# TRI-ML/sdflabel

Hardware: AMD Instinct MI355X
Metric: rendered rays/sec (fwd+bwd) (higher is better)
Workload: dtype f32; 1 GPU; BASELINE configs[1]: one 256x256 crop(s) per GPU, DeepSDF 8x512 on a 40^3 grid, fwd+bwd to yaw/trans/latent, decoder re-evaluated every step; crops_per_gpu=1, rays_per_crop=65536, grid_points=64000, surfels=2751, front_facing=763, parallelism=crop-parallel x1

## Files before the change

### include/sdfr.h

```cpp
#ifndef SDFR_H
#define SDFR_H

#include <stdint.h>

#ifdef __cplusplus
extern "C" {
#endif

#define SDFR_OK 0
#define SDFR_E_INVALID (-1)
#define SDFR_E_HIP (-2)
#define SDFR_E_UNSUPPORTED (-3)

#define SDFR_MAX_LAYERS 16
#define SDFR_TRACE_LEVELS 6
#define SDFR_TRACE_COUNTERS 32

#define SDFR_VERSION 421

int sdfr_version(void);
int sdfr_build_flags(void);
const char* sdfr_last_error(void);

typedef struct sdfr_decoder sdfr_decoder;

int sdfr_decoder_create(sdfr_decoder** out, int n_lin, const int* in_dim, const int* out_dim,
                        const int* inj_n, const int* inj_off, const float* const* h_W, const float* const* h_b,
                        const float* const* h_ln_w, const float* const* h_ln_b, int n_inputs, int use_tanh, int device);
int sdfr_decoder_destroy(sdfr_decoder* dec);
int64_t sdfr_decoder_macs(const sdfr_decoder* dec);

int sdfr_mlp_forward(const sdfr_decoder* dec, const float* inputs, int64_t n, float* sdf,
                     uint32_t* mask_ws ,
                     void* stream);
int sdfr_grid_tile_order(int D, int32_t* out);
int sdfr_mlp_forward_ordered(const sdfr_decoder* dec, const float* inputs, int64_t n, float* sdf, uint32_t* mask_ws, const int32_t* order,
                             int64_t order_rows, void* stream);
int64_t sdfr_mlp_balance_bytes(int64_t order_rows);
int sdfr_mlp_balance_init(void* state, const int32_t* order, int64_t order_rows, void* stream);
int sdfr_mlp_forward_balanced(const sdfr_decoder* dec, const float* inputs, int64_t n, float* sdf, uint32_t* mask_ws, void* state,
                              int64_t order_rows, void* stream);
int sdfr_mlp_forward_f16(const sdfr_decoder* dec, const float* inputs, int64_t n, float* sdf, uint32_t* mask_ws, void* stream);

int sdfr_mlp_forward_f16_counted(const sdfr_decoder* dec, const float* inputs, int64_t n_max, const int32_t* n_dev, float* sdf, uint32_t* mask_ws,
                                 void* stream);

int sdfr_mlp_forward_split(const sdfr_decoder* dec, const float* inputs, int64_t n, float* sdf, uint32_t* mask_ws, void* stream);
int sdfr_mlp_forward_split_counted(const sdfr_decoder* dec, const float* inputs, int64_t n_max, const int32_t* n_dev, float* sdf, void* stream);
int64_t sdfr_decoder_mask_words(const sdfr_decoder* dec, int64_t n);

int sdfr_mlp_jacobian(const sdfr_decoder* dec, const float* inputs, int64_t rows_per_crop, int B,
                      const int32_t* idx, int cap, const int32_t* cnt, float* J, float* sdf_sel,
                      const float* sdf_full ,
                      const uint32_t* mask_ws ,
                      int mask_from_f16 ,
                      void* stream);


int sdfr_band_select(const float* sdf, int64_t G, int B, float thr, int32_t* idx, int cap, int32_t* cnt,
                     int32_t* slot, int32_t* scratch, void* stream);

int sdfr_surface_project(const float* xyz, int xyz_stride, const float* sdf, int64_t G, int B,
                         const int32_t* idx, int cap, const int32_t* cnt, const float* J, int Jstride, int Joff,
                         float* points, float* nocs, float* normals, void* stream);

int sdfr_surface_project_bwd(const float* g_points, const float* g_nocs, const float* normals, int64_t G, int B,
                             const int32_t* idx, int cap, const int32_t* cnt, float* g_sdf, float* g_xyz, void* stream);

int sdfr_scatter_values(float* dst, const float* src, const int32_t* idx, int64_t G, int B, int cap, const int32_t* cnt, void* stream);
int sdfr_band_select_margin(const float* sdf, int64_t G, int B, float thr, const float* thr_extra, int32_t* idx, int cap, int32_t* cnt,
                            int32_t* slot, int32_t* scratch, void* stream);
int sdfr_prefilter_guard(float* sdf_grid, const float* sdf_exact, const int32_t* idx, int64_t G, int B, int cap, const int32_t* cnt,
                         float* margin, float* max_dev, int32_t* violations, void* stream);
int sdfr_prefilter_plan(const float* inputs, int64_t G, int n_inputs, int L, int B, float lip, const float* margin, const float* max_dev,
                        float* lat_ref, int32_t* age, int max_reuse, int32_t* reuse, int32_t* n_full, void* stream);
int sdfr_mlp_forward_f16_skip(const sdfr_decoder* dec, const float* inputs, int64_t n, float* sdf, const int32_t* skip, int64_t rows_per_crop,
                              void* stream);
int sdfr_band_select_skip(const float* sdf, int64_t G, int B, float thr, const float* thr_extra, const int32_t* skip, int32_t* idx, int cap,
                          int32_t* cnt, int32_t* slot, int32_t* scratch, void* stream);
int sdfr_prefilter_guard2(float* sdf_grid, const float* sdf_exact, const int32_t* idx, int64_t G, int B, int cap, const int32_t* cnt,
                          float* margin, float* max_dev, int32_t* violations, const int32_t* reused, void* stream);
int sdfr_gather_rows(float* out, const float* src, int ncol, const int32_t* idx, const int32_t* slot, int64_t G, int B, int cap,
                     int src_cap, const int32_t* cnt, void* stream);
int sdfr_prefilter_audit_select(const float* inputs, const int32_t* cslot, int64_t G, int n_inputs, int B, int stride, const int32_t* phase,
                                float* rows, int32_t* src, int32_t* n_audit, int cap_rows, void* stream);
int sdfr_prefilter_audit_check(const float* sdf_grid, const float* sdf_exact, const int32_t* src, const int32_t* n_audit, int cap_rows,
                               int64_t G, int B, float thr, const int32_t* reused, float* audit_dev, int32_t* violations, int32_t* phase,
                               void* stream);

int sdfr_candidate_rows(const float* inputs, int64_t G, int n_inputs, int B, const int32_t* cidx, int stride, const int32_t* ccnt, float* rows,
                        void* stream);
int sdfr_mlp_forward_f16_ragged(const sdfr_decoder* dec, const float* inputs, int B, int64_t rows_per_crop, const int32_t* cnt, float* sdf,
                                uint32_t* mask_ws, int half_tiles, void* stream);
int sdfr_candidate_band_map(const int32_t* idx, int cap, const int32_t* cnt, const int32_t* cslot, int64_t G, int B, int stride, int32_t* pos,
                            int32_t* violations, void* stream);
int sdfr_mlp_forward_skip(const sdfr_decoder* dec, const float* inputs, int64_t n, float* sdf, const int32_t* skip, int64_t rows_per_crop,
                          void* stream);
int sdfr_mlp_forward_ragged(const sdfr_decoder* dec, const float* inputs, int B, int64_t rows_per_crop, const int32_t* cnt, float* sdf,
                            uint32_t* mask_ws, int half_tiles, void* stream);

int sdfr_sdf_input_grad(const float* g_sdf, const int32_t* slot, const float* J, int n_inputs, int64_t G, int B, int cap,
                        float* g_inputs, int32_t* n_uncached, void* stream);

int sdfr_project_dcm(const float* pose, const float* K, const float* points, const float* normals, const float* colors,
                     int B, int cap, const int32_t* cnt, int output_nocs, int res_x, int res_y,
                     float* p_cam, float* n_cam, float* col, float* uv, int32_t* fidx, int32_t* fcnt, float* xyzf, int32_t* fslot,
                     void* stream);

int sdfr_surfels_forward(const float* xyz, int xyz_stride, const float* sdf, int64_t G, const int32_t* idx, const float* J, int Jstride,
                         int Joff, const float* pose, const float* K, int B, int cap, const int32_t* cnt, int output_nocs, int res_x,
                         int res_y, float diam, float* points, float* normals, float* p_cam, float* n_cam, float* col, int32_t* fidx,
                         int32_t* fcnt, float* xyzf, int32_t* fslot, int32_t* bbox, void* stream);

int sdfr_project_dcm_bwd(const float* pose, const float* points, const float* normals,
                         const float* g_p_cam, const float* g_n_cam, const float* g_col,
                         int B, int cap, const int32_t* cnt, int output_nocs,
                         float* g_points, float* g_normals, float* g_colors, float* g_pose, const float* g_xyzf, const int32_t* fslot,
                         void* stream);

#define SDFR_JAC_MANY_ROWS 16
#define SDFR_JAC_HALF_TILES 32
#define SDFR_JAC_QUARTER_TILES 64
#define SDFR_PRIM_BOXES_READY 256
#define SDFR_PRIM_BINS 512
int64_t sdfr_splat_ws_words(int B, int cap, int W, int H);
int sdfr_splat_forward(int primitive, const float* K, const float* Kinv, const float* p_cam, const float* n_cam, const float* attr,
                       const float* uv, const float* znorm, const float* bg, const float* bg_logit,
                       int B, int cap, const int32_t* cnt, int W, int H, float diam, float depth_constant,
                       int32_t* bbox_ws ,
                       float* color, float* mask, float* depth, float* normals, float* aux, void* stream);

int sdfr_splat_backward(int primitive, const float* K, const float* Kinv, const float* p_cam, const float* n_cam, const float* attr,
                        const float* uv, const float* znorm, const float* bg, const float* bg_logit,
                        int B, int cap, const int32_t* cnt, int W, int H, float diam, float depth_constant,
                        const float* aux, const float* color, const float* mask, const float* depth, const float* normals,
                        const float* g_color, const float* g_mask, const float* g_depth, const float* g_normals,
                        float* g_p_cam, float* g_n_cam, float* g_attr, void* stream);

int64_t sdfr_splat_ws_words_r(int B, int cap, int tiles_cap);
int sdfr_surfels_forward_r(const float* xyz, int xyz_stride, const float* sdf, int64_t G, const int32_t* idx, const float* J, int Jstride,
                           int Joff, const float* pose, const float* K, int B, int cap, const int32_t* cnt, int output_nocs,
                           const int32_t* wh, int tiles_cap, float diam, float* points, float* normals, float* p_cam, float* n_cam, float* col,
                           int32_t* fidx, int32_t* fcnt, float* xyzf, int32_t* fslot, int32_t* bbox, void* stream);
int sdfr_splat_forward_r(int flags , const float* K, const float* Kinv, const float* p_cam,
                         const float* n_cam, const float* attr, int B, int cap, const int32_t* cnt, const int32_t* wh, int pix_stride,
                         int tiles_cap, float diam, float depth_constant, int32_t* bbox_ws, float* color, float* mask, float* depth,
                         float* normals, float* aux, void* stream);
int sdfr_splat_backward_r(const float* K, const float* Kinv, const float* p_cam, const float* n_cam, const float* attr, int B, int cap,
                          const int32_t* cnt, const int32_t* wh, int pix_stride, float diam, float depth_constant, const float* aux,
                          const float* color, const float* mask, const float* depth, const float* normals, const float* g_color,
                          const float* g_mask, const float* g_depth, const float* g_normals, float* g_p_cam, float* g_n_cam, float* g_attr,
                          void* stream);
int sdfr_loss_2d_r(const float* rend, const float* target, int B, const int32_t* wh, int pix_stride, int tiles16_cap, float diam,
                   float threshold_nocs, float weight, float* loss, float* g_rend, int32_t* nvalid, float* scratch, void* stream);

int sdfr_splat_weights(int primitive, const float* K, const float* Kinv, const float* p_cam, const float* n_cam, const float* uv,
                       const float* znorm, const float* bg_logit, int B, int cap, const int32_t* cnt, int W, int H, float diam,
                       float depth_constant, const float* aux, float* weights, void* stream);
int sdfr_splat_weights_backward(int primitive, const float* K, const float* Kinv, const float* p_cam, const float* n_cam, const float* uv,
                                const float* znorm, int has_bg_row, int B, int cap, const int32_t* cnt, int W, int H, float diam,
                                float depth_constant, const float* aux, const float* g_weights, const float* wsum, float* g_p_cam,
                                float* g_n_cam, void* stream);

int sdfr_splat_forward_clamp(int primitive, const float* K, const float* Kinv, const float* p_cam, const float* n_cam, const float* attr,
                             const float* uv, const float* znorm, const float* bg, const float* bg_logit, int B, int cap, const int32_t* cnt,
                             int W, int H, float diam, float depth_constant, int clamp_alt, float clamp_constant, int32_t* bbox_ws,
                             float* color, float* mask, float* depth, float* normals, float* aux, void* stream);
int sdfr_splat_weights_clamp(int primitive, const float* K, const float* Kinv, const float* p_cam, const float* n_cam, const float* uv,
                             const float* znorm, const float* bg_logit, int B, int cap, const int32_t* cnt, int W, int H, float diam,
                             float depth_constant, int clamp_alt, float clamp_constant, const float* aux, float* weights, void* stream);
int sdfr_splat_weights_backward_clamp(int primitive, const float* K, const float* Kinv, const float* p_cam, const float* n_cam, const float* uv,
                                      const float* znorm, int has_bg_row, int B, int cap, const int32_t* cnt, int W, int H, float diam,
                                      float depth_constant, int clamp_alt, float clamp_constant, const float* aux, const float* g_weights,
                                      const float* wsum, float* g_p_cam, float* g_n_cam, void* stream);


int sdfr_params_forward(const float* yaw, const float* trans, const float* latent, int L, const float* grid, int64_t G, int B,
                        float* inputs, float* pose, float* latnorm, void* stream);

int sdfr_surface_latent_grad(const float* g_points, const float* g_nocs, const float* normals, const float* J, int n_inputs, int L,
                             int B, int cap, const int32_t* cnt, float* g_latn, void* stream);

int sdfr_params_backward(const float* yaw, const float* latent, int L, const float* latnorm, const float* g_pose, const float* g_latn,
                         int B, float* g_yaw, float* g_trans, float* g_latent, void* stream);

int sdfr_pose_latent_backward(const float* pose, const float* points, const float* normals, const float* g_p_cam, const float* g_n_cam,
                              const float* g_col, int B, int cap, const int32_t* cnt, int output_nocs, const float* g_xyzf,
                              const int32_t* fslot, const float* J, int n_inputs, int L, const float* yaw, const float* latent,
                              const float* latnorm, float* g_points, float* g_pose, float* g_latn, float* g_yaw, float* g_trans,
                              float* g_latent, void* stream);

int sdfr_gather_rows3(float* out, const float* src, const int32_t* idx, int B, int cap, const int32_t* cnt, void* stream);
int sdfr_scatter_add_rows3(float* dst, const float* src, const int32_t* idx, int B, int cap, const int32_t* cnt, void* stream);


int sdfr_loss_3d(const float* est, const int32_t* ecnt, int ecap, const float* lidar, const int32_t* lcnt, int lcap, const float* scale,
                 float threshold, float weight, int B, float* loss, float* g_est, float* g_scale, int32_t* npairs, float* scratch,
                 void* stream);

int sdfr_loss_2d(const float* rend, const float* target, int B, int H, int W, float diam, float threshold_nocs, float weight,
                 float* loss, float* g_rend, int32_t* nvalid, float* scratch , void* stream);

int sdfr_solver_step(float* params, const float* grads, int L, const float* loss2d, const float* loss3d, const int32_t* npairs,
                     float w2, float w3, float* adam_m, float* adam_v, int32_t* adam_t, float lr_adam, float lr_scale, float lr_latent,
                     int B, float* total, int32_t* stepped, void* stream);

int sdfr_params_plan(const float* yaw, const float* trans, const float* latent, int L, const float* grid, int64_t G, int B, float* inputs,
                     float* pose, float* latnorm, float lip, const float* margin, const float* max_dev, float* lat_ref, int32_t* age,
                     int max_reuse, int32_t* reuse, int32_t* n_full, void* stream);
int sdfr_band_select_ex(const float* sdf, int64_t G, int B, float thr, const float* thr_extra, const int32_t* skip, int32_t* idx, int cap,
                        int32_t* cnt, int32_t* slot, int32_t* scratch, int32_t* over, int over_bit, void* stream);
int sdfr_mlp_forward_candidates(const sdfr_decoder* d, const float* inputs, int64_t rows_per_crop_in, int B, const int32_t* cidx, int64_t stride,
                                const int32_t* cnt, float* sdf, uint32_t* mask_ws, int half, int half_tiles, void* stream);
int sdfr_candidate_band(float* sdf_grid, const float* csdf, const int32_t* cidx, int64_t G, int B, int stride, const int32_t* ccnt, float thr,
                        int32_t* idx, int cap, int32_t* cnt, int32_t* pos, int32_t* over, void* stream);
int sdfr_losses_fused(const float* rend, const float* target, int B, int H, int W, const int32_t* wh, int pix_stride, int tiles16_cap, float diam,
                      float threshold_nocs, float weight2d, float* loss2d, float* g_rend, int32_t* nvalid, float* scratch2, const float* est,
                      const int32_t* ecnt, int ecap, const float* lidar, const int32_t* lcnt, int lcap, const float* scale, float threshold3d,
                      float weight3d, float* loss3d, float* g_est, float* g_scale, int32_t* npairs, float* scratch3, float* kscale,
                      void* stream);
int sdfr_splat_backward_x(const float* K, const float* Kinv, const float* p_cam, const float* n_cam, const float* attr, int B, int cap,
                          const int32_t* cnt, int W, int H, const int32_t* wh, int pix_stride, float diam, float depth_constant, const float* aux,
                          const float* color, const float* g_color, const float* kscale, float* g_p_cam, float* g_n_cam, float* g_attr,
                          const int32_t* bbox_ws, void* stream);
int sdfr_pose_latent_solver(const float* pose, const float* points, const float* normals, const float* g_p_cam, const float* g_n_cam,
                            const float* g_col, int B, int cap, const int32_t* cnt, int output_nocs, const float* g_xyzf, const int32_t* fslot,
                            const float* kscale, const float* J, int n_inputs, int L, const float* yaw, const float* latent, const float* latnorm,
                            float* g_pose, float* g_latn, float* params, float* grads, const float* loss2d, const float* loss3d,
                            const int32_t* npairs, float w2, float w3, float* adam_m, float* adam_v, int32_t* adam_t, float lr_adam,
                            float lr_scale, float lr_latent, float* total, int32_t* stepped, void* stream);

int sdfr_mlp_forward_counted(const sdfr_decoder* dec, const float* inputs, int64_t n_max, const int32_t* n_dev, float* sdf, int half,
                             void* stream);
int sdfr_trace_setup(const float* pose, const float* Kinv, const float* latn, int L, int B, int W, int H, float bound, float near,
                     int32_t* counters, int32_t* pix,
                     float* lam ,
                     float* far, float* inputs, const float* cone, int cone_block, void* stream);
int sdfr_trace_setup2(const float* pose, const float* Kinv, const float* latn, int L, int B, int W, int H, float bound, float near,
                      int32_t* counters, int32_t* pix, float* lam, float* far, float* inputs, const float* cone, int cone_block, float* hit_lam,
                      float* hit_sdf, void* stream);
int sdfr_trace_cone(const sdfr_decoder* dec, const float* pose, const float* Kinv, const float* latn, int L, int B, int W, int H, float bound,
                    float near, float eps, int block, int cone_steps, int spec_k, float sigma, int half, int32_t* counters, int32_t* ids0,
                    float* st0, float* aux0, int32_t* ids1, float* st1, float* aux1, float* inputs, float* sdf, float* cone, void* stream);
int sdfr_trace_step(const float* pose, const float* Kinv, const float* latn, int L, int W, int H, float eps, const float* sdf,
                    int32_t* counters, int step, int64_t n_max, const int32_t* pix_in, const float* lam_in, int32_t* pix_out, float* lam_out,
                    const float* far, float* inputs, float* hit_lam, float* hit_sdf, void* stream);

int sdfr_trace_pool(void);
int sdfr_trace_march(const sdfr_decoder* dec, const float* pose, const float* Kinv, const float* latn, int L, int B, int W, int H, float eps,
                     int steps, int head_steps, int tail_rows, const int32_t* levels, int n_levels, float q_max, float sigma, int half,
                     int32_t* counters, int32_t* pix0, float* lam0, int32_t* pix1, float* lam1, int32_t* pix2, float* lam2, const float* far,
                     float* inputs, float* sdf, float* tail_rows_buf, float* hit_lam, float* hit_sdf, void* stream);
int sdfr_trace_hits(const float* pose, const float* Kinv, const float* latn, int L, int B, int W, int H, const float* hit_lam, int32_t* n_hits,
                    int32_t* hit_slot, int32_t* idx, float* rows, void* stream);
int sdfr_trace_composite(const float* pose, const float* Kinv, int L, int B, int W, int H, const float* hit_lam, const int32_t* hit_slot,
                         const float* J, const float* f0, float* color, float* mask, float* depth, float* normals, float* lam_s, void* stream);
int64_t sdfr_trace_backward_ws_floats(int B, int W, int H);
int sdfr_trace_backward(const float* pose, const float* Kinv, int L, int B, int W, int H, const float* hit_lam, const int32_t* hit_slot,
                        const float* J, const float* f0, const float* g_color, const float* g_depth, const float* g_normals, float* ws,
                        float* g_pose, float* g_latn, void* stream);

typedef struct sdfr_extents { const int32_t* wh; int pix_stride; int cone_cap; } sdfr_extents;
int sdfr_trace_setup_r(const float* pose, const float* Kinv, const float* latn, int L, int B, const sdfr_extents* ext, float bound, float near,
                       int32_t* counters, int32_t* pix, float* lam, float* far, float* inputs, const float* cone, int cone_block, float* hit_lam,
                       float* hit_sdf, void* stream);
int sdfr_trace_cone_r(const sdfr_decoder* dec, const float* pose, const float* Kinv, const float* latn, int L, int B, const sdfr_extents* ext,
                      float bound, float near, float eps, int block, int cone_steps, int spec_k, float sigma, int half, int32_t* counters,
                      int32_t* ids0, float* st0, float* aux0, int32_t* ids1, float* st1, float* aux1, float* inputs, float* sdf, float* cone,
                      void* stream);
int sdfr_trace_march_r(const sdfr_decoder* dec, const float* pose, const float* Kinv, const float* latn, int L, int B, const sdfr_extents* ext, float eps,
                       int steps, int head_steps, int tail_rows, const int32_t* levels, int n_levels, float q_max, float sigma, int half,
                       int32_t* counters, int32_t* pix0, float* lam0, int32_t* pix1, float* lam1, int32_t* pix2, float* lam2, const float* far,
                       float* inputs, float* sdf, float* tail_rows_buf, float* hit_lam, float* hit_sdf, void* stream);
int sdfr_trace_hits_r(const float* pose, const float* Kinv, const float* latn, int L, int B, const sdfr_extents* ext, const float* hit_lam,
                      int32_t* n_hits, int32_t* hit_slot, int32_t* idx, float* rows, void* stream);
int sdfr_trace_composite_r(const float* pose, const float* Kinv, int L, int B, const sdfr_extents* ext, const float* hit_lam, const int32_t* hit_slot,
                           const float* J, const float* f0, float* color, float* mask, float* depth, float* normals, float* lam_s, void* stream);
int sdfr_trace_points_r(const float* Kinv, int B, const sdfr_extents* ext, const int32_t* hit_slot, const float* lam_s, float* xyzf, int ecap,
                        int32_t* ecnt, int32_t* pt_slot, void* stream);
int sdfr_trace_refine_backward_r(const float* pose, const float* Kinv, int L, int B, const sdfr_extents* ext, const float* hit_lam,
                                 const int32_t* hit_slot, const float* J, const float* f0, const float* g_color, const float* g_depth,
                                 const float* g_normals, const float* g_xyzf, const int32_t* pt_slot, int ecap, int surfel, float* ws ,
                                 float* g_pose, float* g_latn, void* stream);

int sdfr_trace_points(const float* Kinv, int B, int W, int H, const int32_t* hit_slot, const float* lam_s, float* xyzf, int ecap,
                      int32_t* ecnt, int32_t* pt_slot, void* stream);
int sdfr_trace_refine_backward(const float* pose, const float* Kinv, int L, int B, int W, int H, const float* hit_lam, const int32_t* hit_slot,
                               const float* J, const float* f0, const float* g_color, const float* g_depth, const float* g_normals,
                               const float* g_xyzf, const int32_t* pt_slot, int ecap, int surfel, float* ws, float* g_pose, float* g_latn,
                               void* stream);

int sdfr_scale_net(const float* latent_row, int L, const float* W1, const float* b1, const float* W2, const float* b2, const float* W3,
                   const float* b3, float* out, void* stream);

int64_t sdfr_ransac_ws_bytes(int B, int ncap, int T);
int sdfr_ransac_sample(int64_t seed, const int64_t* keys, const int32_t* ncnt, int B, int T, int32_t* idx, void* stream);
int sdfr_ransac_pose(const float* model, const float* model_cls, const int32_t* mcnt, int mcap, int model_f16, const float* scene,
                     const float* scene_cls, const int32_t* ncnt, int ncap, int B, const int32_t* idx, int64_t seed, const int64_t* keys,
                     int T, int type, float scale_model, const double* h_thr, void* ws, int32_t* found, int32_t* best, int32_t* n_inliers,
                     float* scale, float* rot, float* tra, int32_t* cnn_idx, int32_t* gate, int32_t* counts, int32_t* idx_out, void* stream);

int sdfr_rotate_iou(const float* boxes, int N, const float* qboxes, int K, int G, const int32_t* boff, const int32_t* qoff,
                    const int64_t* ooff, int criterion, float* out, int64_t out_len, void* stream);
int sdfr_box3d_iou(const double* boxes, int N, const double* qboxes, int K, int G, const int32_t* boff, const int32_t* qoff,
                   const int64_t* ooff, int criterion, int camera_frame, const float* rinc, float* out, int64_t out_len, void* stream);
int sdfr_image_box_iou(const double* boxes, int N, const double* qboxes, int K, int G, const int32_t* boff, const int32_t* qoff,
                       const int64_t* ooff, int criterion, double* out, int64_t out_len, void* stream);

int64_t sdfr_eval_ws_bytes(int G, int NG, int C, int S, int max_nd, int frames_per_chunk);
int sdfr_eval_center_dist(const double* dt_loc, int ND, const double* gt_loc, int NG, int G, const int32_t* doff, const int32_t* goff,
                          const int64_t* ooff, int camera_frame, double* out, int64_t out_len, void* stream);
int sdfr_eval_match_scores(const void* overlaps, int ov_f32, int64_t ov_len, const int64_t* ooff, const int32_t* doff, const int32_t* goff,
                           int G, int ND, int NG, const double* dt_score, const int8_t* ign_dt, const int8_t* ign_gt, int ML, int K,
                           const double* min_overlap, int max_nd, void* ws, int64_t ws_bytes, double* out, void* stream);
int sdfr_eval_thresholds(const double* scores, int NG, const int64_t* num_gt, int ML, int K, int S, void* ws, int64_t ws_bytes, double* thr,
                         int32_t* nthr, int32_t* count, void* stream);
int sdfr_eval_pr(const void* overlaps, int ov_f32, int64_t ov_len, const int64_t* ooff, const int32_t* doff, const int32_t* goff, int G,
                 int ND, int NG, const double* dt_score, const double* dt_yaw, const double* dt_alpha, const double* gt_yaw,
                 const double* gt_alpha, const double* dt_bbox, const int8_t* ign_dt, const int8_t* ign_gt, const double* dc_boxes,
                 int NDC, const int32_t* dc_off, int ML, int K, const double* min_overlap, const double* thr, const int32_t* nthr,
                 int S, int angular, int max_nd, int frames_per_chunk, void* ws, int64_t ws_bytes, double* pr, void* stream);

int sdfr_reproject(const float* depth, const float* color, const int32_t* meta, const float* kinv, int B, int max_pix, int filter, int cap,
                   float* points, float* colors, int32_t* cnt, int32_t* scratch, int32_t* over, int over_bit, void* stream);
int sdfr_point_extents(const float* pts, const int64_t* off, const int32_t* cnt, int cap, int B, const float* A, const float* scale,
                       const float* t, const float* K, int flags, float* ext, int32_t* n_out, void* stream);

int sdfr_depth_map(const void* lidar, int lidar_f64, int N, const float* planes, const double* cam, int w, int h, float* depth,
                   int32_t* winner, int32_t* info, void* stream);
int sdfr_depth_map_masked(const void* lidar, int lidar_f64, int N, const uint8_t* mask, const float* planes, const double* cam, int w, int h,
                          float* depth, int32_t* winner, int32_t* info, void* stream);
int sdfr_match_boxes(const double* anno, int A, const double* det, int M, int32_t* best, double* iou, int32_t* keep, void* stream);
int sdfr_css_input(const float* image, int H, int W, const int32_t* meta, int A, const float* masks, int ksize, int n_hblocks,
                   int32_t* coef, uint8_t* tmp, float* im, float* im_orig, uint8_t* u8, void* stream);

#define SDFR_AUG_PARAMS 20
#define SDFR_AUG_BRIGHTNESS 0
#define SDFR_AUG_CONTRAST 1
#define SDFR_AUG_SATURATION 2
#define SDFR_AUG_HUE 3
#define SDFR_AUG_ORDER 4
#define SDFR_AUG_MATRIX 8
#define SDFR_AUG_BOX_I 14
#define SDFR_AUG_BOX_J 15
#define SDFR_AUG_BOX_H 16
#define SDFR_AUG_BOX_W 17
int sdfr_augment(const uint8_t* rgb_src, const uint8_t* uvw_src, const int32_t* meta, const double* params, int B, int ksize, int32_t* tab,
                 uint8_t* jit, uint8_t* mid_rgb, uint8_t* mid_uvw, float* rgb, uint8_t* uvw, uint8_t* mask, uint8_t* rgb_u8, void* stream);

int64_t sdfr_lidar_normals_ws_bytes(int N);
int sdfr_lidar_normals(const void* points, int points_f64, int N, const float* planes, float radius, int max_nn, double* normals,
                       int32_t* nn_count, int32_t* nn_idx, uint8_t* in_frustum, void* workspace, int64_t workspace_bytes, void* stream);

int sdfr_css_head(const float* x_u, const float* x_v, const float* x_w, const float* x_mask, int B, int C, int H, int W, const float* w_u,
                  const float* b_u, const float* w_v, const float* b_v, const float* w_w, const float* b_w, const float* w_mask,
                  const float* b_mask, float* uvw_sm, float* uvw_sm_masked, float* mask, float* mask_sm, float* u, float* v, float* w,
                  void* stream);
int sdfr_css_latent(const float* x4, int B, int C, int h, int w, const float* w_lat, const float* b_lat, float* latent, void* stream);

#define SDFR_CSS_LOSS_WS_FIXED 16045824ll
int sdfr_css_head_loss(const float* x_u, const float* x_v, const float* x_w, const float* x_mask, int B, int C, int H, int W, const float* w_u,
                       const float* b_u, const float* w_v, const float* b_v, const float* w_w, const float* b_w, const float* w_mask,
                       const float* b_mask, const uint8_t* uvw_gt, const uint8_t* mask_gt, float* loss, float* dx_u, float* dx_v, float* dx_w,
                       float* dx_mask, float* dw_u, float* db_u, float* dw_v, float* db_v, float* dw_w, float* db_w, float* dw_mask,
// ... 95 lines not shown
```

### sdflabel_amd/_lib.py

```python
import ctypes
import os
from ctypes import POINTER, c_char_p, c_float, c_int, c_int32, c_int64, c_void_p

_HERE = os.path.dirname(os.path.abspath(__file__))
LIB_PATH = os.environ.get("SDFR_LIB") or os.path.join(_HERE, "lib", "libsdfr_hip.so")

ABI_VERSION = 421
_lib = None

_PROTOS = {
    "sdfr_version": (c_int, []),
    "sdfr_build_flags": (c_int, []),
    "sdfr_last_error": (c_char_p, []),
    "sdfr_debug_set_trace": (c_int, [c_void_p]),
    "sdfr_debug_set_tile_trace": (c_int, [c_void_p, c_int64]),
    "sdfr_mlp_forward_counted": (c_int, [c_void_p, c_void_p, c_int64, c_void_p, c_void_p, c_int, c_void_p]),
    "sdfr_trace_setup": (c_int, [c_void_p, c_void_p, c_void_p, c_int, c_int, c_int, c_int, c_float, c_float, c_void_p, c_void_p, c_void_p,
                                 c_void_p, c_void_p, c_void_p, c_int, c_void_p]),
    "sdfr_trace_setup2": (c_int, [c_void_p, c_void_p, c_void_p, c_int, c_int, c_int, c_int, c_float, c_float, c_void_p, c_void_p, c_void_p,
                                  c_void_p, c_void_p, c_void_p, c_int, c_void_p, c_void_p, c_void_p]),
    "sdfr_trace_cone": (c_int, [c_void_p, c_void_p, c_void_p, c_void_p, c_int, c_int, c_int, c_int, c_float, c_float, c_float, c_int, c_int,
                                c_int, c_float, c_int, c_void_p, c_void_p, c_void_p, c_void_p, c_void_p, c_void_p, c_void_p, c_void_p, c_void_p,
                                c_void_p, c_void_p]),
    "sdfr_trace_step": (c_int, [c_void_p, c_void_p, c_void_p, c_int, c_int, c_int, c_float, c_void_p, c_void_p, c_int, c_int64, c_void_p,
                                c_void_p, c_void_p, c_void_p, c_void_p, c_void_p, c_void_p, c_void_p, c_void_p]),
    "sdfr_trace_march": (c_int, [c_void_p, c_void_p, c_void_p, c_void_p, c_int, c_int, c_int, c_int, c_float, c_int, c_int, c_int, c_void_p, c_int,
                                 c_float, c_float, c_int, c_void_p, c_void_p, c_void_p, c_void_p, c_void_p, c_void_p, c_void_p, c_void_p,
                                 c_void_p, c_void_p, c_void_p, c_void_p, c_void_p, c_void_p]),
    "sdfr_trace_pool": (c_int, []),
    "sdfr_trace_hits": (c_int, [c_void_p, c_void_p, c_void_p, c_int, c_int, c_int, c_int, c_void_p, c_void_p, c_void_p, c_void_p, c_void_p, c_void_p]),
    "sdfr_trace_composite": (c_int, [c_void_p, c_void_p, c_int, c_int, c_int, c_int, c_void_p, c_void_p, c_void_p, c_void_p, c_void_p, c_void_p,
                                     c_void_p, c_void_p, c_void_p, c_void_p]),
    "sdfr_trace_backward_ws_floats": (c_int64, [c_int, c_int, c_int]),
    "sdfr_trace_backward": (c_int, [c_void_p, c_void_p, c_int, c_int, c_int, c_int, c_void_p, c_void_p, c_void_p, c_void_p, c_void_p, c_void_p,
                                    c_void_p, c_void_p, c_void_p, c_void_p, c_void_p]),
    "sdfr_trace_setup_r": (c_int, [c_void_p, c_void_p, c_void_p, c_int, c_int, c_void_p, c_float, c_float, c_void_p, c_void_p, c_void_p, c_void_p,
                                   c_void_p, c_void_p, c_int, c_void_p, c_void_p, c_void_p]),
    "sdfr_trace_cone_r": (c_int, [c_void_p, c_void_p, c_void_p, c_void_p, c_int, c_int, c_void_p, c_float, c_float, c_float, c_int, c_int, c_int,
                                  c_float, c_int, c_void_p, c_void_p, c_void_p, c_void_p, c_void_p, c_void_p, c_void_p, c_void_p, c_void_p, c_void_p,
                                  c_void_p]),
    "sdfr_trace_march_r": (c_int, [c_void_p, c_void_p, c_void_p, c_void_p, c_int, c_int, c_void_p, c_float, c_int, c_int, c_int, c_void_p, c_int,
                                   c_float, c_float, c_int, c_void_p, c_void_p, c_void_p, c_void_p, c_void_p, c_void_p, c_void_p, c_void_p, c_void_p,
                                   c_void_p, c_void_p, c_void_p, c_void_p, c_void_p]),
    "sdfr_trace_hits_r": (c_int, [c_void_p, c_void_p, c_void_p, c_int, c_int, c_void_p, c_void_p, c_void_p, c_void_p, c_void_p, c_void_p, c_void_p]),
    "sdfr_trace_composite_r": (c_int, [c_void_p, c_void_p, c_int, c_int, c_void_p, c_void_p, c_void_p, c_void_p, c_void_p, c_void_p, c_void_p, c_void_p,
                                       c_void_p, c_void_p, c_void_p]),
    "sdfr_trace_points_r": (c_int, [c_void_p, c_int, c_void_p, c_void_p, c_void_p, c_void_p, c_int, c_void_p, c_void_p, c_void_p]),
    "sdfr_trace_refine_backward_r": (c_int, [c_void_p, c_void_p, c_int, c_int, c_void_p, c_void_p, c_void_p, c_void_p, c_void_p, c_void_p, c_void_p,
                                             c_void_p, c_void_p, c_void_p, c_int, c_int, c_void_p, c_void_p, c_void_p, c_void_p]),
    "sdfr_trace_points": (c_int, [c_void_p, c_int, c_int, c_int, c_void_p, c_void_p, c_void_p, c_int, c_void_p, c_void_p, c_void_p]),
    "sdfr_trace_refine_backward": (c_int, [c_void_p, c_void_p, c_int, c_int, c_int, c_int, c_void_p, c_void_p, c_void_p, c_void_p, c_void_p,
                                           c_void_p, c_void_p, c_void_p, c_void_p, c_int, c_int, c_void_p, c_void_p, c_void_p, c_void_p]),
    "sdfr_splat_ws_words_r": (c_int64, [c_int, c_int, c_int]),
    "sdfr_surfels_forward_r": (c_int, [c_void_p, c_int, c_void_p, c_int64, c_void_p, c_void_p, c_int, c_int, c_void_p, c_void_p, c_int, c_int,
                                       c_void_p, c_int, c_void_p, c_int, c_float, c_void_p, c_void_p, c_void_p, c_void_p, c_void_p, c_void_p, c_void_p,
                                       c_void_p, c_void_p, c_void_p, c_void_p]),
    "sdfr_splat_forward_r": (c_int, [c_int, c_void_p, c_void_p, c_void_p, c_void_p, c_void_p, c_int, c_int, c_void_p, c_void_p, c_int, c_int,
                                     c_float, c_float, c_void_p, c_void_p, c_void_p, c_void_p, c_void_p, c_void_p, c_void_p]),
    "sdfr_splat_backward_r": (c_int, [c_void_p, c_void_p, c_void_p, c_void_p, c_void_p, c_int, c_int, c_void_p, c_void_p, c_int, c_float, c_float,
                                      c_void_p, c_void_p, c_void_p, c_void_p, c_void_p, c_void_p, c_void_p, c_void_p, c_void_p, c_void_p, c_void_p,
                                      c_void_p, c_void_p]),
    "sdfr_loss_2d_r": (c_int, [c_void_p, c_void_p, c_int, c_void_p, c_int, c_int, c_float, c_float, c_float, c_void_p, c_void_p, c_void_p,
                               c_void_p, c_void_p]),
    "sdfr_prefilter_audit_select": (c_int, [c_void_p, c_void_p, c_int64, c_int, c_int, c_int, c_void_p, c_void_p, c_void_p, c_void_p, c_int, c_void_p]),
    "sdfr_prefilter_audit_check": (c_int, [c_void_p, c_void_p, c_void_p, c_void_p, c_int, c_int64, c_int, c_float, c_void_p, c_void_p, c_void_p,
                                           c_void_p, c_void_p]),
    "sdfr_scale_net": (c_int, [c_void_p, c_int, c_void_p, c_void_p, c_void_p, c_void_p, c_void_p, c_void_p, c_void_p, c_void_p]),
    "sdfr_decoder_create": (c_int, [POINTER(c_void_p), c_int, POINTER(c_int), POINTER(c_int), POINTER(c_int), POINTER(c_int),
                                    POINTER(c_void_p), POINTER(c_void_p), POINTER(c_void_p), POINTER(c_void_p), c_int, c_int, c_int]),
    "sdfr_decoder_destroy": (c_int, [c_void_p]),
    "sdfr_decoder_macs": (c_int64, [c_void_p]),
    "sdfr_mlp_forward": (c_int, [c_void_p, c_void_p, c_int64, c_void_p, c_void_p, c_void_p]),
    "sdfr_grid_tile_order": (c_int, [c_int, c_void_p]),
    "sdfr_mlp_forward_ordered": (c_int, [c_void_p, c_void_p, c_int64, c_void_p, c_void_p, c_void_p, c_int64, c_void_p]),
    "sdfr_mlp_balance_bytes": (c_int64, [c_int64]),
    "sdfr_mlp_balance_init": (c_int, [c_void_p, c_void_p, c_int64, c_void_p]),
    "sdfr_mlp_forward_balanced": (c_int, [c_void_p, c_void_p, c_int64, c_void_p, c_void_p, c_void_p, c_int64, c_void_p]),
    "sdfr_mlp_forward_f16": (c_int, [c_void_p, c_void_p, c_int64, c_void_p, c_void_p, c_void_p]),
    "sdfr_mlp_forward_f16_counted": (c_int, [c_void_p, c_void_p, c_int64, c_void_p, c_void_p, c_void_p, c_void_p]),
    "sdfr_mlp_forward_split": (c_int, [c_void_p, c_void_p, c_int64, c_void_p, c_void_p, c_void_p]),
    "sdfr_mlp_forward_split_counted": (c_int, [c_void_p, c_void_p, c_int64, c_void_p, c_void_p, c_void_p]),
    "sdfr_decoder_mask_words": (c_int64, [c_void_p, c_int64]),
    "sdfr_mlp_jacobian": (c_int, [c_void_p, c_void_p, c_int64, c_int, c_void_p, c_int, c_void_p, c_void_p, c_void_p, c_void_p,
                                  c_void_p, c_int, c_void_p]),
    "sdfr_band_select": (c_int, [c_void_p, c_int64, c_int, c_float, c_void_p, c_int, c_void_p, c_void_p, c_void_p, c_void_p]),
    "sdfr_band_select_margin": (c_int, [c_void_p, c_int64, c_int, c_float, c_void_p, c_void_p, c_int, c_void_p, c_void_p, c_void_p, c_void_p]),
    "sdfr_prefilter_guard": (c_int, [c_void_p, c_void_p, c_void_p, c_int64, c_int, c_int, c_void_p, c_void_p, c_void_p, c_void_p, c_void_p]),
    "sdfr_prefilter_plan": (c_int, [c_void_p, c_int64, c_int, c_int, c_int, c_float, c_void_p, c_void_p, c_void_p, c_void_p, c_int, c_void_p, c_void_p,
                                    c_void_p]),
    "sdfr_mlp_forward_f16_skip": (c_int, [c_void_p, c_void_p, c_int64, c_void_p, c_void_p, c_int64, c_void_p]),
    "sdfr_band_select_skip": (c_int, [c_void_p, c_int64, c_int, c_float, c_void_p, c_void_p, c_void_p, c_int, c_void_p, c_void_p, c_void_p, c_void_p]),
    "sdfr_prefilter_guard2": (c_int, [c_void_p, c_void_p, c_void_p, c_int64, c_int, c_int, c_void_p, c_void_p, c_void_p, c_void_p, c_void_p, c_void_p]),
    "sdfr_candidate_rows": (c_int, [c_void_p, c_int64, c_int, c_int, c_void_p, c_int, c_void_p, c_void_p, c_void_p]),
    "sdfr_mlp_forward_f16_ragged": (c_int, [c_void_p, c_void_p, c_int, c_int64, c_void_p, c_void_p, c_void_p, c_int, c_void_p]),
    "sdfr_mlp_forward_skip": (c_int, [c_void_p, c_void_p, c_int64, c_void_p, c_void_p, c_int64, c_void_p]),
    "sdfr_mlp_forward_ragged": (c_int, [c_void_p, c_void_p, c_int, c_int64, c_void_p, c_void_p, c_void_p, c_int, c_void_p]),
    "sdfr_candidate_band_map": (c_int, [c_void_p, c_int, c_void_p, c_void_p, c_int64, c_int, c_int, c_void_p, c_void_p, c_void_p]),
    "sdfr_surface_project": (c_int, [c_void_p, c_int, c_void_p, c_int64, c_int, c_void_p, c_int, c_void_p, c_void_p, c_int, c_int,
                                     c_void_p, c_void_p, c_void_p, c_void_p]),
    "sdfr_surface_project_bwd": (c_int, [c_void_p, c_void_p, c_void_p, c_int64, c_int, c_void_p, c_int, c_void_p, c_void_p, c_void_p,
                                         c_void_p]),
    "sdfr_sdf_input_grad": (c_int, [c_void_p, c_void_p, c_void_p, c_int, c_int64, c_int, c_int, c_void_p, c_void_p, c_void_p]),
    "sdfr_project_dcm": (c_int, [c_void_p, c_void_p, c_void_p, c_void_p, c_void_p, c_int, c_int, c_void_p, c_int, c_int, c_int,
                                 c_void_p, c_void_p, c_void_p, c_void_p, c_void_p, c_void_p, c_void_p, c_void_p, c_void_p]),
    "sdfr_surfels_forward": (c_int, [c_void_p, c_int, c_void_p, c_int64, c_void_p, c_void_p, c_int, c_int, c_void_p, c_void_p, c_int, c_int,
                                     c_void_p, c_int, c_int, c_int, c_float, c_void_p, c_void_p, c_void_p, c_void_p, c_void_p, c_void_p, c_void_p,
                                     c_void_p, c_void_p, c_void_p, c_void_p]),
    "sdfr_project_dcm_bwd": (c_int, [c_void_p, c_void_p, c_void_p, c_void_p, c_void_p, c_void_p, c_int, c_int, c_void_p, c_int,
                                     c_void_p, c_void_p, c_void_p, c_void_p, c_void_p, c_void_p, c_void_p]),
    "sdfr_splat_forward": (c_int, [c_int, c_void_p, c_void_p, c_void_p, c_void_p, c_void_p, c_void_p, c_void_p, c_void_p, c_void_p,
                                   c_int, c_int, c_void_p, c_int, c_int, c_float, c_float, c_void_p, c_void_p, c_void_p, c_void_p,
                                   c_void_p, c_void_p, c_void_p]),
    "sdfr_splat_backward": (c_int, [c_int, c_void_p, c_void_p, c_void_p, c_void_p, c_void_p, c_void_p, c_void_p, c_void_p, c_void_p,
                                    c_int, c_int, c_void_p, c_int, c_int, c_float, c_float, c_void_p, c_void_p, c_void_p, c_void_p,
                                    c_void_p, c_void_p, c_void_p, c_void_p, c_void_p, c_void_p, c_void_p, c_void_p, c_void_p]),
    "sdfr_splat_ws_words": (c_int64, [c_int, c_int, c_int, c_int]),
    "sdfr_splat_weights": (c_int, [c_int, c_void_p, c_void_p, c_void_p, c_void_p, c_void_p, c_void_p, c_void_p, c_int, c_int, c_void_p, c_int,
                                   c_int, c_float, c_float, c_void_p, c_void_p, c_void_p]),
    "sdfr_splat_weights_backward": (c_int, [c_int, c_void_p, c_void_p, c_void_p, c_void_p, c_void_p, c_void_p, c_int, c_int, c_int, c_void_p,
                                            c_int, c_int, c_float, c_float, c_void_p, c_void_p, c_void_p, c_void_p, c_void_p, c_void_p]),
    "sdfr_splat_forward_clamp": (c_int, [c_int, c_void_p, c_void_p, c_void_p, c_void_p, c_void_p, c_void_p, c_void_p, c_void_p, c_void_p,
                                         c_int, c_int, c_void_p, c_int, c_int, c_float, c_float, c_int, c_float, c_void_p, c_void_p, c_void_p, c_void_p,
                                         c_void_p, c_void_p, c_void_p]),
    "sdfr_splat_weights_clamp": (c_int, [c_int, c_void_p, c_void_p, c_void_p, c_void_p, c_void_p, c_void_p, c_void_p, c_int, c_int, c_void_p, c_int,
                                         c_int, c_float, c_float, c_int, c_float, c_void_p, c_void_p, c_void_p]),
    "sdfr_splat_weights_backward_clamp": (c_int, [c_int, c_void_p, c_void_p, c_void_p, c_void_p, c_void_p, c_void_p, c_int, c_int, c_int, c_void_p,
                                                  c_int, c_int, c_float, c_float, c_int, c_float, c_void_p, c_void_p, c_void_p, c_void_p, c_void_p,
                                                  c_void_p]),
    "sdfr_params_forward": (c_int, [c_void_p, c_void_p, c_void_p, c_int, c_void_p, c_int64, c_int, c_void_p, c_void_p, c_void_p, c_void_p]),
    "sdfr_surface_latent_grad": (c_int, [c_void_p, c_void_p, c_void_p, c_void_p, c_int, c_int, c_int, c_int, c_void_p, c_void_p, c_void_p]),
    "sdfr_params_backward": (c_int, [c_void_p, c_void_p, c_int, c_void_p, c_void_p, c_void_p, c_int, c_void_p, c_void_p, c_void_p,
                                     c_void_p]),
    "sdfr_pose_latent_backward": (c_int, [c_void_p, c_void_p, c_void_p, c_void_p, c_void_p, c_void_p, c_int, c_int, c_void_p, c_int, c_void_p,
                                          c_void_p, c_void_p, c_int, c_int, c_void_p, c_void_p, c_void_p, c_void_p, c_void_p, c_void_p, c_void_p,
                                          c_void_p, c_void_p, c_void_p]),
    "sdfr_gather_rows3": (c_int, [c_void_p, c_void_p, c_void_p, c_int, c_int, c_void_p, c_void_p]),
    "sdfr_scatter_values": (c_int, [c_void_p, c_void_p, c_void_p, c_int64, c_int, c_int, c_void_p, c_void_p]),
    "sdfr_gather_rows": (c_int, [c_void_p, c_void_p, c_int, c_void_p, c_void_p, c_int64, c_int, c_int, c_int, c_void_p, c_void_p]),
    "sdfr_scatter_add_rows3": (c_int, [c_void_p, c_void_p, c_void_p, c_int, c_int, c_void_p, c_void_p]),
    "sdfr_loss_3d": (c_int, [c_void_p, c_void_p, c_int, c_void_p, c_void_p, c_int, c_void_p, c_float, c_float, c_int, c_void_p, c_void_p,
                             c_void_p, c_void_p, c_void_p, c_void_p]),
    "sdfr_loss_2d": (c_int, [c_void_p, c_void_p, c_int, c_int, c_int, c_float, c_float, c_float, c_void_p, c_void_p, c_void_p, c_void_p,
                             c_void_p]),
    "sdfr_solver_step": (c_int, [c_void_p, c_void_p, c_int, c_void_p, c_void_p, c_void_p, c_float, c_float, c_void_p, c_void_p, c_void_p,
                                 c_float, c_float, c_float, c_int, c_void_p, c_void_p, c_void_p]),
    "sdfr_params_plan": (c_int, [c_void_p, c_void_p, c_void_p, c_int, c_void_p, c_int64, c_int, c_void_p, c_void_p, c_void_p, c_float, c_void_p,
                                 c_void_p, c_void_p, c_void_p, c_int, c_void_p, c_void_p, c_void_p]),
    "sdfr_band_select_ex": (c_int, [c_void_p, c_int64, c_int, c_float, c_void_p, c_void_p, c_void_p, c_int, c_void_p, c_void_p, c_void_p, c_void_p,
                                    c_int, c_void_p]),
    "sdfr_mlp_forward_candidates": (c_int, [c_void_p, c_void_p, c_int64, c_int, c_void_p, c_int64, c_void_p, c_void_p, c_void_p, c_int, c_int,
                                            c_void_p]),
    "sdfr_candidate_band": (c_int, [c_void_p, c_void_p, c_void_p, c_int64, c_int, c_int, c_void_p, c_float, c_void_p, c_int, c_void_p, c_void_p,
                                    c_void_p, c_void_p]),
    "sdfr_losses_fused": (c_int, [c_void_p, c_void_p, c_int, c_int, c_int, c_void_p, c_int, c_int, c_float, c_float, c_float, c_void_p, c_void_p,
                                  c_void_p, c_void_p, c_void_p, c_void_p, c_int, c_void_p, c_void_p, c_int, c_void_p, c_float, c_float, c_void_p,
                                  c_void_p, c_void_p, c_void_p, c_void_p, c_void_p, c_void_p]),
    "sdfr_splat_backward_x": (c_int, [c_void_p, c_void_p, c_void_p, c_void_p, c_void_p, c_int, c_int, c_void_p, c_int, c_int, c_void_p, c_int,
                                      c_float, c_float, c_void_p, c_void_p, c_void_p, c_void_p, c_void_p, c_void_p, c_void_p, c_void_p, c_void_p]),
    "sdfr_pose_latent_solver": (c_int, [c_void_p, c_void_p, c_void_p, c_void_p, c_void_p, c_void_p, c_int, c_int, c_void_p, c_int, c_void_p,
                                        c_void_p, c_void_p, c_void_p, c_int, c_int, c_void_p, c_void_p, c_void_p, c_void_p, c_void_p, c_void_p,
                                        c_void_p, c_void_p, c_void_p, c_void_p, c_float, c_float, c_void_p, c_void_p, c_void_p, c_float, c_float,
                                        c_float, c_void_p, c_void_p, c_void_p]),
    "sdfr_ransac_ws_bytes": (c_int64, [c_int, c_int, c_int]),
    "sdfr_ransac_sample": (c_int, [c_int64, c_void_p, c_void_p, c_int, c_int, c_void_p, c_void_p]),
    "sdfr_ransac_pose": (c_int, [c_void_p, c_void_p, c_void_p, c_int, c_int, c_void_p, c_void_p, c_void_p, c_int, c_int, c_void_p, c_int64,
                                 c_void_p, c_int, c_int, c_float, c_void_p, c_void_p, c_void_p, c_void_p, c_void_p, c_void_p, c_void_p, c_void_p,
                                 c_void_p, c_void_p, c_void_p, c_void_p, c_void_p]),
    "sdfr_rotate_iou": (c_int, [c_void_p, c_int, c_void_p, c_int, c_int, c_void_p, c_void_p, c_void_p, c_int, c_void_p, c_int64, c_void_p]),
    "sdfr_box3d_iou": (c_int, [c_void_p, c_int, c_void_p, c_int, c_int, c_void_p, c_void_p, c_void_p, c_int, c_int, c_void_p, c_void_p,
                               c_int64, c_void_p]),
    "sdfr_image_box_iou": (c_int, [c_void_p, c_int, c_void_p, c_int, c_int, c_void_p, c_void_p, c_void_p, c_int, c_void_p, c_int64, c_void_p]),
    "sdfr_eval_ws_bytes": (c_int64, [c_int, c_int, c_int, c_int, c_int, c_int]),
    "sdfr_eval_center_dist": (c_int, [c_void_p, c_int, c_void_p, c_int, c_int, c_void_p, c_void_p, c_void_p, c_int, c_void_p, c_int64, c_void_p]),
    "sdfr_eval_match_scores": (c_int, [c_void_p, c_int, c_int64, c_void_p, c_void_p, c_void_p, c_int, c_int, c_int, c_void_p, c_void_p, c_void_p,
                                       c_int, c_int, c_void_p, c_int, c_void_p, c_int64, c_void_p, c_void_p]),
    "sdfr_eval_thresholds": (c_int, [c_void_p, c_int, c_void_p, c_int, c_int, c_int, c_void_p, c_int64, c_void_p, c_void_p, c_void_p, c_void_p]),
    "sdfr_eval_pr": (c_int, [c_void_p, c_int, c_int64, c_void_p, c_void_p, c_void_p, c_int, c_int, c_int, c_void_p, c_void_p, c_void_p, c_void_p,
                             c_void_p, c_void_p, c_void_p, c_void_p, c_void_p, c_int, c_void_p, c_int, c_int, c_void_p, c_void_p, c_void_p, c_int,
                             c_int, c_int, c_int, c_void_p, c_int64, c_void_p, c_void_p]),
    "sdfr_reproject": (c_int, [c_void_p, c_void_p, c_void_p, c_void_p, c_int, c_int, c_int, c_int, c_void_p, c_void_p, c_void_p, c_void_p,
                               c_void_p, c_int, c_void_p]),
    "sdfr_point_extents": (c_int, [c_void_p, c_void_p, c_void_p, c_int, c_int, c_void_p, c_void_p, c_void_p, c_void_p, c_int, c_void_p,
                                   c_void_p, c_void_p]),
    "sdfr_depth_map": (c_int, [c_void_p, c_int, c_int, c_void_p, c_void_p, c_int, c_int, c_void_p, c_void_p, c_void_p, c_void_p]),
    "sdfr_match_boxes": (c_int, [c_void_p, c_int, c_void_p, c_int, c_void_p, c_void_p, c_void_p, c_void_p]),
    "sdfr_css_input": (c_int, [c_void_p, c_int, c_int, c_void_p, c_int, c_void_p, c_int, c_int, c_void_p, c_void_p, c_void_p, c_void_p,
                               c_void_p, c_void_p]),
    "sdfr_depth_map_masked": (c_int, [c_void_p, c_int, c_int, c_void_p, c_void_p, c_void_p, c_int, c_int, c_void_p, c_void_p, c_void_p, c_void_p]),
    "sdfr_augment": (c_int, [c_void_p, c_void_p, c_void_p, c_void_p, c_int, c_int] + [c_void_p] * 9),
    "sdfr_lidar_normals_ws_bytes": (c_int64, [c_int]),
    "sdfr_lidar_normals": (c_int, [c_void_p, c_int, c_int, c_void_p, c_float, c_int, c_void_p, c_void_p, c_void_p, c_void_p, c_void_p, c_int64,
                                   c_void_p]),
    "sdfr_css_head": (c_int, [c_void_p, c_void_p, c_void_p, c_void_p, c_int, c_int, c_int, c_int, c_void_p, c_void_p, c_void_p, c_void_p, c_void_p,
                              c_void_p, c_void_p, c_void_p, c_void_p, c_void_p, c_void_p, c_void_p, c_void_p, c_void_p, c_void_p, c_void_p]),
    "sdfr_css_latent": (c_int, [c_void_p, c_int, c_int, c_int, c_int, c_void_p, c_void_p, c_void_p, c_void_p]),
    "sdfr_css_head_loss": (c_int, [c_void_p, c_void_p, c_void_p, c_void_p, c_int, c_int, c_int, c_int] + [c_void_p] * 8 + [c_void_p, c_void_p]
                           + [c_void_p] * 13 + [c_void_p, c_int64, c_void_p]),
    "sdfr_css_latent_loss": (c_int, [c_void_p, c_int, c_int, c_int, c_int, c_void_p, c_void_p, c_void_p, c_void_p, c_void_p, c_void_p, c_void_p,
                                     c_void_p, c_int64, c_void_p]),
    "sdfr_mesh_ws_bytes": (c_int64, [c_int, c_int]),
    "sdfr_mesh_lattice_inputs": (c_int, [c_void_p, c_int, c_int, c_int, c_int64, c_int64, c_void_p, c_void_p]),
    "sdfr_mesh_count": (c_int, [c_void_p, c_int, c_int, c_void_p, c_void_p, c_void_p, c_int64, c_void_p]),
    "sdfr_mesh_emit": (c_int, [c_void_p, c_int, c_int, c_void_p, c_void_p, c_void_p, c_int64, c_void_p, c_int64, c_void_p, c_int64, c_void_p]),
    "sdfr_mesh_raster": (c_int, [c_void_p, c_int64, c_void_p, c_int64, c_void_p, c_void_p, c_void_p, c_void_p, c_int64, c_int, c_int, c_int,
                                 c_void_p, c_float, c_void_p, c_void_p, c_void_p, c_void_p, c_void_p, c_void_p]),
    "sdfr_verify_mask_counts": (c_int, [c_void_p, c_void_p, c_void_p, c_void_p, c_int64, c_int, c_int, c_int, c_void_p, c_void_p]),
    "sdfr_verify_point_rows": (c_int, [c_void_p, c_int64, c_void_p, c_int, c_void_p, c_void_p, c_int, c_int64, c_int64, c_void_p, c_void_p,
                                       c_void_p]),
    "sdfr_verify_band_counts": (c_int, [c_void_p, c_void_p, c_int64, c_void_p, c_int, c_void_p, c_float, c_void_p, c_void_p]),
    "sdfr_crop_owner": (c_int, [c_void_p, c_void_p, c_void_p, c_void_p, c_int64, c_int, c_int, c_int, c_void_p, c_void_p]),
    "sdfr_crop_export": (c_int, [c_void_p, c_int64, c_void_p, c_int64, c_void_p, c_void_p, c_void_p, c_void_p, c_void_p, c_int64, c_void_p, c_void_p,
                                 c_void_p, c_void_p, c_int64, c_void_p, c_int, c_int, c_int, c_void_p, c_float, c_void_p, c_void_p, c_void_p,
                                 c_void_p]),
    "sdfr_crop_counts": (c_int, [c_void_p, c_void_p, c_void_p, c_void_p, c_int64, c_void_p, c_void_p, c_int64, c_void_p, c_int, c_int, c_int,
                                 c_void_p, c_void_p]),
    "sdfr_synth_owner": (c_int, [c_void_p, c_void_p, c_void_p, c_void_p, c_int64, c_void_p, c_int, c_int, c_int, c_void_p, c_void_p]),
    "sdfr_synth_shade": (c_int, [c_void_p, c_int64, c_void_p, c_int64, c_void_p, c_void_p, c_void_p, c_void_p, c_void_p, c_int64, c_void_p, c_void_p,
                                 c_void_p, c_void_p, c_void_p, c_int64, c_void_p, c_void_p, c_int, c_void_p, c_void_p, c_int, c_void_p, c_int, c_int,
                                 c_int, c_void_p, c_float, c_void_p, c_void_p, c_void_p]),
    "sdfr_mesh_sdf_ws_bytes": (c_int64, [c_int, c_int64, c_int64]),
    "sdfr_mesh_sdf": (c_int, [c_void_p, c_int64, c_void_p, c_int64, c_void_p, c_void_p, c_void_p, c_int64, c_void_p, c_int, c_int, c_void_p, c_int64,
                              c_void_p, c_void_p, c_void_p, c_void_p, c_void_p, c_void_p, c_void_p]),
    "sdfr_mesh_surface_ws_bytes": (c_int64, [c_int, c_int64]),
    "sdfr_mesh_surface_points": (c_int, [c_void_p, c_int64, c_void_p, c_int64, c_void_p, c_void_p, c_void_p, c_int64, c_void_p, c_int, c_void_p,
                                         c_int64, c_void_p, c_void_p, c_void_p, c_void_p]),
    "sdfr_decoder_train_bytes": (c_int64, [c_int, POINTER(c_int), POINTER(c_int), POINTER(c_int), POINTER(c_int), c_int, c_int64]),
    "sdfr_decoder_train_forward": (c_int, [c_int, POINTER(c_int), POINTER(c_int), POINTER(c_int), POINTER(c_int), c_int, c_int, POINTER(c_void_p),
                                           POINTER(c_void_p), c_void_p, c_int64, c_float, c_int, c_int64, c_void_p, c_void_p, c_int64, c_void_p]),
    "sdfr_decoder_train_backward": (c_int, [c_int, POINTER(c_int), POINTER(c_int), POINTER(c_int), POINTER(c_int), c_int, c_int, POINTER(c_void_p),
                                            c_void_p, c_int64, c_void_p, c_int64, POINTER(c_void_p), POINTER(c_void_p), c_void_p, c_void_p]),
    "sdfr_encode_ws_bytes": (c_int64, [c_int, c_int64, c_int]),
    "sdfr_encode_rows": (c_int, [c_void_p, c_int64, c_void_p, c_int, c_int, c_int64, c_int, c_int64, c_int64, c_void_p, c_int, c_int, c_void_p, c_void_p,
                                 c_void_p, c_void_p, c_void_p]),
    "sdfr_encode_reduce": (c_int, [c_void_p, c_void_p, c_void_p, c_int, c_int, c_int, c_int64, c_float, c_void_p, c_int64, c_void_p, c_void_p,
                                   c_void_p, c_void_p]),
    "sdfr_encode_step": (c_int, [c_void_p, c_void_p, c_void_p, c_int, c_int, c_int, c_void_p, c_void_p, c_void_p, c_float, c_float, c_int, c_void_p,
                                 c_int64, c_void_p]),
    "sdfr_view_samples": (c_int, [c_void_p, c_void_p, c_int64, c_void_p, c_int, c_void_p, c_void_p, c_int, c_int, c_float, c_float, c_int64,
                                  c_void_p, c_void_p, c_void_p]),
    "sdfr_bound_rows": (c_int, [c_void_p, c_int64, c_void_p, c_int, c_int, c_int64, c_int, c_int64, c_int64, c_void_p, c_int, c_int, c_void_p, c_void_p,
                                c_void_p, c_void_p, c_void_p, c_void_p]),
    "sdfr_bound_reduce": (c_int, [c_void_p, c_void_p, c_void_p, c_void_p, c_int, c_int, c_int, c_int64, c_float, c_void_p, c_int64, c_void_p, c_void_p,
                                  c_void_p, c_void_p]),
    "sdfr_align_samples": (c_int, [c_void_p, c_void_p, c_int64, c_void_p, c_int, c_void_p, c_int, c_int, c_float, c_float, c_int64, c_void_p,
                                   c_void_p, c_void_p]),
    "sdfr_align_rows": (c_int, [c_void_p, c_int64, c_void_p, c_int, c_int, c_int64, c_int, c_int64, c_int64, c_void_p, c_int, c_int, c_void_p, c_void_p,
                                c_void_p, c_void_p, c_void_p, c_void_p, c_void_p, c_void_p]),
    "sdfr_align_ws_bytes": (c_int64, [c_int, c_int64, c_int]),
    "sdfr_align_reduce": (c_int, [c_void_p, c_void_p, c_void_p, c_void_p, c_int, c_void_p, c_void_p, c_int, c_int, c_int64, c_float, c_void_p, c_int64,
                                  c_void_p, c_void_p, c_void_p, c_void_p]),
    "sdfr_align_step": (c_int, [c_void_p, c_void_p, c_void_p, c_int, c_int, c_int, c_void_p, c_void_p, c_void_p, c_void_p, c_void_p, c_void_p, c_void_p,
                                c_float, c_float, c_void_p, c_int, c_void_p, c_int64, c_void_p]),
    "sdfr_cluster_ws_bytes": (c_int64, [c_int, c_int]),
    "sdfr_lidar_clusters": (c_int, [c_void_p, c_int, c_int, c_void_p, c_float, c_int, c_int, c_int, c_void_p, c_void_p, c_void_p, c_void_p, c_void_p,
                                    c_int64, c_void_p]),
    "sdfr_cluster_boxes": (c_int, [c_void_p, c_int, c_int, c_void_p, c_void_p, c_void_p, c_int, c_void_p, c_int, c_void_p, c_void_p]),
}

EXPORTS = tuple(_PROTOS)


class SdfrError(RuntimeError):
    pass


class Extents(ctypes.Structure):
    _fields_ = [("wh", c_void_p), ("pix_stride", c_int), ("cone_cap", c_int)]


def lib():
    global _lib
    if _lib is None:
        if not os.path.isfile(LIB_PATH):
            raise SdfrError("libsdfr_hip.so is missing (%s): build it with `python -c 'import __graft_entry__ as g; g.build()'` "
                            "or sdflabel_amd/csrc/build.sh -- there is no CPU fallback" % LIB_PATH)
        h = ctypes.CDLL(LIB_PATH)
        try:
            h.sdfr_version.restype = c_int
            h.sdfr_version.argtypes = []
            ver = int(h.sdfr_version())
        except AttributeError:
            ver = -1
        if ver != ABI_VERSION:
            raise SdfrError("%s reports ABI version %d, this binding is written against %d (include/sdfr.h SDFR_VERSION): rebuild the library"
                            % (LIB_PATH, ver, ABI_VERSION))
        for name, (res, args) in _PROTOS.items():
            fn = getattr(h, name)
            fn.restype = res
            fn.argtypes = args
        if h.sdfr_version() != ABI_VERSION:
            raise SdfrError("%s reports ABI version %d, this binding is written against %d (include/sdfr.h SDFR_VERSION): rebuild the library"
                            % (LIB_PATH, h.sdfr_version(), ABI_VERSION))
        flags = h.sdfr_build_flags()
        if flags and os.environ.get("SDFR_ALLOW_AB") != "1":
            raise SdfrError("%s is an experiment build (sdfr_build_flags() = %d%s): the product refuses it; set SDFR_ALLOW_AB=1 for A/B timing runs"
                            % (LIB_PATH, flags, ", results wrong by construction" if flags & 2 else ""))
        _lib = h
    return _lib


def check(rc, what):
    if rc != 0:
# ... 89 lines not shown
```

### sdflabel_amd/batch.py

```python
import math
import os

import torch

from . import _lib
from .grid import Grid3D

_DIAM_DISC = 0.04
_DEPTH_CONSTANT = 150.0
P, ck = _lib.ptr, _lib.check


class BatchRenderer:
    def __init__(self, decoder, density, K, resolution_px, batch, cap=None, device="cuda", threshold=0.03, output_nocs=True,
                 max_pixels=None, max_side=None, candidate_reuse=None):
        dev = torch.device(device)
        if dev.type != "cuda":
            raise _lib.SdfrError("BatchRenderer runs on the GPU only")
        self.dev, self.B = dev, int(batch)
        self._f = lambda *shape: torch.zeros(shape, dtype=torch.float32, device=dev)
        self._i = lambda *shape: torch.zeros(shape, dtype=torch.int32, device=dev)
        self.W, self.H = int(resolution_px[0]), int(resolution_px[1])
        self.thr = float(threshold)
        self.nocs_mode = 1 if output_nocs else 0
        if not output_nocs:
            raise NotImplementedError("BatchRenderer composites NOCS colours (the optimizer's configuration)")
        self.decoder = decoder
        prec = getattr(decoder, "mlp_precision", torch.float32)
        self.f16, self.split, self.prefilter = prec == torch.float16, prec == "float32_split", prec == "float32_prefilter"
        self.margin = float(getattr(decoder, "prefilter_margin", 0.005))
        self.handle = decoder.handle(dev)
        self.fused = bool(getattr(decoder, "fused_launches", True))
        self.L, self.NI = decoder.latent_size, decoder.latent_size + 3
        self.grid = Grid3D(density, dev).points.detach().contiguous()
        self.G = self.grid.shape[0]
        self.fwd_order = None
        if prec == torch.float32 and self.handle.hp == 512 and not self.handle.has_ln and self.G == int(density) ** 3:
            order = torch.empty(self.G, dtype=torch.int32)
            ck(_lib.lib().sdfr_grid_tile_order(int(density), P(order)), "sdfr_grid_tile_order")
            self.fwd_order = order.to(dev)
            lib = _lib.lib()
            self.fwd_balance = torch.empty(int(lib.sdfr_mlp_balance_bytes(self.G)) // 4, dtype=torch.int32, device=dev)
            with _lib.guard(dev):
                ck(lib.sdfr_mlp_balance_init(P(self.fwd_balance), P(self.fwd_order), self.G, _lib.stream_ptr()), "sdfr_mlp_balance_init")
        self.cap = int(cap) if cap is not None else max(256, self.G // 8)
        self._init_extents(K, max_pixels, max_side)
        self._alloc_common()
        want_reuse = bool(getattr(decoder, "candidate_reuse", False)) if candidate_reuse is None else bool(candidate_reuse)
        self.creuse = (self.f16 or prec == torch.float32) and want_reuse and self.handle.hp == 512 and not self.handle.has_ln
        self.reuse_off_reason = None
        if want_reuse and not self.creuse:
            self.reuse_off_reason = "candidate reuse needs a float16 / float32 decoder of padded width 512 without LayerNorm"
        if self.prefilter:
            self._setup_prefilter(decoder)
        elif self.creuse:
            self._setup_candidate_reuse(decoder)
        self.mode = "prefilter" if self.prefilter else ("creuse" if self.creuse else "plain")
        self.guarded = self.prefilter or self.creuse
        self.n_full = self._i(self.B) if self.guarded else None
        if self.guarded:
            self._alloc_audit()
            self.fault = None
        self._alloc_surfels_images_backward()
        self._graph = None
        self.freeze_shape, self._shape_valid = False, False
        self.fused_tail = True
        self.fused_head = True

    def _init_extents(self, K, max_pixels, max_side):
        B, W, H, dev = self.B, self.W, self.H, self.dev
        self.ragged = max_pixels is not None
        if self.ragged:
            self.PS = int(max_pixels)
            self.max_side = int(max_side) if max_side is not None else min(self.PS, 4 * int(math.ceil(math.sqrt(self.PS))))
            if W * H > self.PS or max(W, H) > self.max_side:
                raise _lib.SdfrError("resolution_px %dx%d exceeds max_pixels %d / max_side %d" % (W, H, self.PS, self.max_side))
            self.tiles_cap = (self.PS + 63) // 64 + (2 * self.max_side + 7) // 8 + 2
            self.tiles16_cap = (self.PS + 255) // 256 + (2 * self.max_side + 15) // 16 + 2
            self.wh = torch.tensor([[W, H]] * B, dtype=torch.int32, device=dev)
            self.sizes = [(W, H)] * B
        else:
            self.PS = W * H
        K = torch.as_tensor(K, dtype=torch.float32)
        if K.dim() == 2:
            K = K.unsqueeze(0).expand(B, 3, 3)
        self.K = K.contiguous().to(dev)
        self.Kinv = torch.linalg.inv(K.cpu().float()).contiguous().to(dev)

    def _alloc_common(self):
        f, i, B, G, cap, NI = self._f, self._i, self.B, self.G, self.cap, self.NI
        self.yaw, self.trans, self.latent = f(B), f(B, 3), f(B, self.L)
        self.inputs, self.sdf, self.pose, self.latnorm = f(B * G, NI), f(B * G), f(B, 16), f(B)
        self.mask_ws = i(int(_lib.lib().sdfr_decoder_mask_words(self.handle.h, B * G)))
        self.idx, self.cnt, self.scratch, self.J, self.sdf_band = i(B, cap), i(B), i(B * ((G + 255) // 256) + 1), f(B, cap, NI), f(B, cap)
        self.over, self._side_pending = i(B), False

    def _half_kernel_deviation(self, each=None):
        L, G, st = _lib.lib(), self.G, _lib.stream_ptr()
        gen = torch.Generator().manual_seed(0)
        s32, s16 = self._f(G), self._f(G)
        worst = 0.0
        for _ in range(4):
            lat = torch.nn.functional.normalize(torch.randn(self.L, generator=gen), dim=0).to(self.dev)
            inp = torch.cat([lat.expand(G, -1), self.grid], 1).contiguous()
            ck(L.sdfr_mlp_forward(self.handle.h, P(inp), G, P(s32), None, st), "sdfr_mlp_forward")
            ck(L.sdfr_mlp_forward_f16(self.handle.h, P(inp), G, P(s16), None, st), "sdfr_mlp_forward_f16")
            worst = max(worst, float((s32 - s16).abs().max()))
            if each is not None:
                each(gen, lat, s32)
        return worst, inp

    def _setup_prefilter(self, decoder):
        f, i, B, G, cap, st = self._f, self._i, self.B, self.G, self.cap, _lib.stream_ptr()
        self.reuse = bool(getattr(decoder, "prefilter_reuse", False))
        self.max_reuse = int(getattr(decoder, "prefilter_max_reuse", 16))
        self.audit = bool(getattr(decoder, "prefilter_audit", True))
        self.audit_stride = int(getattr(decoder, "prefilter_audit_stride", 16))
        self.audit_split = str(getattr(decoder, "prefilter_audit_arith", "split")) == "split" and self.handle.hp == 512 and not self.handle.has_ln
        self.cidx, self.ccnt, self.cslot = i(B, cap), i(B), i(B * G)
        self.Jc = f(B, cap, self.NI)
        s32b, lip = f(G), [0.0]

        def sampled_lipschitz(gen, lat, s32):
            lat2 = torch.nn.functional.normalize(lat + 0.02 * torch.randn(self.L, generator=gen).to(self.dev), dim=0)
            inp2 = torch.cat([lat2.expand(G, -1), self.grid], 1).contiguous()
            ck(_lib.lib().sdfr_mlp_forward(self.handle.h, P(inp2), G, P(s32b), None, st), "sdfr_mlp_forward")
            lip[0] = max(lip[0], float((s32b - s32).abs().max()) / max(float((lat2 - lat).norm()), 1e-12))

        self.f16_error, _ = self._half_kernel_deviation(sampled_lipschitz)
        self.margin = max(self.margin, 4.0 * self.f16_error)
        self.lipschitz_sampled = lip[0]
        self.margin_dev = torch.full((B,), self.margin, dtype=torch.float32, device=self.dev)
        self.max_dev = f(B)
        self.violations = i(B, 2)
        self.lipschitz = float(decoder.latent_lipschitz_bound())
        self.lat_ref, self.age, self.reuse_flag = f(B, self.L), i(B), i(B)

    def _setup_candidate_reuse(self, decoder):
        f, i, B, G, cap, dev = self._f, self._i, self.B, self.G, self.cap, self.dev
        safety, max_margin = float(getattr(decoder, "candidate_error_safety", 2.0)), float(getattr(decoder, "candidate_max_margin", self.thr))
        select = str(getattr(decoder, "candidate_select", "float16"))
        self.max_reuse = int(getattr(decoder, "candidate_max_reuse", 64))
        self.audit = bool(getattr(decoder, "candidate_audit", True))
        self.audit_stride = int(getattr(decoder, "candidate_audit_stride", 32))
        self.audit_split = (not self.f16) and str(getattr(decoder, "candidate_audit_arith", "split")) == "split"
        self.audit_side = self.audit and B <= int(getattr(decoder, "candidate_audit_side_max_crops", 64)) and bool(getattr(decoder, "candidate_audit_side_stream", True))
        self.half_tiles = self.f16 and B <= 2 and bool(getattr(decoder, "candidate_half_tiles", True))
        self.quarter_tiles = self.half_tiles and B == 1 and self.fused and bool(getattr(decoder, "candidate_quarter_tiles", True))
        self.e32 = max(1e-6, 4.0 * float(decoder.kernel_error_f32(dev)))
        self.f16_deviation_sampled, self.calib_inputs = self._half_kernel_deviation()
        e16 = safety * self.f16_deviation_sampled + self.e32
        self.select_half = (not self.f16) and select == "float16"
        self.f16_error = e16 if self.f16 else self.e32
        self.select_error = e16 if self.select_half else self.f16_error
        need = 4.0 * max(self.f16_error, self.select_error)
        lipschitz = float(decoder.latent_lipschitz_bound())
        if need > max_margin:
            self.reuse_off_reason = ("kernel error %.3g (x%g safety) needs a candidate margin %.3g > candidate_max_margin %.3g"
                                     % (max(self.f16_error, self.select_error), safety, need, max_margin))
        elif not (lipschitz < float("inf")):
            self.reuse_off_reason = "no finite latent Lipschitz bound for this decoder"
        if self.reuse_off_reason is not None:
            self.creuse = False
            return
        self.cstride = cs = (cap + 127) // 128 * 128
        self.cidx, self.ccnt, self.cslot, self.cpos = i(B, cs), i(B), i(B * G), i(B, cap)
        self.crow, self.csdf = f(B * cs, self.NI), f(B * cs)
        self.cmask = i(int(_lib.lib().sdfr_decoder_mask_words(self.handle.h, B * cs)))
        self.margin_grown = need > self.margin
        self.margin = max(self.margin, need)
        self.margin_dev = torch.full((B,), self.margin, dtype=torch.float32, device=dev)
        self.max_dev = f(B)
        self.violations = i(B, 2)
        self.lipschitz = lipschitz
        kernel_errors = 2.0 * self.f16_error if self.f16 else self.select_error + self.f16_error
        self.latent_share = max(0.45, 0.95 - kernel_errors / self.margin)
        self.lipschitz_plan = self.lipschitz * (0.25 / self.latent_share)
        self.reuse = True
        self.lat_ref, self.age, self.reuse_flag = f(B, self.L), i(B), i(B)
        self._side = torch.cuda.Stream(device=dev) if self.audit_side else None

    def _alloc_audit(self):
        if self.audit:
            self.audit_cap = self.B * ((self.G + self.audit_stride - 1) // self.audit_stride)
            self.audit_rows, self.audit_src, self.audit_sdf = self._f(self.audit_cap, self.NI), self._i(self.audit_cap), self._f(self.audit_cap)
            self.audit_n, self.audit_phase, self.audit_dev = self._i(1), self._i(1), self._f(self.B)

    def _alloc_surfels_images_backward(self):
        f, i, B, cap, W, H, dev = self._f, self._i, self.B, self.cap, self.W, self.H, self.dev
        self.points, self.nocs, self.normals = f(B, cap, 3), f(B, cap, 3), f(B, cap, 3)
        self.p_cam, self.n_cam, self.attr = f(B, cap, 3), f(B, cap, 3), f(B, cap, 3)
        self.fidx, self.fcnt, self.fslot = i(B, cap), i(B), i(B, cap)
        if self.ragged:
            self.bbox = torch.empty((int(_lib.lib().sdfr_splat_ws_words_r(B, max(cap, 1), self.tiles_cap)),), dtype=torch.int32, device=dev)
        else:
            self.bbox = _lib.splat_ws(B, cap, W, H, dev)
        self.binned = B >= 4
        px = (self.PS,) if self.ragged else (H, W)
        self.color, self.mask, self.depth, self.nimg = f(B, 3, *px), f(B, 1, *px), f(B, 1, *px), f(B, 3, *px)
        self.aux, self.xyzf = f(B, self.PS, 4), f(B, cap, 3)
        self.g_p, self.g_n, self.g_a = f(B, cap, 3), f(B, cap, 3), f(B, cap, 3)
        self.g_points, self.g_normals, self.g_pose, self.g_latn = f(B, cap, 3), f(B, cap, 3), f(B, 16), f(B, self.L)
        self.g_yaw, self.g_trans, self.g_latent = f(B), f(B, 3), f(B, self.L)

    @property
    def boxes(self):
        return self.bbox[:self.B * self.cap * 4].view(self.B, self.cap, 4)

    def set_extents(self, sizes_wh, K=None):
        if not self.ragged:
            raise _lib.SdfrError("set_extents needs a BatchRenderer built with max_pixels")
        sizes = [(int(w), int(h)) for w, h in sizes_wh]
        if len(sizes) != self.B:
            raise _lib.SdfrError("set_extents: %d sizes for %d crops" % (len(sizes), self.B))
        for w, h in sizes:
            if w < 1 or h < 1 or w * h > self.PS or max(w, h) > self.max_side:
                raise _lib.SdfrError("crop of %dx%d pixels exceeds max_pixels %d / max_side %d" % (w, h, self.PS, self.max_side))
        self.sizes = sizes
        self.wh.copy_(torch.tensor(sizes, dtype=torch.int32))
        if K is not None:
            K = torch.as_tensor(K, dtype=torch.float32).cpu()
            if K.dim() == 2:
                K = K.unsqueeze(0).expand(self.B, 3, 3)
            self.K.copy_(K.contiguous())
            self.Kinv.copy_(torch.linalg.inv(K.float()).contiguous())

    def image(self, b, name="color"):
        t = {"color": self.color, "mask": self.mask, "depth": self.depth, "normals": self.nimg}[name]
        if not self.ragged:
            return t[b]
        w, h = self.sizes[b]
        return t[b, :, :w * h].view(t.shape[1], h, w)

    def set_params(self, yaw, trans, latent):
        self.yaw.copy_(yaw.reshape(self.B))
        self.trans.copy_(trans.reshape(self.B, 3))
        self.latent.copy_(latent.reshape(self.B, self.L))
        self._shape_valid = False
        self.clear_overflow()
        self.reset_guard()

    def invalidate_shape(self):
        self._shape_valid = False
        if self.guarded:
            self.age.zero_()

    def clear_overflow(self):
        self.over.zero_()

    def reset_guard(self):
        if self.guarded:
            self.age.zero_()
            self.violations.zero_()
            self.over.zero_()
            self.n_full.zero_()
            self.max_dev.zero_()
            self.margin_dev.fill_(self.margin)
            if self.audit:
                self.audit_dev.zero_()

    def forward(self, yaw=None, trans=None, latent=None, mlp_events=None, events=None):
        with _lib.guard(self.dev):
            return self._forward(yaw, trans, latent, mlp_events, events or {})

    def backward(self, g_color=None, g_mask=None, g_depth=None, g_normals=None, g_xyzf=None, events=None):
        with _lib.guard(self.dev):
            return self._backward(g_color, g_mask, g_depth, g_normals, g_xyzf, events or {})

    def _forward(self, yaw, trans, latent, mlp_events, events):
        if yaw is not None:
            self.set_params(yaw, trans, latent)
        L, st = _lib.lib(), _lib.stream_ptr()
        frozen = self.freeze_shape and self._shape_valid
        self._params_stage(L, st, frozen)
        if mlp_events is not None:
            mlp_events[0].record()
        if frozen:
            if mlp_events is not None:
                mlp_events[1].record()
        elif self.mode == "prefilter":
            self._decoder_prefilter(L, st, mlp_events)
        elif self.mode == "creuse":
            self._decoder_candidates(L, st, mlp_events, events)
        else:
            self._decoder_plain(L, st, mlp_events, events)
        self._shape_valid = True
        prim = self._surfels_stage(L, st)
        if "splat_fwd" in events:
            events["splat_fwd"][0].record()
        self._splat_stage(L, st, prim)
        if "splat_fwd" in events:
            events["splat_fwd"][1].record()
        if self._side_pending:
            torch.cuda.current_stream(self.dev).wait_stream(self._side)
            self._side_pending = False
        return {"color": self.color, "mask": self.mask, "depth": self.depth, "normals": self.nimg, "xyzf": self.xyzf, "nf": self.fcnt, "n": self.cnt}

    def _params_stage(self, L, st, frozen):
        B, G = self.B, self.G
        if self.creuse and self.fused and not frozen:
            ck(L.sdfr_params_plan(P(self.yaw), P(self.trans), P(self.latent), self.L, P(self.grid), G, B, P(self.inputs), P(self.pose), P(self.latnorm),
                                  self.lipschitz_plan, P(self.margin_dev), P(self.max_dev), P(self.lat_ref), P(self.age), self.max_reuse, P(self.reuse_flag),
                                  P(self.n_full), st), "sdfr_params_plan")
        else:
            ck(L.sdfr_params_forward(P(self.yaw), P(self.trans), P(self.latent), self.L, P(self.grid), G, B, None if frozen else P(self.inputs),
                                     P(self.pose), P(self.latnorm), st), "sdfr_params_forward")

    def _decoder_plain(self, L, st, mlp_events, events):
        B, G, cap = self.B, self.G, self.cap
        fwd = L.sdfr_mlp_forward_f16 if self.f16 else (L.sdfr_mlp_forward_split if self.split else L.sdfr_mlp_forward)
        if self.fwd_order is not None and os.environ.get("SDFR_FWD_ORDER", "1") != "0" and os.environ.get("SDFR_FWD_BALANCE", "1") != "0":
            ck(L.sdfr_mlp_forward_balanced(self.handle.h, P(self.inputs), B * G, P(self.sdf), P(self.mask_ws), P(self.fwd_balance), G, st),
               "sdfr_mlp_forward_balanced")
        elif self.fwd_order is not None and os.environ.get("SDFR_FWD_ORDER", "1") != "0":
            ck(L.sdfr_mlp_forward_ordered(self.handle.h, P(self.inputs), B * G, P(self.sdf), P(self.mask_ws), P(self.fwd_order), G, st),
               "sdfr_mlp_forward_ordered")
        else:
            ck(fwd(self.handle.h, P(self.inputs), B * G, P(self.sdf), P(self.mask_ws), st), fwd.__name__)
        if mlp_events is not None:
            mlp_events[1].record()
        ck(L.sdfr_band_select_ex(P(self.sdf), G, B, self.thr, None, None, P(self.idx), cap, P(self.cnt), None, P(self.scratch), P(self.over), 1, st),
           "sdfr_band_select_ex")
        if "jacobian" in events:
            events["jacobian"][0].record()
        ck(L.sdfr_mlp_jacobian(self.handle.h, P(self.inputs), G, B, P(self.idx), cap, P(self.cnt), P(self.J), P(self.sdf_band), P(self.sdf),
                               P(self.mask_ws), 2 if self.f16 else 0, st), "sdfr_mlp_jacobian")
        if "jacobian" in events:
            events["jacobian"][1].record()

    def _audit(self, L, st, half, reuse_flag):
        ck(L.sdfr_prefilter_audit_select(P(self.inputs), P(self.cslot), self.G, self.NI, self.B, self.audit_stride, P(self.audit_phase), P(self.audit_rows),
                                         P(self.audit_src), P(self.audit_n), self.audit_cap, st), "sdfr_prefilter_audit_select")
        if half is None:
            ck(L.sdfr_mlp_forward_split_counted(self.handle.h, P(self.audit_rows), self.audit_cap, P(self.audit_n), P(self.audit_sdf), st),
               "sdfr_mlp_forward_split_counted")
        else:
            ck(L.sdfr_mlp_forward_counted(self.handle.h, P(self.audit_rows), self.audit_cap, P(self.audit_n), P(self.audit_sdf), half, st), "sdfr_mlp_forward_counted")
        ck(L.sdfr_prefilter_audit_check(P(self.sdf), P(self.audit_sdf), P(self.audit_src), P(self.audit_n), self.audit_cap, self.G, self.B, self.thr,
                                        reuse_flag, P(self.audit_dev), P(self.violations), P(self.audit_phase), st), "sdfr_prefilter_audit_check")

    def _decoder_prefilter(self, L, st, mlp_events):
        B, G, cap = self.B, self.G, self.cap
        flag = P(self.reuse_flag) if self.reuse else None
        if self.reuse:
            ck(L.sdfr_prefilter_plan(P(self.inputs), G, self.NI, self.L, B, self.lipschitz, P(self.margin_dev), P(self.max_dev), P(self.lat_ref),
                                     P(self.age), self.max_reuse, P(self.reuse_flag), P(self.n_full), st), "sdfr_prefilter_plan")
            ck(L.sdfr_mlp_forward_f16_skip(self.handle.h, P(self.inputs), B * G, P(self.sdf), flag, G, st), "sdfr_mlp_forward_f16_skip")
        else:
            ck(L.sdfr_mlp_forward_f16(self.handle.h, P(self.inputs), B * G, P(self.sdf), None, st), "sdfr_mlp_forward_f16")
        if self.fault is not None:
            self.sdf.index_copy_(0, self.fault[0], self.fault[1])
        ck(L.sdfr_band_select_ex(P(self.sdf), G, B, self.thr, P(self.margin_dev), flag, P(self.cidx), cap, P(self.ccnt), P(self.cslot),
                                 P(self.scratch), P(self.over), 2, st), "sdfr_band_select_ex")
        if self.audit:
            self._audit(L, st, None if self.audit_split else 0, flag)
        ck(L.sdfr_mlp_jacobian(self.handle.h, P(self.inputs), G, B, P(self.cidx), cap, P(self.ccnt), P(self.Jc), P(self.sdf_band), None, None, 0, st), "sdfr_mlp_jacobian")
        ck(L.sdfr_prefilter_guard2(P(self.sdf), P(self.sdf_band), P(self.cidx), G, B, cap, P(self.ccnt), P(self.margin_dev), P(self.max_dev),
                                   P(self.violations), flag, st), "sdfr_prefilter_guard2")
        ck(L.sdfr_band_select_ex(P(self.sdf), G, B, self.thr, None, None, P(self.idx), cap, P(self.cnt), None, P(self.scratch), P(self.over), 1, st),
           "sdfr_band_select_ex")
        ck(L.sdfr_gather_rows(P(self.J), P(self.Jc), self.NI, P(self.idx), P(self.cslot), G, B, cap, cap, P(self.cnt), st), "sdfr_gather_rows")
        if mlp_events is not None:
            mlp_events[1].record()

    def _decoder_candidates(self, L, st, mlp_events, events):
        B, G, cap, cs, flag = self.B, self.G, self.cap, self.cstride, P(self.reuse_flag)
        if not self.fused:
            ck(L.sdfr_prefilter_plan(P(self.inputs), G, self.NI, self.L, B, self.lipschitz_plan, P(self.margin_dev), P(self.max_dev), P(self.lat_ref),
                                     P(self.age), self.max_reuse, P(self.reuse_flag), P(self.n_full), st), "sdfr_prefilter_plan")
        fwd_skip = L.sdfr_mlp_forward_f16_skip if (self.f16 or self.select_half) else L.sdfr_mlp_forward_skip
        ck(fwd_skip(self.handle.h, P(self.inputs), B * G, P(self.sdf), flag, G, st), fwd_skip.__name__)
        if self.fault is not None:
            self.sdf.index_copy_(0, self.fault[0], self.fault[1])
        if self.fused:
            ck(L.sdfr_band_select_ex(P(self.sdf), G, B, self.thr, P(self.margin_dev), flag, P(self.cidx), cs, P(self.ccnt), P(self.cslot),
                                     P(self.scratch), P(self.over), 2, st), "sdfr_band_select_ex")
        else:
            ck(L.sdfr_band_select_skip(P(self.sdf), G, B, self.thr, P(self.margin_dev), flag, P(self.cidx), cs, P(self.ccnt), P(self.cslot),
                                       P(self.scratch), st), "sdfr_band_select_skip")
        if self.audit:
            ast = st
            if self.audit_side:
                self._side.wait_stream(torch.cuda.current_stream(self.dev))
                ast = self._side.cuda_stream
                self._side_pending = True
            self._audit(L, ast, 3 if self.f16 else (None if self.audit_split else 0), flag)
        ht = 2 if self.quarter_tiles else (1 if self.half_tiles else 0)
        if self.fused:
            ck(L.sdfr_mlp_forward_candidates(self.handle.h, P(self.inputs), G, B, P(self.cidx), cs, P(self.ccnt), P(self.csdf), P(self.cmask),
                                             1 if self.f16 else 0, ht, st), "sdfr_mlp_forward_candidates")
            if mlp_events is not None:
                mlp_events[1].record()
            ck(L.sdfr_candidate_band(P(self.sdf), P(self.csdf), P(self.cidx), G, B, cs, P(self.ccnt), self.thr, P(self.idx), cap, P(self.cnt),
                                     P(self.cpos), P(self.over), st), "sdfr_candidate_band")
        else:
            ck(L.sdfr_candidate_rows(P(self.inputs), G, self.NI, B, P(self.cidx), cs, P(self.ccnt), P(self.crow), st), "sdfr_candidate_rows")
            fwd_ragged = L.sdfr_mlp_forward_f16_ragged if self.f16 else L.sdfr_mlp_forward_ragged
            ck(fwd_ragged(self.handle.h, P(self.crow), B, cs, P(self.ccnt), P(self.csdf), P(self.cmask), ht, st), fwd_ragged.__name__)
            ck(L.sdfr_scatter_values(P(self.sdf), P(self.csdf), P(self.cidx), G, B, cs, P(self.ccnt), st), "sdfr_scatter_values")
            if mlp_events is not None:
                mlp_events[1].record()
            ck(L.sdfr_band_select(P(self.sdf), G, B, self.thr, P(self.idx), cap, P(self.cnt), None, P(self.scratch), st), "sdfr_band_select")
            ck(L.sdfr_candidate_band_map(P(self.idx), cap, P(self.cnt), P(self.cslot), G, B, cs, P(self.cpos), P(self.violations), st), "sdfr_candidate_band_map")
        if "jacobian" in events:
            events["jacobian"][0].record()
        ck(L.sdfr_mlp_jacobian(self.handle.h, P(self.crow), cs, B, P(self.cpos), cap, P(self.cnt), P(self.J), P(self.sdf_band), P(self.csdf), P(self.cmask),
                               (2 if self.f16 else 0) | (64 if self.quarter_tiles else (32 if self.half_tiles else 0)), st), "sdfr_mlp_jacobian")
        if "jacobian" in events:
            events["jacobian"][1].record()

    def _surfels_stage(self, L, st):
        B, G, cap, NI = self.B, self.G, self.cap, self.NI
        xyz = self.inputs[:, NI - 3:]
        prim = 512 if self.binned else 0
        if self.ragged:
            ck(L.sdfr_surfels_forward_r(P(xyz), NI, P(self.sdf), G, P(self.idx), P(self.J), NI, NI - 3, P(self.pose), P(self.K), B, cap, P(self.cnt),
                                        self.nocs_mode | 4 | (8 if self.binned else 0), P(self.wh), self.tiles_cap, _DIAM_DISC, P(self.points), P(self.normals),
                                        P(self.p_cam), P(self.n_cam), P(self.attr), P(self.fidx), P(self.fcnt), P(self.xyzf), P(self.fslot), P(self.bbox), st),
               "sdfr_surfels_forward_r")
            return prim | 256
        if self.fused_head:
            ck(L.sdfr_surfels_forward(P(xyz), NI, P(self.sdf), G, P(self.idx), P(self.J), NI, NI - 3, P(self.pose), P(self.K), B, cap, P(self.cnt),
                                      self.nocs_mode | 4 | (8 if self.binned else 0), self.W, self.H, _DIAM_DISC, P(self.points), P(self.normals), P(self.p_cam),
                                      P(self.n_cam), P(self.attr), P(self.fidx), P(self.fcnt), P(self.xyzf), P(self.fslot), P(self.bbox), st), "sdfr_surfels_forward")
            return prim | 256
        ck(L.sdfr_surface_project(P(xyz), NI, P(self.sdf), G, B, P(self.idx), cap, P(self.cnt), P(self.J), NI, NI - 3,
                                  P(self.points), P(self.nocs), P(self.normals), st), "sdfr_surface_project")
        ck(L.sdfr_project_dcm(P(self.pose), P(self.K), P(self.points), P(self.normals), None, B, cap, P(self.cnt), self.nocs_mode | 4, self.W, self.H, P(self.p_cam),
                              P(self.n_cam), P(self.attr), None, P(self.fidx), P(self.fcnt), P(self.xyzf), P(self.fslot), st), "sdfr_project_dcm")
        return prim

    def _splat_stage(self, L, st, prim):
        B, cap = self.B, self.cap
        if self.ragged:
            ck(L.sdfr_splat_forward_r(prim, P(self.K), P(self.Kinv), P(self.p_cam), P(self.n_cam), P(self.attr), B, cap, P(self.cnt), P(self.wh), self.PS, self.tiles_cap,
                                      _DIAM_DISC, _DEPTH_CONSTANT, P(self.bbox), P(self.color), P(self.mask), P(self.depth), P(self.nimg), P(self.aux), st),
               "sdfr_splat_forward_r")
        else:
            ck(L.sdfr_splat_forward(prim, P(self.K), P(self.Kinv), P(self.p_cam), P(self.n_cam), P(self.attr), None, None, None, None, B, cap, P(self.cnt), self.W, self.H,
                                    _DIAM_DISC, _DEPTH_CONSTANT, P(self.bbox), P(self.color), P(self.mask), P(self.depth), P(self.nimg), P(self.aux), st),
               "sdfr_splat_forward")

    def _backward(self, g_color, g_mask, g_depth, g_normals, g_xyzf, events):
        L, st = _lib.lib(), _lib.stream_ptr()
        B, cap, W, H = self.B, self.cap, self.W, self.H

        def c(g, shape):
            return None if g is None else g.to(torch.float32).expand(shape).contiguous()

        g_color, g_mask = c(g_color, self.color.shape), c(g_mask, self.mask.shape)
        g_depth, g_normals = c(g_depth, self.depth.shape), c(g_normals, self.nimg.shape)
        if "splat_bwd" in events:
            events["splat_bwd"][0].record()
        if self.ragged:
            ck(L.sdfr_splat_backward_r(P(self.K), P(self.Kinv), P(self.p_cam), P(self.n_cam), P(self.attr), B, cap, P(self.cnt), P(self.wh), self.PS,
                                       _DIAM_DISC, _DEPTH_CONSTANT, P(self.aux), P(self.color), P(self.mask), P(self.depth), P(self.nimg),
                                       P(g_color), P(g_mask), P(g_depth), P(g_normals), P(self.g_p), P(self.g_n), P(self.g_a), st),
               "sdfr_splat_backward_r")
        else:
            ck(L.sdfr_splat_backward(0, P(self.K), P(self.Kinv), P(self.p_cam), P(self.n_cam), P(self.attr), None, None, None, None, B, cap, P(self.cnt), W, H, _DIAM_DISC,
                                     _DEPTH_CONSTANT, P(self.aux), P(self.color), P(self.mask), P(self.depth), P(self.nimg), P(g_color),
                                     P(g_mask), P(g_depth), P(g_normals), P(self.g_p), P(self.g_n), P(self.g_a), st), "sdfr_splat_backward")
        if "splat_bwd" in events:
            events["splat_bwd"][1].record()
        g_xyzf = c(g_xyzf, self.xyzf.shape)
        if self.L <= 8 and self.fused_tail:
            ck(L.sdfr_pose_latent_backward(P(self.pose), P(self.points), P(self.normals), P(self.g_p), P(self.g_n), P(self.g_a), B, cap,
                                           P(self.cnt), self.nocs_mode | 4, P(g_xyzf), P(self.fslot), None if self.freeze_shape else P(self.J), self.NI, self.L, P(self.yaw),
                                           P(self.latent), P(self.latnorm), None, P(self.g_pose), P(self.g_latn), P(self.g_yaw),
                                           P(self.g_trans), P(self.g_latent), st), "sdfr_pose_latent_backward")
            return self.g_yaw, self.g_trans, self.g_latent
        ck(L.sdfr_project_dcm_bwd(P(self.pose), P(self.points), P(self.normals), P(self.g_p), P(self.g_n), P(self.g_a), B, cap,
                                  P(self.cnt), self.nocs_mode | 4, P(self.g_points), P(self.g_normals), None, P(self.g_pose), P(g_xyzf),
                                  P(self.fslot), st), "sdfr_project_dcm_bwd")
        ck(L.sdfr_surface_latent_grad(P(self.g_points), None, P(self.normals), P(self.J), self.NI, self.L, B, cap, P(self.cnt),
# ... 95 lines not shown
```

### sdflabel_amd/csrc/mlp.hip

```cpp
#include "mlp_kernel.h"
#include <algorithm>
#include <cmath>
#include <stdlib.h>
#include <string.h>
#include <vector>


#define SDFR_DEVICE_CHECK(d, what)                                                                                                          \
    do {                                                                                                                                    \
        int cur_ = -1;                                                                                                                      \
        SDFR_HIP_CHECK(hipGetDevice(&cur_));                                                                                                \
        SDFR_REQUIRE(cur_ == (d)->device, "%s: the decoder's weights live on device %d but the current device (the launch stream's) is %d: " \
                     "create one decoder handle per device", what, (d)->device, cur_);                                                      \
    } while (0)

extern "C" int sdfr_decoder_create(sdfr_decoder** out, int n_lin, const int* in_dim, const int* out_dim,
                                   const int* inj_n, const int* inj_off, const float* const* h_W,
                                   const float* const* h_b, const float* const* h_ln_w, const float* const* h_ln_b, int n_inputs,
                                   int use_tanh, int device) {
    SDFR_REQUIRE(out && in_dim && out_dim && inj_n && inj_off && h_W && h_b, "sdfr_decoder_create: NULL argument");
    SDFR_REQUIRE(n_lin >= 2 && n_lin <= SDFR_MAX_LAYERS, "sdfr_decoder_create: n_lin=%d outside [2,%d]", n_lin, SDFR_MAX_LAYERS);
    SDFR_REQUIRE(out_dim[n_lin - 1] == 1, "sdfr_decoder_create: last layer must have out_dim 1 (got %d)", out_dim[n_lin - 1]);
    SDFR_REQUIRE(in_dim[0] == n_inputs && inj_n[0] == 0, "sdfr_decoder_create: layer 0 must consume exactly the input row");
    int width = 0;
    for (int l = 0; l < n_lin; ++l) {
        SDFR_REQUIRE(in_dim[l] > 0 && out_dim[l] > 0 && inj_n[l] >= 0 && inj_off[l] >= 0 && inj_off[l] + inj_n[l] <= n_inputs,
                     "sdfr_decoder_create: bad dims at layer %d", l);
        if (l > 0) SDFR_REQUIRE(in_dim[l] == out_dim[l - 1] + inj_n[l], "sdfr_decoder_create: layer %d in_dim %d != %d + %d", l,
                                in_dim[l], out_dim[l - 1], inj_n[l]);
        width = in_dim[l] > width ? in_dim[l] : width;
        if (l < n_lin - 1) width = out_dim[l] > width ? out_dim[l] : width;
    }
    SDFR_REQUIRE(width <= 512, "sdfr_decoder_create: hidden width %d > 512 unsupported", width);
    const int HP = width <= 128 ? 128 : (width <= 256 ? 256 : 512);
    SdfrDeviceGuard dev_guard(device);
    SDFR_HIP_CHECK(dev_guard.err);

    sdfr_decoder* d = new sdfr_decoder();
    memset(d, 0, sizeof(*d));
    d->device = device; d->n_lin = n_lin; d->n_inputs = n_inputs; d->use_tanh = use_tanh; d->HP = HP;
    MlpParams& P = d->proto;
    P.n_mfma = n_lin - 1; P.n_inputs = n_inputs; P.use_tanh = use_tanh;
    int64_t off_f = 0, off_b = 0, off_h = 0, off_s = 0, off_bh = 0;
    const bool kinj = (n_inputs <= 8) && (HP == 512);
    P.kinj = kinj ? 1 : 0;
    for (int l = 0; l < n_lin; ++l) {
        MlpLayer& L = P.L[l];
        L.in_dim = in_dim[l]; L.out_dim = out_dim[l]; L.inj_n = inj_n[l]; L.inj_off = inj_off[l];
        L.ln = (l < n_lin - 1 && h_ln_w && h_ln_w[l] != nullptr) ? 1 : 0;
        if (L.ln) { SDFR_REQUIRE(h_ln_b && h_ln_b[l], "sdfr_decoder_create: LayerNorm weight without bias at layer %d", l); d->has_ln = 1; }
        L.kp_f = 16 * ((in_dim[l] + 15) / 16); L.kp_b = 16 * ((out_dim[l] + 15) / 16); L.kp_h = 32 * ((in_dim[l] + 31) / 32);
        L.off_f = (int)off_f; L.off_b = (int)off_b; L.off_h = (int)off_h;
        if (kinj && l > 0 && inj_n[l] > 0) L.kp_h = HP + 32;
        L.kp_s = 64 * ((in_dim[l] + 63) / 64); L.off_s = (int)off_s;
        L.kp_bh = 128 * ((out_dim[l] + 127) / 128); L.off_bh = (int)off_bh;
        d->macs += (int64_t)in_dim[l] * out_dim[l];
        if (l < n_lin - 1) { off_f += (int64_t)(L.kp_f / 4) * HP; off_b += (int64_t)(L.kp_b / 4) * HP; off_h += (int64_t)(L.kp_h / 8) * HP;
                             off_s += (int64_t)(L.kp_s / 8) * HP * 2; off_bh += (int64_t)(L.kp_bh / 8) * HP; }
    }
    std::vector<float> Wf((size_t)off_f * 4, 0.f), Wb((size_t)off_b * 4, 0.f), bias((size_t)(n_lin - 1) * HP, 0.f), wl(HP, 0.f);
    std::vector<_Float16> Wh((size_t)off_h * 8, (_Float16)0.f), Ws((size_t)off_s * 8, (_Float16)0.f), Wbh((size_t)off_bh * 8, (_Float16)0.f);
    for (int l = 0; l < n_lin - 1; ++l) {
        const MlpLayer& L = P.L[l];
        const float* W = h_W[l];
        for (int r = 0; r < L.out_dim; ++r)
            for (int k = 0; k < L.in_dim; ++k) {
                const float w = W[(size_t)r * L.in_dim + k];
                Wf[((size_t)L.off_f + (size_t)(k / 4) * HP + r) * 4 + (k % 4)] = w;
                const _Float16 wh = (_Float16)w;
                const int prev_out = l > 0 ? P.L[l - 1].out_dim : 0;
                const int kh = (kinj && l > 0 && L.inj_n > 0 && k >= prev_out) ? HP + L.inj_off + (k - prev_out) : k;
                Wh[((size_t)L.off_h + (size_t)(kh / 8) * HP + r) * 8 + (kh % 8)] = wh;
                const size_t es = ((size_t)L.off_s + ((size_t)(k / 8) * HP + r) * 2) * 8 + (k % 8);
                Ws[es] = wh;
                Ws[es + 8] = (_Float16)((w - (float)wh) * 2048.f);
                Wb[((size_t)L.off_b + (size_t)(r / 4) * HP + k) * 4 + (r % 4)] = w;
                Wbh[((size_t)L.off_bh + (size_t)(r / 8) * HP + k) * 8 + (r % 8)] = wh;
            }
        for (int r = 0; r < L.out_dim; ++r) bias[(size_t)l * HP + r] = h_b[l][r];
    }
    std::vector<float> Wk;
    bool finite = true;
    if (HP == 512 && !d->has_ln) {
        int64_t wk_floats = off_f * 4;
        for (int l = 1; l < n_lin - 1; ++l) wk_floats = std::max(wk_floats, sdfr_kcd_wk_floats((int64_t)P.L[l].off_f * 4));
        Wk.assign((size_t)wk_floats, 0.f);
        for (int l = 0; l < n_lin - 1; ++l) {
            const MlpLayer& L = P.L[l];
            for (int r = 0; r < L.out_dim; ++r)
                for (int k = 0; k < L.in_dim; ++k) {
                    const float w = h_W[l][(size_t)r * L.in_dim + k];
                    finite = finite && std::isfinite(w);
                    Wk[(size_t)L.off_f * 4 + (size_t)k * HP + sdfr_wk_row(r)] = w;
                }
        }
    }
    std::vector<float> Wkj;
    bool kcj_ok = HP == 512 && !d->has_ln && n_lin >= 3;
    for (int l = 1; l < n_lin - 1; ++l) kcj_ok = kcj_ok && in_dim[l] == HP;
    if (kcj_ok) {
        Wkj.assign((size_t)off_b * 4, 0.f);
        for (int l = 0; l < n_lin - 1; ++l) {
            const MlpLayer& L = P.L[l];
            for (int r = 0; r < L.out_dim; ++r)
                for (int k = 0; k < L.in_dim; ++k) Wkj[(size_t)L.off_b * 4 + (size_t)r * HP + sdfr_kcj_col(k)] = h_W[l][(size_t)r * L.in_dim + k];
        }
    }
    for (int k = 0; k < in_dim[n_lin - 1]; ++k) wl[k] = h_W[n_lin - 1][k];
    P.b_last = h_b[n_lin - 1][0];

    SDFR_HIP_CHECK(hipMalloc(&d->d_Wf, Wf.size() * sizeof(float)));
    SDFR_HIP_CHECK(hipMalloc(&d->d_Wb, Wb.size() * sizeof(float)));
    if (d->has_ln) {
        std::vector<float> lg((size_t)(n_lin - 1) * HP, 0.f), lb((size_t)(n_lin - 1) * HP, 0.f);
        for (int l = 0; l < n_lin - 1; ++l)
            if (P.L[l].ln)
                for (int r = 0; r < P.L[l].out_dim; ++r) { lg[(size_t)l * HP + r] = h_ln_w[l][r]; lb[(size_t)l * HP + r] = h_ln_b[l][r]; }
        SDFR_HIP_CHECK(hipMalloc(&d->d_lng, lg.size() * sizeof(float)));
        SDFR_HIP_CHECK(hipMalloc(&d->d_lnb, lb.size() * sizeof(float)));
        SDFR_HIP_CHECK(hipMemcpy(d->d_lng, lg.data(), lg.size() * sizeof(float), hipMemcpyHostToDevice));
        SDFR_HIP_CHECK(hipMemcpy(d->d_lnb, lb.data(), lb.size() * sizeof(float), hipMemcpyHostToDevice));
        P.ln_gamma = d->d_lng; P.ln_beta = d->d_lnb;
    }
    SDFR_HIP_CHECK(hipMalloc(&d->d_Wh, Wh.size() * sizeof(_Float16)));
    SDFR_HIP_CHECK(hipMemcpy(d->d_Wh, Wh.data(), Wh.size() * sizeof(_Float16), hipMemcpyHostToDevice));
    SDFR_HIP_CHECK(hipMalloc(&d->d_Wbh, Wbh.size() * sizeof(_Float16)));
    SDFR_HIP_CHECK(hipMemcpy(d->d_Wbh, Wbh.data(), Wbh.size() * sizeof(_Float16), hipMemcpyHostToDevice));
    SDFR_HIP_CHECK(hipMalloc(&d->d_Ws, Ws.size() * sizeof(_Float16)));
    SDFR_HIP_CHECK(hipMemcpy(d->d_Ws, Ws.data(), Ws.size() * sizeof(_Float16), hipMemcpyHostToDevice));
    SDFR_HIP_CHECK(hipMalloc(&d->d_bias, bias.size() * sizeof(float)));
    SDFR_HIP_CHECK(hipMalloc(&d->d_wlast, wl.size() * sizeof(float)));
    SDFR_HIP_CHECK(hipMemcpy(d->d_Wf, Wf.data(), Wf.size() * sizeof(float), hipMemcpyHostToDevice));
    SDFR_HIP_CHECK(hipMemcpy(d->d_Wb, Wb.data(), Wb.size() * sizeof(float), hipMemcpyHostToDevice));
    SDFR_HIP_CHECK(hipMemcpy(d->d_bias, bias.data(), bias.size() * sizeof(float), hipMemcpyHostToDevice));
    SDFR_HIP_CHECK(hipMemcpy(d->d_wlast, wl.data(), wl.size() * sizeof(float), hipMemcpyHostToDevice));
    if (!Wk.empty()) {
        SDFR_HIP_CHECK(hipMalloc(&d->d_Wk, Wk.size() * sizeof(float)));
        SDFR_HIP_CHECK(hipMemcpy(d->d_Wk, Wk.data(), Wk.size() * sizeof(float), hipMemcpyHostToDevice));
        P.Wk = d->d_Wk;
        P.kcompact = finite ? 1 : 0;
    }
    if (!Wkj.empty()) {
        SDFR_HIP_CHECK(hipMalloc(&d->d_Wkj, Wkj.size() * sizeof(float)));
        SDFR_HIP_CHECK(hipMemcpy(d->d_Wkj, Wkj.data(), Wkj.size() * sizeof(float), hipMemcpyHostToDevice));
        P.Wkj = d->d_Wkj;
        P.jcompact = finite ? 1 : 0;
    }
    P.Wf = d->d_Wf; P.Wb = d->d_Wb; P.Wh = d->d_Wh; P.Ws = d->d_Ws; P.Wbh = d->d_Wbh; P.bias = d->d_bias; P.w_last = d->d_wlast; P.fwd_np = 2;
    *out = d;
    return SDFR_OK;
}

static unsigned long long* g_trace = nullptr;
extern "C" int sdfr_debug_set_trace(void* device_buffer) { g_trace = (unsigned long long*)device_buffer; return SDFR_OK; }
static unsigned long long* g_tile_trace = nullptr;
static int64_t g_tile_trace_cap = 0;
extern "C" int sdfr_debug_set_tile_trace(void* device_buffer, int64_t tiles) {
    g_tile_trace = tiles > 0 ? (unsigned long long*)device_buffer : nullptr;
    g_tile_trace_cap = g_tile_trace ? tiles : 0;
    return SDFR_OK;
}

extern "C" int sdfr_decoder_destroy(sdfr_decoder* d) {
    if (!d) return SDFR_OK;
    void* bufs[] = {d->d_Wf, d->d_Wb, d->d_Wk, d->d_Wkj, d->d_Wh, d->d_Ws, d->d_Wbh, d->d_bias, d->d_wlast, d->d_lng, d->d_lnb, d->ln_ws};
    for (void* b : bufs) (void)hipFree(b);
    delete d;
    return SDFR_OK;
}

extern "C" int64_t sdfr_decoder_macs(const sdfr_decoder* d) { return d ? d->macs : 0; }

static void mask_geometry(int HP, int* ft, int* nt) {
    if (HP == 128) { *ft = 1; *nt = 256; }
    else if (HP == 256) { *ft = 2; *nt = 256; }
    else { *ft = 2; *nt = 512; }
}

extern "C" int64_t sdfr_decoder_mask_words(const sdfr_decoder* d, int64_t n) {
    if (!d || n <= 0) return 0;
    int ft, nt;
    mask_geometry(d->HP, &ft, &nt);
    return ((n + 127) / 128) * 2 * (int64_t)(d->n_lin - 1) * ft * nt;
}

extern "C" int sdfr_mlp_forward(const sdfr_decoder* d, const float* inputs, int64_t n, float* sdf, uint32_t* mask_ws, void* stream) {
    SDFR_REQUIRE(d && inputs && sdf, "sdfr_mlp_forward: NULL argument");
    SDFR_DEVICE_CHECK(d, "sdfr_mlp_forward");
    SDFR_REQUIRE(n >= 0 && n < (int64_t)1 << 31, "sdfr_mlp_forward: n=%lld out of range", (long long)n);
    if (n == 0) return SDFR_OK;
    MlpParams P = d->proto;
    P.inputs = inputs; P.n = n; P.sdf = sdf; P.maskbuf = mask_ws; P.trace = g_trace;
    P.tile_trace = g_tile_trace; P.tile_trace_cap = g_tile_trace_cap;
    const int grid = sdfr_cdiv(n, 64);
    if (d->has_ln) sdfr_launch_ln(P, d->HP, false, grid, 1, (hipStream_t)stream);
    else if (d->HP == 512) sdfr_launch_fwd_f32_512(P, n, mask_ws != nullptr, (hipStream_t)stream);
    else sdfr_launch_small(P, d->HP, mask_ws ? 1 : 0, grid, 1, (hipStream_t)stream);
    SDFR_LAUNCH_CHECK();
    return SDFR_OK;
}

extern "C" int sdfr_grid_tile_order(int D, int32_t* out) {
    SDFR_REQUIRE(out, "sdfr_grid_tile_order: NULL argument");
    SDFR_REQUIRE(D >= 1 && D <= 1024, "sdfr_grid_tile_order: D=%d outside [1,1024]", D);
    int64_t j = 0;
    for (int bx = 0; bx < D; bx += 4)
        for (int by = 0; by < D; by += 4)
            for (int bz = 0; bz < D; bz += 4)
                for (int x = bx; x < bx + 4 && x < D; ++x)
                    for (int y = by; y < by + 4 && y < D; ++y)
                        for (int z = bz; z < bz + 4 && z < D; ++z) out[j++] = (int32_t)(((int64_t)x * D + y) * D + z);
    return SDFR_OK;
}

extern "C" int sdfr_mlp_forward_ordered(const sdfr_decoder* d, const float* inputs, int64_t n, float* sdf, uint32_t* mask_ws, const int32_t* order,
                                        int64_t order_rows, void* stream) {
    SDFR_REQUIRE(d && inputs && sdf && order, "sdfr_mlp_forward_ordered: NULL argument");
    SDFR_REQUIRE(n >= 0 && n < (int64_t)1 << 31, "sdfr_mlp_forward_ordered: n=%lld out of range", (long long)n);
    SDFR_REQUIRE(order_rows > 0, "sdfr_mlp_forward_ordered: order_rows=%lld must be positive", (long long)order_rows);
    SDFR_REQUIRE(n % order_rows == 0, "sdfr_mlp_forward_ordered: n=%lld is not a multiple of order_rows=%lld", (long long)n, (long long)order_rows);
    SDFR_REQUIRE(d->HP == 512 && !d->has_ln, "sdfr_mlp_forward_ordered: needs a float32 decoder of padded width 512 without LayerNorm (this one: %d%s)",
                 d->HP, d->has_ln ? ", LayerNorm" : "");
    SDFR_REQUIRE(!mask_ws || ((n + 127) / 128) * 128 * (int64_t)(d->n_lin - 1) < (int64_t)1 << 31,
                 "sdfr_mlp_forward_ordered: n=%lld rows with masks of %d layers exceed the kernel's line index", (long long)n, d->n_lin - 1);
    SDFR_DEVICE_CHECK(d, "sdfr_mlp_forward_ordered");
    if (n == 0) return SDFR_OK;
    MlpParams P = d->proto;
    P.inputs = inputs; P.n = n; P.sdf = sdf; P.maskbuf = mask_ws; P.trace = g_trace;
    P.tile_trace = g_tile_trace; P.tile_trace_cap = g_tile_trace_cap;
    sdfr_launch_fwd_f32_512_ordered(P, n, order, order_rows, (hipStream_t)stream);
    SDFR_LAUNCH_CHECK();
    return SDFR_OK;
}

extern "C" int64_t sdfr_mlp_balance_bytes(int64_t order_rows) {
    return order_rows > 0 && order_rows < (int64_t)1 << 31 ? sdfr_tb_state_words(order_rows) * 4 : 0;
}

extern "C" int sdfr_mlp_balance_init(void* state, const int32_t* order, int64_t order_rows, void* stream) {
    SDFR_REQUIRE(state && order, "sdfr_mlp_balance_init: NULL argument");
    SDFR_REQUIRE(order_rows > 0 && order_rows < (int64_t)1 << 31, "sdfr_mlp_balance_init: order_rows=%lld out of range", (long long)order_rows);
    int cur = -1;
    hipPointerAttribute_t attr;
    SDFR_HIP_CHECK(hipGetDevice(&cur));
    SDFR_HIP_CHECK(hipPointerGetAttributes(&attr, state));
    SDFR_REQUIRE(attr.type == hipMemoryTypeDevice && attr.device == cur,
                 "sdfr_mlp_balance_init: the state must be device memory of the current device %d (the launch stream's); it is %s of device %d", cur,
                 attr.type == hipMemoryTypeDevice ? "memory" : "not device memory", attr.device);
    sdfr_launch_tile_balance_init((int32_t*)state, order, order_rows, (hipStream_t)stream);
    SDFR_LAUNCH_CHECK();
    return SDFR_OK;
}

extern "C" int sdfr_mlp_forward_balanced(const sdfr_decoder* d, const float* inputs, int64_t n, float* sdf, uint32_t* mask_ws, void* state,
                                         int64_t order_rows, void* stream) {
    SDFR_REQUIRE(d && inputs && sdf && state, "sdfr_mlp_forward_balanced: NULL argument");
    SDFR_REQUIRE(n >= 0 && n < (int64_t)1 << 31, "sdfr_mlp_forward_balanced: n=%lld out of range", (long long)n);
    SDFR_REQUIRE(order_rows > 0, "sdfr_mlp_forward_balanced: order_rows=%lld must be positive", (long long)order_rows);
    SDFR_REQUIRE(n % order_rows == 0, "sdfr_mlp_forward_balanced: n=%lld is not a multiple of order_rows=%lld", (long long)n, (long long)order_rows);
    SDFR_REQUIRE(d->HP == 512 && !d->has_ln, "sdfr_mlp_forward_balanced: needs a float32 decoder of padded width 512 without LayerNorm (this one: %d%s)",
                 d->HP, d->has_ln ? ", LayerNorm" : "");
    SDFR_REQUIRE(!mask_ws || ((n + 127) / 128) * 128 * (int64_t)(d->n_lin - 1) < (int64_t)1 << 31,
                 "sdfr_mlp_forward_balanced: n=%lld rows with masks of %d layers exceed the kernel's line index", (long long)n, d->n_lin - 1);
    SDFR_DEVICE_CHECK(d, "sdfr_mlp_forward_balanced");
    if (n == 0) return SDFR_OK;
    int32_t* st = (int32_t*)state;
    const bool ranked = sdfr_tb_ranked(order_rows);
    MlpParams P = d->proto;
    P.inputs = inputs; P.n = n; P.sdf = sdf; P.maskbuf = mask_ws; P.trace = g_trace;
    P.tile_trace = g_tile_trace; P.tile_trace_cap = g_tile_trace_cap;
    P.tile_cost = ranked ? st + sdfr_tb_cost_word(order_rows) : nullptr;
    P.tile_at = st + sdfr_tb_at_word(order_rows);
    sdfr_launch_fwd_f32_512_ordered(P, n, st + sdfr_tb_order_word(order_rows), order_rows, (hipStream_t)stream);
    SDFR_LAUNCH_CHECK();
    if (ranked) {
        sdfr_launch_tile_balance(st, order_rows, (hipStream_t)stream);
        SDFR_LAUNCH_CHECK();
    }
    return SDFR_OK;
}

#ifndef SDFR_COUNTED_TILE16_ROWS
#define SDFR_COUNTED_TILE16_ROWS 4096
#endif
extern "C" int sdfr_mlp_forward_counted(const sdfr_decoder* d, const float* inputs, int64_t n_max, const int32_t* n_dev, float* sdf, int half,
                                        void* stream) {
    SDFR_REQUIRE(d && inputs && sdf && n_dev, "sdfr_mlp_forward_counted: NULL argument");
    SDFR_DEVICE_CHECK(d, "sdfr_mlp_forward_counted");
    SDFR_REQUIRE(n_max >= 0 && n_max < (int64_t)1 << 31, "sdfr_mlp_forward_counted: n_max=%lld out of range", (long long)n_max);
    SDFR_REQUIRE(!half || (d->HP == 512 && !d->has_ln), "sdfr_mlp_forward_counted: half operands need a 512-wide decoder without LayerNorm");
    if (n_max == 0) return SDFR_OK;
    MlpParams P = d->proto;
    P.inputs = inputs; P.n = n_max; P.sdf = sdf; P.maskbuf = nullptr; P.n_dev = n_dev; P.trace = g_trace;
    hipStream_t s = (hipStream_t)stream;
    if (half & 2) {
        const int mid = 64 * 256 + 1;
        P.n_dev_lo = mid; P.n_dev_hi = 0x7fffffff;
        if (n_max >= mid) sdfr_launch_fwd_f16_512(P, n_max, false, s);
        P.n_dev_lo = 0; P.n_dev_hi = mid;
        sdfr_launch_fwd_f16_512_tile64(P, n_max < mid ? n_max : (int64_t)mid, s);
    } else if (half) {
        P.n_dev_lo = SDFR_COUNTED_TILE16_ROWS; P.n_dev_hi = 0x7fffffff;
        if (n_max >= SDFR_COUNTED_TILE16_ROWS) sdfr_launch_fwd_f16_512(P, n_max, false, s);
        P.n_dev_lo = 0; P.n_dev_hi = SDFR_COUNTED_TILE16_ROWS;
        sdfr_launch_fwd_f16_512_tile16(P, n_max < SDFR_COUNTED_TILE16_ROWS ? n_max : (int64_t)SDFR_COUNTED_TILE16_ROWS, s);
    } else if (d->has_ln) sdfr_launch_ln(P, d->HP, false, sdfr_cdiv(n_max, 64), 1, s);
    else if (d->HP == 512) {
        P.n_dev_lo = SDFR_COUNTED_TILE16_ROWS; P.n_dev_hi = 0x7fffffff;
        if (n_max >= SDFR_COUNTED_TILE16_ROWS) sdfr_launch_fwd_f32_512(P, n_max, false, s);
        P.n_dev_lo = 0; P.n_dev_hi = SDFR_COUNTED_TILE16_ROWS;
        sdfr_launch_fwd_f32_512_tile16(P, n_max < SDFR_COUNTED_TILE16_ROWS ? n_max : (int64_t)SDFR_COUNTED_TILE16_ROWS, s);
    } else sdfr_launch_small(P, d->HP, 0, sdfr_cdiv(n_max, 64), 1, s);
    SDFR_LAUNCH_CHECK();
    return SDFR_OK;
}

extern "C" int sdfr_mlp_forward_f16_counted(const sdfr_decoder* d, const float* inputs, int64_t n_max, const int32_t* n_dev, float* sdf,
                                            uint32_t* mask_ws, void* stream) {
    SDFR_REQUIRE(d && inputs && sdf && n_dev, "sdfr_mlp_forward_f16_counted: NULL argument");
    SDFR_DEVICE_CHECK(d, "sdfr_mlp_forward_f16_counted");
    SDFR_REQUIRE(n_max >= 0 && n_max < (int64_t)1 << 31, "sdfr_mlp_forward_f16_counted: n_max=%lld out of range", (long long)n_max);
    SDFR_REQUIRE(d->HP == 512 && !d->has_ln, "sdfr_mlp_forward_f16_counted: half operands need a 512-wide decoder without LayerNorm");
    if (n_max == 0) return SDFR_OK;
    MlpParams P = d->proto;
    P.inputs = inputs; P.n = n_max; P.sdf = sdf; P.maskbuf = mask_ws; P.n_dev = n_dev; P.n_dev_lo = 0; P.n_dev_hi = 0; P.trace = nullptr;
    sdfr_launch_fwd_f16_512(P, n_max, mask_ws != nullptr, (hipStream_t)stream);
    SDFR_LAUNCH_CHECK();
    return SDFR_OK;
}

extern "C" int sdfr_mlp_forward_f16(const sdfr_decoder* d, const float* inputs, int64_t n, float* sdf, uint32_t* mask_ws, void* stream) {
    SDFR_REQUIRE(d && inputs && sdf, "sdfr_mlp_forward_f16: NULL argument");
    SDFR_DEVICE_CHECK(d, "sdfr_mlp_forward_f16");
    SDFR_REQUIRE(n >= 0 && n < (int64_t)1 << 31, "sdfr_mlp_forward_f16: n=%lld out of range", (long long)n);
    SDFR_REQUIRE(d->HP == 512, "sdfr_mlp_forward_f16: built for hidden widths 257..512 (padded width %d)", d->HP);
    SDFR_REQUIRE(!d->has_ln, "sdfr_mlp_forward_f16: LayerNorm decoders run in float32");
    if (n == 0) return SDFR_OK;
    MlpParams P = d->proto;
    P.inputs = inputs; P.n = n; P.sdf = sdf; P.maskbuf = mask_ws; P.trace = g_trace;
    sdfr_launch_fwd_f16_512(P, n, mask_ws != nullptr, (hipStream_t)stream);
    SDFR_LAUNCH_CHECK();
    return SDFR_OK;
}

extern "C" int sdfr_mlp_forward_skip(const sdfr_decoder* d, const float* inputs, int64_t n, float* sdf, const int32_t* skip, int64_t rows_per_crop,
                                     void* stream) {
    SDFR_REQUIRE(d && inputs && sdf && skip && rows_per_crop > 0, "sdfr_mlp_forward_skip: bad argument");
    SDFR_DEVICE_CHECK(d, "sdfr_mlp_forward_skip");
    SDFR_REQUIRE(n >= 0 && n < (int64_t)1 << 31, "sdfr_mlp_forward_skip: n=%lld out of range", (long long)n);
    SDFR_REQUIRE(d->HP == 512 && !d->has_ln, "sdfr_mlp_forward_skip: 512-wide decoders without LayerNorm");
    if (n == 0) return SDFR_OK;
    MlpParams P = d->proto;
    P.inputs = inputs; P.n = n; P.sdf = sdf; P.maskbuf = nullptr; P.skip = skip; P.skip_rows = rows_per_crop;
    P.n_crops = (int)((n + rows_per_crop - 1) / rows_per_crop);
    sdfr_launch_pool_f32_skip(P, n, (hipStream_t)stream);
    SDFR_LAUNCH_CHECK();
    return SDFR_OK;
}

extern "C" int sdfr_mlp_forward_ragged(const sdfr_decoder* d, const float* inputs, int B, int64_t rows_per_crop, const int32_t* cnt, float* sdf,
                                       uint32_t* mask_ws, int half_tiles, void* stream) {
    SDFR_REQUIRE(d && inputs && sdf && cnt, "sdfr_mlp_forward_ragged: NULL argument");
    SDFR_DEVICE_CHECK(d, "sdfr_mlp_forward_ragged");
    SDFR_REQUIRE(B >= 0 && rows_per_crop >= 0 && rows_per_crop % 64 == 0 && (int64_t)B * rows_per_crop < (int64_t)1 << 31,
                 "sdfr_mlp_forward_ragged: B=%d rows_per_crop=%lld (a multiple of 64, B * rows < 2^31)", B, (long long)rows_per_crop);
    SDFR_REQUIRE(d->HP == 512 && !d->has_ln, "sdfr_mlp_forward_ragged: 512-wide decoders without LayerNorm");
    if (B == 0 || rows_per_crop == 0) return SDFR_OK;
    MlpParams P = d->proto;
    P.inputs = inputs; P.n = (int64_t)B * rows_per_crop; P.sdf = sdf; P.maskbuf = mask_ws; P.crop_cnt = cnt; P.crop_rows = rows_per_crop; P.trace = nullptr;
    if (half_tiles) { sdfr_set_error("sdfr_mlp_forward_ragged: half_tiles is a float16 option (sdfr_mlp_forward_f16_ragged)"); return SDFR_E_UNSUPPORTED; }
    P.n_crops = B;
    sdfr_launch_pool_f32_ragged(P, P.n, false, (hipStream_t)stream);
    SDFR_LAUNCH_CHECK();
    return SDFR_OK;
}

extern "C" int sdfr_mlp_forward_f16_ragged(const sdfr_decoder* d, const float* inputs, int B, int64_t rows_per_crop, const int32_t* cnt, float* sdf,
                                           uint32_t* mask_ws, int half_tiles, void* stream) {
    SDFR_REQUIRE(d && inputs && sdf && cnt, "sdfr_mlp_forward_f16_ragged: NULL argument");
    SDFR_DEVICE_CHECK(d, "sdfr_mlp_forward_f16_ragged");
    SDFR_REQUIRE(B >= 0 && rows_per_crop >= 0 && rows_per_crop % 128 == 0 && (int64_t)B * rows_per_crop < (int64_t)1 << 31,
                 "sdfr_mlp_forward_f16_ragged: B=%d rows_per_crop=%lld (a multiple of 128, B * rows < 2^31)", B, (long long)rows_per_crop);
    SDFR_REQUIRE(d->HP == 512 && !d->has_ln, "sdfr_mlp_forward_f16_ragged: half operands need a 512-wide decoder without LayerNorm");
    if (B == 0 || rows_per_crop == 0) return SDFR_OK;
    MlpParams P = d->proto;
    P.inputs = inputs; P.n = (int64_t)B * rows_per_crop; P.sdf = sdf; P.maskbuf = mask_ws; P.crop_cnt = cnt; P.crop_rows = rows_per_crop; P.trace = nullptr;
    P.n_crops = B;
    if (half_tiles) sdfr_launch_pool_f16_ragged_half_tiles(P, P.n, false, (hipStream_t)stream);
    else sdfr_launch_pool_f16_ragged(P, P.n, false, (hipStream_t)stream);
    SDFR_LAUNCH_CHECK();
    return SDFR_OK;
}

extern "C" int sdfr_mlp_forward_candidates(const sdfr_decoder* d, const float* inputs, int64_t rows_per_crop_in, int B, const int32_t* cidx,
                                           int64_t stride, const int32_t* cnt, float* sdf, uint32_t* mask_ws, int half, int half_tiles,
                                           void* stream) {
    SDFR_REQUIRE(d && inputs && cidx && cnt && sdf, "sdfr_mlp_forward_candidates: NULL argument");
    SDFR_DEVICE_CHECK(d, "sdfr_mlp_forward_candidates");
    const int tile = half ? (half_tiles == 2 ? 32 : (half_tiles ? 64 : 128)) : 64;
    SDFR_REQUIRE(B >= 0 && stride >= 0 && stride % tile == 0 && (int64_t)B * stride < (int64_t)1 << 31 && rows_per_crop_in > 0 &&
                 (int64_t)B * rows_per_crop_in < (int64_t)1 << 31, "sdfr_mlp_forward_candidates: B=%d stride=%lld (a multiple of %d) rows_per_crop_in=%lld",
                 B, (long long)stride, tile, (long long)rows_per_crop_in);
    SDFR_REQUIRE(d->HP == 512 && !d->has_ln, "sdfr_mlp_forward_candidates: 512-wide decoders without LayerNorm");
    SDFR_REQUIRE(half || !half_tiles, "sdfr_mlp_forward_candidates: half_tiles is a float16 option");
    if (B == 0 || stride == 0) return SDFR_OK;
    MlpParams P = d->proto;
    P.inputs = inputs; P.n = (int64_t)B * stride; P.sdf = sdf; P.maskbuf = mask_ws; P.crop_cnt = cnt; P.crop_rows = stride; P.trace = nullptr;
    P.gather_idx = cidx; P.gather_rows = rows_per_crop_in; P.n_crops = B;
    if (!half) sdfr_launch_pool_f32_ragged(P, P.n, true, (hipStream_t)stream);
    else if (half_tiles == 2) sdfr_launch_pool_f16_ragged_quarter_tiles(P, P.n, (hipStream_t)stream);
    else if (half_tiles) sdfr_launch_pool_f16_ragged_half_tiles(P, P.n, true, (hipStream_t)stream);
    else sdfr_launch_pool_f16_ragged(P, P.n, true, (hipStream_t)stream);
    SDFR_LAUNCH_CHECK();
    return SDFR_OK;
}

extern "C" int sdfr_mlp_forward_f16_skip(const sdfr_decoder* d, const float* inputs, int64_t n, float* sdf, const int32_t* skip,
                                         int64_t rows_per_crop, void* stream) {
    SDFR_REQUIRE(d && inputs && sdf && skip && rows_per_crop > 0, "sdfr_mlp_forward_f16_skip: bad argument");
    SDFR_DEVICE_CHECK(d, "sdfr_mlp_forward_f16_skip");
    SDFR_REQUIRE(n >= 0 && n < (int64_t)1 << 31, "sdfr_mlp_forward_f16_skip: n=%lld out of range", (long long)n);
    SDFR_REQUIRE(d->HP == 512 && !d->has_ln, "sdfr_mlp_forward_f16_skip: 512-wide decoders without LayerNorm");
    if (n == 0) return SDFR_OK;
    MlpParams P = d->proto;
    P.inputs = inputs; P.n = n; P.sdf = sdf; P.maskbuf = nullptr; P.skip = skip; P.skip_rows = rows_per_crop;
    P.n_crops = (int)((n + rows_per_crop - 1) / rows_per_crop);
    sdfr_launch_pool_f16_skip(P, n, (hipStream_t)stream);
    SDFR_LAUNCH_CHECK();
    return SDFR_OK;
}

extern "C" int sdfr_mlp_forward_split(const sdfr_decoder* d, const float* inputs, int64_t n, float* sdf, uint32_t* mask_ws, void* stream) {
// ... 72 lines not shown
```

### sdflabel_amd/csrc/mlp_balance.hip

```cpp
#include <hip/hip_runtime.h>
#include "sdfr_common.h"
#include "tile_balance.h"

constexpr int TB_NT = 256, TB_WAVES = TB_NT / 64;

__global__ __launch_bounds__(256) void sdfr_tile_balance_init_kernel(int32_t* __restrict__ state, const int32_t* __restrict__ order, int64_t order_rows) {
    const int64_t i = (int64_t)blockIdx.x * blockDim.x + threadIdx.x;
    const int64_t T = sdfr_tb_chunks(order_rows);
    if (i < 3 * T + SDFR_TB_CTL) state[i] = (i < 2 * T || i >= 3 * T) ? 0 : (int32_t)(i - 2 * T);
    if (i < order_rows) {
        const int32_t o = order[i];
        state[sdfr_tb_order_word(order_rows) + i] = o;
        state[sdfr_tb_fixed_word(order_rows) + i] = o;
    }
}

__global__ __launch_bounds__(TB_NT) void sdfr_tile_balance_kernel(int32_t* __restrict__ state, int64_t order_rows) {
    __shared__ int32_t cost[SDFR_TB_MAX_CHUNKS];
    __shared__ int last_reader;
    const int T = (int)sdfr_tb_chunks(order_rows), full = (int)sdfr_tb_full_chunks(order_rows);
    int32_t* g_cost = state + sdfr_tb_cost_word(order_rows);
    int32_t* g_last = state + sdfr_tb_last_word(order_rows);
    int32_t* g_at = state + sdfr_tb_at_word(order_rows);
    int32_t* ctl = state + sdfr_tb_ctl_word(order_rows);
    int32_t* order = state + sdfr_tb_order_word(order_rows);
    const int32_t* fixed = state + sdfr_tb_fixed_word(order_rows);
    const int tid = threadIdx.x, lane = tid & 63, wave = tid >> 6;
    const int c = (int)blockIdx.x * TB_WAVES + wave;
    const int64_t i = (int64_t)c * SDFR_TB_CHUNK + lane;
    const bool moves = c < T && i < order_rows;
    const int32_t entry = moves ? fixed[i] : 0;
    for (int k = tid; k < T; k += TB_NT) cost[k] = g_cost[k];
    __syncthreads();
    if (c < T) {
        int r = c;
        if (c < full) {
            r = sdfr_tb_rank_part(cost, full, c, lane, 64);
#pragma unroll
            for (int d = 32; d >= 1; d >>= 1) r += __shfl_xor(r, d, 64);
        }
        if (lane == 0) {
            g_last[c] = cost[c];
            g_at[r] = c;
        }
        if (moves) order[sdfr_tb_dest(c, r, lane, full)] = entry;
    }
    if (tid == 0) last_reader = atomicAdd(ctl, 1) == (int)gridDim.x - 1 ? 1 : 0;
    __syncthreads();
    if (last_reader) {
        for (int k = tid; k < T; k += TB_NT) g_cost[k] = 0;
        if (tid == 0) ctl[0] = 0;
    }
}

void sdfr_launch_tile_balance_init(int32_t* state, const int32_t* order, int64_t order_rows, hipStream_t s) {
    const int64_t head = 3 * sdfr_tb_chunks(order_rows) + SDFR_TB_CTL, n = order_rows > head ? order_rows : head;
    hipLaunchKernelGGL(sdfr_tile_balance_init_kernel, dim3(sdfr_cdiv(n, 256)), dim3(256), 0, s, state, order, order_rows);
}

void sdfr_launch_tile_balance(int32_t* state, int64_t order_rows, hipStream_t s) {
    hipLaunchKernelGGL(sdfr_tile_balance_kernel, dim3(sdfr_cdiv(sdfr_tb_chunks(order_rows), TB_WAVES)), dim3(TB_NT), 0, s, state, order_rows);
}
```

### sdflabel_amd/csrc/mlp_jac.hip

```cpp
#include "mlp_kernel.h"
#ifndef SDFR_JAC_MS
#define SDFR_JAC_MS 32
#define SDFR_JAC_FT 4
#define SDFR_JAC_NP 1
#define SDFR_JAC_NW 4
#define SDFR_JAC_PF 2
#endif
#ifndef SDFR_JAC_SMALL_FT
#define SDFR_JAC_SMALL_FT 8
#define SDFR_JAC_SMALL_NW 4
#define SDFR_JAC_SMALL_PF 4
#endif
#ifndef SDFR_JAC_SWITCH_ROWS
#define SDFR_JAC_SWITCH_ROWS 8
#endif
void sdfr_launch_jac_f32_512_recompute32(const MlpParams& P, int cap, int B, hipStream_t s) {
    hipLaunchKernelGGL((sdfr_mlp_kernel<float, 32, 4, 1, 4, 2, 2>), dim3(sdfr_cdiv(cap, 32), B), dim3(256), 0, s, P);
}

#include <stdlib.h>
static int jac_pool_crops() {
    static const int v = [] { const char* e = getenv("SDFR_JAC_POOL_CROPS"); return e ? atoi(e) : 12; }();
    return v;
}
void sdfr_launch_jac_f32_512(const MlpParams& P, int cap, int B, bool from_masks, hipStream_t s) {
    static_assert(SDFR_JAC_MS * SDFR_JAC_FT * SDFR_JAC_NW == 512 && 16 * SDFR_JAC_SMALL_FT * SDFR_JAC_SMALL_NW == 512, "padded width 512 = MS * FT * NW");
    if (!from_masks) {
        hipLaunchKernelGGL((sdfr_mlp_kernel<float, 16, 8, 1, 4, 4, 2>), dim3(sdfr_cdiv(cap, 16), B), dim3(256), 0, s, P);
    } else if (B >= jac_pool_crops() && B <= 64 && P.n_crops == B) {
        const int64_t tiles = (int64_t)sdfr_cdiv(cap, SDFR_JAC_MS * SDFR_JAC_NP) * B;
        hipLaunchKernelGGL((sdfr_mlp_kernel<float, SDFR_JAC_MS, SDFR_JAC_FT, SDFR_JAC_NP, SDFR_JAC_NW, SDFR_JAC_PF, 3, 0, false, 2>),
                           dim3((unsigned)(tiles < 512 ? tiles : 512)), dim3(64 * SDFR_JAC_NW), 0, s, P);
    } else if (B >= SDFR_JAC_SWITCH_ROWS) {
        hipLaunchKernelGGL((sdfr_mlp_kernel<float, SDFR_JAC_MS, SDFR_JAC_FT, SDFR_JAC_NP, SDFR_JAC_NW, SDFR_JAC_PF, 3>),
                           dim3(sdfr_cdiv(cap, SDFR_JAC_MS * SDFR_JAC_NP), B), dim3(64 * SDFR_JAC_NW), 0, s, P);
    } else {
        MlpParams Q = P;
        const char* e = getenv("SDFR_JAC_COMPACT");
        if (e && e[0] == '0') Q.jcompact = 0;
        hipLaunchKernelGGL((sdfr_mlp_kernel<float, 16, SDFR_JAC_SMALL_FT, 1, SDFR_JAC_SMALL_NW, SDFR_JAC_SMALL_PF, 3>), dim3(sdfr_cdiv(cap, 16), B),
                           dim3(64 * SDFR_JAC_SMALL_NW), 0, s, Q);
    }
}

void sdfr_launch_fwd_f32_512_tile16(const MlpParams& P, int64_t n, hipStream_t s) {
    hipLaunchKernelGGL((sdfr_mlp_kernel<float, 16, SDFR_JAC_SMALL_FT, 1, SDFR_JAC_SMALL_NW, SDFR_JAC_SMALL_PF, 0>), dim3(sdfr_cdiv(n, 16)),
                       dim3(64 * SDFR_JAC_SMALL_NW), 0, s, P);
}

void sdfr_launch_tail_f32_512(const MlpParams& P, int64_t n_rays, int spec_k, hipStream_t s) {
    const dim3 grid(sdfr_cdiv(n_rays, P.t_rt));
    if (spec_k > 1)
        hipLaunchKernelGGL((sdfr_mlp_kernel<float, 16, SDFR_JAC_SMALL_FT, 4, SDFR_JAC_SMALL_NW, 2, 4>), grid, dim3(64 * SDFR_JAC_SMALL_NW), 0, s, P);
    else
        hipLaunchKernelGGL((sdfr_mlp_kernel<float, 16, SDFR_JAC_SMALL_FT, 1, SDFR_JAC_SMALL_NW, SDFR_JAC_SMALL_PF, 4>), grid, dim3(64 * SDFR_JAC_SMALL_NW), 0,
                           s, P);
}
```

### sdflabel_amd/csrc/mlp_kernel.h

```cpp
#pragma once
#include "sdfr_common.h"
#include "kc_slots.h"
#include "kcj_slots.h"
#include "tile_balance.h"
#include <math.h>
#include <type_traits>

typedef float f32x16 __attribute__((ext_vector_type(16)));
typedef float f32x4 __attribute__((ext_vector_type(4)));
typedef _Float16 h16;
typedef h16 h16x8 __attribute__((ext_vector_type(8)));
typedef h16 h16x4 __attribute__((ext_vector_type(4)));

struct MlpLayer {
    int in_dim, out_dim;
    int inj_n, inj_off;
    int kp_f, kp_b, kp_h;
    int off_f, off_b, off_h;
    int kp_bh, off_bh;
    int kp_s, off_s;
    int ln;
};

struct MlpParams {
    const float4* Wf;
    const float4* Wb;
    const void* Wh;
    const void* Wbh;
    const void* Ws;
    const float* Wk;
    int kcompact;
    int kinj;
    int fwd_np;
    const float* bias;
    const float* ln_gamma;
    const float* ln_beta;
    float4* ln_ws;
    const float* w_last;
    float b_last;
    int n_mfma;
    int n_inputs;
    int use_tanh;
    MlpLayer L[SDFR_MAX_LAYERS];
    const float* inputs;
    int64_t n;
    float* sdf;
    int64_t rows_per_crop;
    const int32_t* idx;
    const int32_t* cnt;
    int cap;
    float* J;
    float* sdf_sel;
    const float* sdf_in;
    uint32_t* maskbuf;
    const int32_t* skip;
    int64_t skip_rows;
    const int32_t* crop_cnt;
    int64_t crop_rows;
    const int32_t* gather_idx;
    int64_t gather_rows;
    int n_crops;
    const int32_t* n_dev;
    int n_dev_lo, n_dev_hi;
    unsigned long long* trace;
    float* t_rows;
    int t_rt;
    const float* t_latn;
    const int32_t* t_pix;
    const float4* t_lam;
    int t_step0;
    int t_nlv;
    int t_lv_from[SDFR_TRACE_LEVELS], t_lv_k[SDFR_TRACE_LEVELS];
    float t_qmax;
    int32_t* t_tile_ctr;
    int t_stage;
    int32_t* t_next_cnt;
    int32_t* t_next_pix;
    float4* t_next_lam;
    const float* t_far;
    const float* t_pose;
    const float* t_Kinv;
    float* t_hit_lam;
    float* t_hit_sdf;
    int t_W, t_H, t_steps;
    const int32_t* t_wh; int t_PS;
    float t_eps, t_sigma;
    unsigned long long* t_evals;
    int32_t* t_unresolved;
    const float* Wkj;
    int jcompact;
    int32_t* tile_cost;
    const int32_t* tile_at;
    unsigned long long* tile_trace;
    int64_t tile_trace_cap;
};
#define SDFR_TILE_TRACE_WORDS 6

struct sdfr_decoder {
    int device;
    int n_lin, n_inputs, use_tanh, HP;
    float4* d_Wf;
    float4* d_Wb;
    float* d_Wk;
    float* d_Wkj;
    void* d_Wh;
    void* d_Ws;
    void* d_Wbh;
    float* d_lng;
    float* d_lnb;
    int has_ln;
    mutable float4* ln_ws;
    mutable size_t ln_ws_bytes;
    float* d_bias;
    float* d_wlast;
    int64_t macs;
    MlpParams proto;
};

__device__ __forceinline__ float f4c(const float4& v, int i) { return i == 0 ? v.x : (i == 1 ? v.y : (i == 2 ? v.z : v.w)); }

template <typename ET, int MS> struct Mma;
template <> struct Mma<float, 32> {
    typedef f32x16 acc_t; typedef float4 vec_t;
    static constexpr int KV = 4, NSTEP = 4;
    static __device__ __forceinline__ acc_t step(const vec_t& a, const vec_t& b, acc_t c, int ks) {
        return __builtin_amdgcn_mfma_f32_32x32x2f32(f4c(a, ks), f4c(b, ks), c, 0, 0, 0);
    }
};
template <> struct Mma<float, 16> {
    typedef f32x4 acc_t; typedef float4 vec_t;
    static constexpr int KV = 4, NSTEP = 4;
    static __device__ __forceinline__ acc_t step(const vec_t& a, const vec_t& b, acc_t c, int ks) {
        return __builtin_amdgcn_mfma_f32_16x16x4f32(f4c(a, ks), f4c(b, ks), c, 0, 0, 0);
    }
};
template <> struct Mma<h16, 32> {
    typedef f32x16 acc_t; typedef h16x8 vec_t;
    static constexpr int KV = 8, NSTEP = 1;
    static __device__ __forceinline__ acc_t step(const vec_t& a, const vec_t& b, acc_t c, int) {
#ifdef SDFR_ABL_NOMFMA
        c[0] += (float)a[0] * (float)b[0];
        return c;
#else
        return __builtin_amdgcn_mfma_f32_32x32x16_f16(a, b, c, 0, 0, 0);
#endif
    }
};
template <> struct Mma<h16, 16> {
    typedef f32x4 acc_t; typedef h16x8 vec_t;
    static constexpr int KV = 8, NSTEP = 1;
    static __device__ __forceinline__ acc_t step(const vec_t& a, const vec_t& b, acc_t c, int) {
        return __builtin_amdgcn_mfma_f32_16x16x32_f16(a, b, c, 0, 0, 0);
    }
};
__device__ __forceinline__ void store4(float* dst, const float* v) { *reinterpret_cast<float4*>(dst) = make_float4(v[0], v[1], v[2], v[3]); }
__device__ __forceinline__ void store4(h16* dst, const float* v) {
// ... 1006 lines not shown
                    mb[off + 2 * f] = (uint16_t)(mw[fi >> 1] >> ((fi & 1) * 16));
                }
            }
            }
        }
        SDFR_STAMP(l, 3);
        __syncthreads();
        if (DBUF) { vec_t* t_ = act; act = actw; actw = t_; ET* e_ = act_e; act_e = actw_e; actw_e = e_; }
        SDFR_STAMP(l, 4);
    }

    if (GMASK) {
        if (tid < PT) {
            const float o = P.sdf_in[rows[tid]];
            gy[tid] = 1.f - o * o;
            if (tid < n_valid && P.sdf_sel) P.sdf_sel[slots[tid]] = o;
        }
    } else {
        constexpr int SL = HALF ? (NT / PT < 4 ? NT / PT : 4) : NT / PT;
        static_assert(!KC || (SL == 8 && KG / SL * KV == 64), "exact-f32 grid forward: last linear in 8 slices of 64 k");
        static_assert(SL * PT <= NT, "last linear: one thread per (slice, point)");
        constexpr int KGS = KG / SL;
        const int sl = tid / PT, pt = tid - sl * PT;
        float s = 0.f;
        if (sl < SL) {
            const float* wl = P.w_last + sl * KGS * KV;
            const vec_t* a4 = act + (sl * KGS) * PT + pt;
#pragma unroll 4
            for (int g = 0; g < KGS; ++g) {
                const vec_t a = a4[g * PT];
#pragma unroll
                for (int i = 0; i < KV; ++i) s = fmaf((float)a[i], wl[g * KV + i], s);
            }
        }
        red[tid] = s;
        __syncthreads();
        if (tid < PT) {
            float y = 0.f;
#pragma unroll
            for (int q = 0; q < SL; ++q) y += red[q * PT + tid];
            if (KGX > KG && P.kinj) {
                const MlpLayer Ll = P.L[P.n_mfma];
                for (int c = 0; c < Ll.inj_n; ++c) {
                    const int kc = Ll.inj_off + c;
                    y = fmaf((float)act_e[((KG + kc / KV) * PT + tid) * KV + (kc % KV)], P.w_last[P.L[P.n_mfma - 1].out_dim + c], y);
                }
            }
            y += P.b_last;
            const float y1 = P.use_tanh ? tanhf(y) : y;
            const float o = tanhf(y1);
            if (JAC) {
                float g = 1.f - o * o;
                if (P.use_tanh) g *= (1.f - y1 * y1);
                gy[tid] = g;
                if (tid < n_valid && P.sdf_sel) P.sdf_sel[slots[tid]] = o;
            } else if (TAIL) {
                const int k = pass_k(P.t_step0 + t_pass);
                const unsigned long long live = __ballot(t_act && tid < RT);
                if (tid == 0) t_ev += (unsigned long long)(__popcll(live) * k);
                {
                    const int li = tid < RT ? tid : 0;
                    float vj = o, rj = fabsf(o), pj = t_st.x, prev = t_st.y;
                    bool done = rj < P.t_eps, ishit = done;
                    float pc = t_st.x, qp = t_st.z, vp = o;
                    for (int j = 1; j < k; ++j) {
                        const float vc = __shfl(o, li + RT * j, 64);
                        const float pn = pc + ((P.t_sigma * qp) * t_st.y) / t_idn;
                        qp = qp * t_st.z;
                        const float rp = fabsf(vp);
                        const bool cov = ((pn - pc) * t_idn <= rp) && (vp > 0.f) && (pn > pc);
                        const bool take = cov && !done;
                        done = done || !cov;
                        if (take) {
                            prev = rp; vj = vc; rj = fabsf(vc); pj = pn;
                            if (rj < P.t_eps) { ishit = true; done = true; }
                        }
                        pc = pn; vp = vc;
                    }
                  if (t_act && tid < RT) {
                    if (ishit) {
                        P.t_hit_lam[t_gp] = pj;
                        P.t_hit_sdf[t_gp] = vj;
                        t_act = false;
                    } else {
                        const float qn = (prev > 0.f) ? fminf(fmaxf(rj / prev, 0.5f), P.t_qmax) : 1.f;
                        const float l2 = pj + vj / t_idn;
                        t_st.y = rj; t_st.z = qn;
                        if ((l2 < t_farl) && (vj == vj)) t_st.x = l2;
                        else t_act = false;
                    }
                  }
                }
            } else if constexpr (ORDER) {
                const int row = slots[tid];
                if (row >= 0 && (!P.skip || !P.skip[row / P.skip_rows])) P.sdf[row] = o;
                if (P.tile_cost && tid == 0) {
                    const int place = sdfr_tb_place_of_tile(tile, P.gather_rows);
                    atomicAdd(P.tile_cost + sdfr_tb_cost_index(P.tile_at[place], place, P.gather_rows), rows[127]);
                }
            } else {
                if (tid < n_valid) {
                    const int64_t row = (int64_t)tile * PT + tid;
                    if (!P.skip || !P.skip[row / P.skip_rows]) P.sdf[row] = o;
                }
            }
        }
    }
#ifdef SDFR_MLP_TRACE
    if (tt_on) {
        unsigned long long* tt = P.tile_trace + (int64_t)blockIdx.x * SDFR_TILE_TRACE_WORDS;
        tt[2] = __builtin_amdgcn_s_memtime();
        tt[3] = __builtin_amdgcn_s_memrealtime();
    }
#endif
    if constexpr (TAIL) {
        --t_left;
        if (tid == 0) *t_more = 0;
        __syncthreads();
        if (t_act && t_left > 0) *t_more = 1;
        __syncthreads();
        if (*t_more == 0) break;
        ++t_pass;
        tail_rows(pass_k(P.t_step0 + t_pass), false);
        __syncthreads();
        build_operand();
        __syncthreads();
    }
    } while (TAIL);
    if constexpr (TAIL) {
        if (tid < 64) {
            const unsigned long long left_over = __ballot(t_act && tid < RT);
            const bool hand_over = P.t_next_cnt && (P.t_stage < P.t_steps);
            int base = 0;
            if (tid == 0) {
                if (P.t_evals) atomicAdd(P.t_evals, t_ev);
                if (left_over && !hand_over && P.t_unresolved) atomicAdd(P.t_unresolved, (int)__popcll(left_over));
                if (left_over && hand_over) base = atomicAdd(P.t_next_cnt, (int)__popcll(left_over));
            }
            if (hand_over && left_over) {
                base = __shfl(base, 0, 64);
                if (t_act && tid < RT) {
                    const int at = base + (int)__popcll(left_over & ((1ull << tid) - 1ull));
                    P.t_next_pix[at] = t_gp;
                    P.t_next_lam[at] = t_st;
                }
            }
        }
        if (!P.t_tile_ctr) return;
        continue;
    }
    if constexpr (JAC) {
    uint32_t raw[NP * FT * RG];
    const bool kcj_on = KCJ && P.jcompact && P.Wkj;
    uint32_t kcj_w[4] = {0u, 0u, 0u, 0u};
    int kcj_n = 0;
    auto kcj_vote = [&](int l, const uint32_t* raw) {
        const int prev_out = P.L[l - 1].out_dim;
        uint32_t m = 0u;
#pragma unroll
        for (int f = 0; f < FT; ++f) m |= ((raw[f] >> sdfr_mask_shift(fbase + f * MS + 4 * lg)) & 0xFu) << (4 * f);
        if (__builtin_amdgcn_readfirstlane((int)(fbase + MS * FT > prev_out)) != 0) {
            uint32_t keep = 0u;
#pragma unroll
            for (int f = 0; f < FT; ++f) {
                const int nv = min(max(prev_out - (fbase + f * MS + 4 * lg), 0), 4);
                keep |= ((1u << nv) - 1u) << (4 * f);
            }
            m &= keep;
        }
        int x = (int)m;
        x |= __builtin_amdgcn_update_dpp(0, x, 0xB1, 0xf, 0xf, false);
        x |= __builtin_amdgcn_update_dpp(0, x, 0x4E, 0xf, 0xf, false);
        x |= __builtin_amdgcn_update_dpp(0, x, 0x124, 0xf, 0xf, false);
        x |= __builtin_amdgcn_update_dpp(0, x, 0x128, 0xf, 0xf, false);
#pragma unroll
        for (int g = 0; g < 4; ++g) kcj_w[g] = (uint32_t)__builtin_amdgcn_readlane(x, 16 * g);
        if (lane == 0) reinterpret_cast<int*>(kcj_cnt4)[wave] = sdfr_kcj_count(kcj_w[0], kcj_w[1], kcj_w[2], kcj_w[3]);
    };
    const bool kcj_top = kcj_on && P.n_mfma >= 2;
    if constexpr (KCJ) {
        if (kcj_top) {
            const int r = rows[lp];
#pragma unroll
            for (int f = 0; f < FT; ++f) raw[f] = P.maskbuf[sdfr_mask_dword(r, P.n_mfma - 1, P.n_mfma, HP / 32, fbase + f * MS + 4 * lg)];
            kcj_vote(P.n_mfma, raw);
        }
    }
    __syncthreads();
    SDFR_STAMP(8, 2);

    auto mask_addr = [&](int j, int r, int l, int& shift) -> int64_t {
        shift = sdfr_mask_shift(j);
        return sdfr_mask_dword(r, l - 1, P.n_mfma, HP / 32, j);
    };
    auto fetch_masks = [&](int l, uint32_t* raw) {
#pragma unroll
        for (int p = 0; p < NP; ++p) {
            const int r = rows[p * MS + lp];
#pragma unroll
            for (int f = 0; f < FT; ++f)
#pragma unroll
                for (int rg = 0; rg < RG; ++rg) {
                    int shift;
                    raw[(p * FT + f) * RG + rg] = P.maskbuf[mask_addr(feat0(f, rg), r, l, shift)];
                }
        }
    };
    auto store_in_grad = [&](int l, const uint32_t* raw, auto&& value) {
        const MlpLayer L = P.L[l];
        const int prev_out = P.L[l - 1].out_dim;
        const int inj_hi = prev_out + L.inj_n;
        if constexpr (MLDS) {
            const uint2* mst = reinterpret_cast<const uint2*>(mlds) + ((int64_t)wave * SDFR_MAX_LAYERS + (l - 1)) * PT;
            const int msh = (lg & 1) * 16 + (lg >> 1) * 4;
            uint32_t mk[NP][2];
#pragma unroll
            for (int p = 0; p < NP; ++p) {
                const uint2 m2 = mst[p * MS + lp];
                mk[p][0] = m2.x >> msh; mk[p][1] = m2.y >> msh;
            }
#pragma unroll
            for (int f = 0; f < FT; ++f) {
                const int j0 = feat0(f, 0);
                const bool tail_f = __builtin_amdgcn_readfirstlane((int)(fbase + (f + 1) * MS > prev_out)) != 0;
#pragma unroll
                for (int p = 0; p < NP; ++p) {
                    const int pt = p * MS + lp;
                    float v[4];
#pragma unroll
                    for (int i = 0; i < 4; ++i) {
                        const float x = value(f, p, 0, i, j0 + i, pt);
                        const int m = __builtin_amdgcn_sbfe((int)mk[p][f >> 1], (f & 1) * 8 + i, 1);
                        v[i] = __int_as_float(__float_as_int(x) & m);
                    }
                    if (tail_f) {
#pragma unroll
                        for (int i = 0; i < 4; ++i) {
                            const int k = j0 + i;
                            if (k >= prev_out) {
                                if (k < inj_hi) {
                                    if (jdir) jinj[pt * 8 + L.inj_off + (k - prev_out)] += value(f, p, 0, i, k, pt);
                                    else if (slots[pt] >= 0) atomicAdd(P.J + (int64_t)slots[pt] * NI + L.inj_off + (k - prev_out), value(f, p, 0, i, k, pt));
                                }
                                v[i] = 0.f;
                            }
                        }
                    }
                    store4(act_e + ((j0 / KV) * PT + pt) * KV + (j0 % KV), v);
                }
            }
            return;
        }
        uint32_t mw[MW];
        if (GMASK) {
#pragma unroll
            for (int w = 0; w < MW; ++w) mw[w] = 0u;
#pragma unroll
            for (int p = 0; p < NP; ++p) {
                const int r = rows[p * MS + lp];
#pragma unroll
                for (int f = 0; f < FT; ++f)
#pragma unroll
                    for (int rg = 0; rg < RG; ++rg) {
                        int shift;
                        (void)mask_addr(feat0(f, rg), r, l, shift);
                        const uint32_t nib = (raw[(p * FT + f) * RG + rg] >> shift) & 0xFu;
                        const int bit = ((f * NP + p) * RG + rg) * 4;
                        mw[bit >> 5] |= nib << (bit & 31);
                    }
            }
        } else {
#pragma unroll
            for (int w = 0; w < MW; ++w) mw[w] = masks[((l - 1) * MW + w) * NT + tid];
        }
        const bool tail_here = __builtin_amdgcn_readfirstlane((int)(fbase + MS * FT > prev_out)) != 0;
        auto apply_masks = [&](auto tail_tag) {
            constexpr bool TAIL = decltype(tail_tag)::value;
#pragma unroll
            for (int f = 0; f < FT; ++f)
#pragma unroll
                for (int rg = 0; rg < RG; ++rg) {
                    const int j0 = feat0(f, rg);
#pragma unroll
                    for (int p = 0; p < NP; ++p) {
                        const int pt = p * MS + lp;
#pragma unroll
                        for (int i = 0; i < 4; ++i) {
                            const int k = j0 + i;
                            const int bit = ((f * NP + p) * RG + rg) * 4 + i;
                            float x = value(f, p, rg, i, k, pt);
                            if (!TAIL || k < prev_out) {
                                x = ((mw[bit >> 5] >> (bit & 31)) & 1u) ? x : 0.f;
                            } else {
                                if (k < inj_hi && slots[pt] >= 0)
                                    atomicAdd(P.J + (int64_t)slots[pt] * NI + L.inj_off + (k - prev_out), x);
                                x = 0.f;
                            }
                            acc[f][p][rg * 4 + i] = x;
                        }
                    }
                }
        };
        if (tail_here) apply_masks(std::true_type{});
        else apply_masks(std::false_type{});
        if constexpr (LN) {
            if (P.L[l - 1].ln) {
                const float* gam = P.ln_gamma + (l - 1) * HP;
                const float4* xh4 = P.ln_ws + ((wg_lin * P.n_mfma + (l - 1)) * (HP / 4)) * PT;
                float s1[NP], s2[NP];
#pragma unroll
                for (int p = 0; p < NP; ++p) { s1[p] = 0.f; s2[p] = 0.f; }
#pragma unroll
                for (int f = 0; f < FT; ++f)
#pragma unroll
                    for (int rg = 0; rg < RG; ++rg) {
                        const int j0 = feat0(f, rg);
#pragma unroll
                        for (int p = 0; p < NP; ++p) {
                            const float4 xh = xh4[(j0 >> 2) * PT + p * MS + lp];
#pragma unroll
                            for (int i = 0; i < 4; ++i) {
                                const int k = j0 + i;
                                const float gh = (k < prev_out) ? acc[f][p][rg * 4 + i] * gam[k] : 0.f;
                                acc[f][p][rg * 4 + i] = gh;
                                s1[p] += gh;
                                s2[p] += gh * f4c(xh, i);
                            }
                        }
                    }
                point_sums(s1);
                point_sums(s2);
#pragma unroll
                for (int f = 0; f < FT; ++f)
#pragma unroll
                    for (int rg = 0; rg < RG; ++rg) {
                        const int j0 = feat0(f, rg);
#pragma unroll
                        for (int p = 0; p < NP; ++p) {
                            const float4 xh = xh4[(j0 >> 2) * PT + p * MS + lp];
                            const float rs = lnrstd[(l - 1) * PT + p * MS + lp];
                            const float m1 = s1[p] / (float)prev_out, m2 = s2[p] / (float)prev_out;
#pragma unroll
                            for (int i = 0; i < 4; ++i)
                                acc[f][p][rg * 4 + i] = (j0 + i < prev_out) ? rs * (acc[f][p][rg * 4 + i] - m1 - f4c(xh, i) * m2) : 0.f;
                        }
                    }
            }
        }
        if constexpr (KCJ) {
            if (kcj_on && l >= 2) {
                const int4 c4 = kcj_cnt4[0];
                const int c[4] = {c4.x, c4.y, c4.z, c4.w};
                int off = 0, tot = 0;
#pragma unroll
                for (int w = 0; w < 4; ++w) {
                    off += w < wave ? c[w] : 0;
                    tot += c[w];
                }
                off = __builtin_amdgcn_readfirstlane(off);
                tot = __builtin_amdgcn_readfirstlane(tot);
                const uint32_t mine = lg == 0 ? kcj_w[0] : lg == 1 ? kcj_w[1] : lg == 2 ? kcj_w[2] : kcj_w[3];
                int n = off;
#pragma unroll
                for (int q = 0; q < 32; ++q) {
                    const int b0 = (int)((kcj_w[0] >> q) & 1u), b1 = (int)((kcj_w[1] >> q) & 1u), b2 = (int)((kcj_w[2] >> q) & 1u),
                              b3 = (int)((kcj_w[3] >> q) & 1u);
                    const int front = ((b0 << 2) | ((b0 + b1) << 4) | ((b0 + b1 + b2) << 6)) >> (2 * lg) & 3;
                    if ((mine >> q) & 1u) act_e[sdfr_kcj_elem(n + front, lp)] = acc[q >> 2][0][q & 3];
                    n += b0 + b1 + b2 + b3;
                }
#pragma unroll
                for (int h = 0; h < 2; ++h) {
                    const int q = lp + 16 * h;
                    if ((mine >> q) & 1u)
                        reinterpret_cast<int*>(kcj_list4)[sdfr_kcj_kidx(off + sdfr_kcj_rank(kcj_w[0], kcj_w[1], kcj_w[2], kcj_w[3], q, lg))] =
                            (fbase + sdfr_kcj_feature(q, lg)) * HP;
                }
                const int padded = sdfr_kcj_padded(tot);
                for (int e = tid; e < (padded - tot) * PT; e += NT) {
                    const int pos = sdfr_kcj_pad_pos(tot, e);
                    act_e[sdfr_kcj_elem(pos, sdfr_kcj_pad_point(e))] = 0.f;
                    if (sdfr_kcj_pad_point(e) == 0) reinterpret_cast<int*>(kcj_list4)[sdfr_kcj_kidx(pos)] = 0;
                }
                kcj_n = padded;
                return;
            }
        }
#pragma unroll
        for (int f = 0; f < FT; ++f)
#pragma unroll
            for (int rg = 0; rg < RG; ++rg) {
                const int j0 = feat0(f, rg);
#pragma unroll
                for (int p = 0; p < NP; ++p) {
                    float v[4];
#pragma unroll
                    for (int i = 0; i < 4; ++i) v[i] = acc[f][p][rg * 4 + i];
                    store4(act_e + ((j0 / KV) * PT + p * MS + lp) * KV + (j0 % KV), v);
                }
            }
    };

    if (GMASK && !MLDS && !kcj_top) fetch_masks(P.n_mfma, raw);
    SDFR_STAMP(8, 3);
    if constexpr (MLDS) {
        if (P.n_mfma >= 1 && !(P.n_mfma - 1 == 0 && P.L[0].in_dim <= 8))
            preload_a(reinterpret_cast<const vec_t*>(P.Wbh) + P.L[P.n_mfma - 1].off_bh);
        float4 wl[FT];
        float gyp[NP];
#pragma unroll
        for (int f = 0; f < FT; ++f) wl[f] = *reinterpret_cast<const float4*>(P.w_last + feat0(f, 0));
#pragma unroll
        for (int p = 0; p < NP; ++p) gyp[p] = gy[p * MS + lp];
        store_in_grad(P.n_mfma, raw, [&](int f, int p, int, int i, int, int) { return f4c(wl[f], i) * gyp[p]; });
    } else
    store_in_grad(P.n_mfma, raw, [&](int, int, int, int, int k, int pt) { return P.w_last[k] * gy[pt]; });
    __syncthreads();
    SDFR_STAMP(8, 4);
    for (int l = P.n_mfma - 1; l >= 0; --l) {
        const MlpLayer L = P.L[l];
        if constexpr (MLDS) {
          if (l == 0 && L.in_dim <= 8) {
            constexpr int TPW = (HP / KT) / NW;
            const vec_t* Wl = reinterpret_cast<const vec_t*>(P.Wbh) + L.off_bh;
            const int nkt = L.kp_bh / KT;
            acc_t a0[NP];
            vec_t av[TPW], bv[TPW][NP];
            SDFR_STAMP(9, 0);
#pragma unroll
            for (int u = 0; u < TPW; ++u) {
                const int t = wave * TPW + u;
#pragma unroll
                for (int i = 0; i < KV; ++i) av[u][i] = (ET)0;
                if (t < nkt) av[u] = Wl[(int64_t)(t * NLG + lg) * HP + lp];
#pragma unroll
                for (int p = 0; p < NP; ++p) bv[u][p] = act[(t * NLG + lg) * PT + p * MS + lp];
            }
#pragma unroll
            for (int p = 0; p < NP; ++p) {
#pragma unroll
                for (int r = 0; r < 4; ++r) a0[p][r] = 0.f;
#pragma unroll
                for (int u = 0; u < TPW; ++u) a0[p] = M::step(av[u], bv[u][p], a0[p], 0);
            }
            SDFR_STAMP(9, 1);
            float* part = reinterpret_cast<float*>(mlds);
            if (lg < 2) {
#pragma unroll
                for (int p = 0; p < NP; ++p)
                    *reinterpret_cast<float4*>(part + ((wave * PT + p * MS + lp) * 8 + 4 * lg)) = make_float4(a0[p][0], a0[p][1], a0[p][2], a0[p][3]);
            }
            __syncthreads();
            for (int e = tid; e < 8 * PT; e += NT) {
                const int q = e >> 3, k = e & 7;
                float t = 0.f;
#pragma unroll
                for (int w = 0; w < NW; ++w) t += part[(w * PT + q) * 8 + k];
                if (k < NI && slots[q] >= 0) {
                    if (k >= L.in_dim) t = 0.f;
                    if (jdir) P.J[(int64_t)slots[q] * NI + k] = jinj[q * 8 + k] + t;
                    else atomicAdd(P.J + (int64_t)slots[q] * NI + k, t);
                }
            }
            SDFR_STAMP(9, 2);
            break;
          }
        }
        if (!MLDS && l == 0 && L.in_dim <= 8) {
            constexpr int TPP = NT / PT;
            constexpr int PMIN = (HP == 512) ? (HALF ? 32 : 16) : 1;
            constexpr int PARTS = (TPP < PMIN) ? PMIN : TPP, PPT = PARTS / TPP, JS = HP / PARTS;
            static_assert(NT % PT == 0 && HP % PARTS == 0 && PARTS % TPP == 0 && PARTS * 8 * PT * 4 <= KG * PT * 16,
                          "first-layer reduction scratch fits the operand tile");
            const int pt = tid % PT, t0 = (PT % 64 == 0) ? __builtin_amdgcn_readfirstlane(tid / PT) : tid / PT;
            const float4* W0 = P.Wf + L.off_f;
            float s8[PPT][8];
            SDFR_STAMP(9, 0);
#pragma unroll
            for (int q = 0; q < PPT; ++q) {
                const int part = t0 * PPT + q;
#pragma unroll
                for (int k = 0; k < 8; ++k) s8[q][k] = 0.f;
#pragma unroll 8
                for (int jj = 0; jj < JS; ++jj) {
                    const int j = part * JS + jj;
                    const float g = (float)act_e[((j / KV) * PT + pt) * KV + (j % KV)];
                    float4 wa, wb;
                    if constexpr (PT % 64 == 0) {
                        typedef const f32x4 __attribute__((address_space(4))) * cf4p;
                        const cf4p W0c = (cf4p)(uintptr_t)W0;
                        const f32x4 va = W0c[j];
                        f32x4 vb = {0.f, 0.f, 0.f, 0.f};
                        if (L.kp_f > 4) vb = W0c[HP + j];
                        wa = make_float4(va[0], va[1], va[2], va[3]);
                        wb = make_float4(vb[0], vb[1], vb[2], vb[3]);
                    } else {
                        wa = W0[j];
                        wb = (L.kp_f > 4) ? W0[HP + j] : make_float4(0.f, 0.f, 0.f, 0.f);
                    }
                    s8[q][0] = fmaf(wa.x, g, s8[q][0]); s8[q][1] = fmaf(wa.y, g, s8[q][1]); s8[q][2] = fmaf(wa.z, g, s8[q][2]); s8[q][3] = fmaf(wa.w, g, s8[q][3]);
                    s8[q][4] = fmaf(wb.x, g, s8[q][4]); s8[q][5] = fmaf(wb.y, g, s8[q][5]); s8[q][6] = fmaf(wb.z, g, s8[q][6]); s8[q][7] = fmaf(wb.w, g, s8[q][7]);
                }
            }
            SDFR_STAMP(9, 1);
            __syncthreads();
            float* scr = reinterpret_cast<float*>(lds4);
#pragma unroll
            for (int q = 0; q < PPT; ++q)
#pragma unroll
                for (int k = 0; k < 8; ++k) scr[((t0 * PPT + q) * 8 + k) * PT + pt] = s8[q][k];
            __syncthreads();
            for (int e = tid; e < 8 * PT; e += NT) {
                const int k = e / PT, q = e % PT;
                float t = 0.f;
                for (int r = 0; r < PARTS; ++r) t += scr[(r * 8 + k) * PT + q];
                if (k < NI && k < L.in_dim && slots[q] >= 0) atomicAdd(P.J + (int64_t)slots[q] * NI + k, t);
            }
            SDFR_STAMP(9, 2);
            break;
        }
        SDFR_STAMP(l, 0);
        if (GMASK && !MLDS && l > 0) fetch_masks(l, raw);
// ... 73 lines not shown
```

Before: 56.36 million rays/s.

## Fuse tile-balance ranking into band-select launch and add branch-free Jacobian compaction

Adds a new band-select kernel that computes each point's rank with a block-parallel prefix count over earlier rows. Its grid also carries the tile-balance ranking blocks, so the separate balance launch after the balanced forward is deferred into the band-select launch, removing one kernel launch per step. The Jacobian kernel's compaction path also gains a mode that precomputes per-group chain words. It then writes compacted activations without a serial per-bit running count, sending inactive lanes to a dead slot. Risks are redundant prefix reads of earlier rows in each band block, and extra writes to the dead position.

```diff
diff --git a/include/sdfr.h b/include/sdfr.h
--- a/include/sdfr.h
+++ b/include/sdfr.h
@@ -16,7 +16,7 @@
 #define SDFR_TRACE_LEVELS 6
 #define SDFR_TRACE_COUNTERS 32
 
-#define SDFR_VERSION 421
+#define SDFR_VERSION 422
 
 int sdfr_version(void);
 int sdfr_build_flags(void);
@@ -40,6 +40,8 @@
 int sdfr_mlp_balance_init(void* state, const int32_t* order, int64_t order_rows, void* stream);
 int sdfr_mlp_forward_balanced(const sdfr_decoder* dec, const float* inputs, int64_t n, float* sdf, uint32_t* mask_ws, void* state,
                               int64_t order_rows, void* stream);
+int sdfr_mlp_forward_balanced_deferred(const sdfr_decoder* dec, const float* inputs, int64_t n, float* sdf, uint32_t* mask_ws, void* state,
+                                       int64_t order_rows, void* stream);
 int sdfr_mlp_forward_f16(const sdfr_decoder* dec, const float* inputs, int64_t n, float* sdf, uint32_t* mask_ws, void* stream);
 
 int sdfr_mlp_forward_f16_counted(const sdfr_decoder* dec, const float* inputs, int64_t n_max, const int32_t* n_dev, float* sdf, uint32_t* mask_ws,
@@ -210,6 +212,9 @@
                      int max_reuse, int32_t* reuse, int32_t* n_full, void* stream);
 int sdfr_band_select_ex(const float* sdf, int64_t G, int B, float thr, const float* thr_extra, const int32_t* skip, int32_t* idx, int cap,
                         int32_t* cnt, int32_t* slot, int32_t* scratch, int32_t* over, int over_bit, void* stream);
+int sdfr_band_select_rank(const float* sdf, int64_t G, int B, float thr, const float* thr_extra, const int32_t* skip, int32_t* idx, int cap,
+                          int32_t* cnt, int32_t* slot, int32_t* over, int over_bit, void* balance_state, int64_t order_rows, void* stream);
+int64_t sdfr_band_select_rank_max_rows(void);
 int sdfr_mlp_forward_candidates(const sdfr_decoder* d, const float* inputs, int64_t rows_per_crop_in, int B, const int32_t* cidx, int64_t stride,
                                 const int32_t* cnt, float* sdf, uint32_t* mask_ws, int half, int half_tiles, void* stream);
 int sdfr_candidate_band(float* sdf_grid, const float* csdf, const int32_t* cidx, int64_t G, int B, int stride, const int32_t* ccnt, float thr,
diff --git a/sdflabel_amd/_lib.py b/sdflabel_amd/_lib.py
--- a/sdflabel_amd/_lib.py
+++ b/sdflabel_amd/_lib.py
@@ -5,7 +5,7 @@
 _HERE = os.path.dirname(os.path.abspath(__file__))
 LIB_PATH = os.environ.get("SDFR_LIB") or os.path.join(_HERE, "lib", "libsdfr_hip.so")
 
-ABI_VERSION = 421
+ABI_VERSION = 422
 _lib = None
 
 _PROTOS = {
@@ -76,6 +76,7 @@
     "sdfr_mlp_balance_bytes": (c_int64, [c_int64]),
     "sdfr_mlp_balance_init": (c_int, [c_void_p, c_void_p, c_int64, c_void_p]),
     "sdfr_mlp_forward_balanced": (c_int, [c_void_p, c_void_p, c_int64, c_void_p, c_void_p, c_void_p, c_int64, c_void_p]),
+    "sdfr_mlp_forward_balanced_deferred": (c_int, [c_void_p, c_void_p, c_int64, c_void_p, c_void_p, c_void_p, c_int64, c_void_p]),
     "sdfr_mlp_forward_f16": (c_int, [c_void_p, c_void_p, c_int64, c_void_p, c_void_p, c_void_p]),
     "sdfr_mlp_forward_f16_counted": (c_int, [c_void_p, c_void_p, c_int64, c_void_p, c_void_p, c_void_p, c_void_p]),
     "sdfr_mlp_forward_split": (c_int, [c_void_p, c_void_p, c_int64, c_void_p, c_void_p, c_void_p]),
@@ -148,6 +149,9 @@
                                  c_void_p, c_void_p, c_void_p, c_int, c_void_p, c_void_p, c_void_p]),
     "sdfr_band_select_ex": (c_int, [c_void_p, c_int64, c_int, c_float, c_void_p, c_void_p, c_void_p, c_int, c_void_p, c_void_p, c_void_p, c_void_p,
                                     c_int, c_void_p]),
+    "sdfr_band_select_rank": (c_int, [c_void_p, c_int64, c_int, c_float, c_void_p, c_void_p, c_void_p, c_int, c_void_p, c_void_p, c_void_p, c_int,
+                                      c_void_p, c_int64, c_void_p]),
+    "sdfr_band_select_rank_max_rows": (c_int64, []),
     "sdfr_mlp_forward_candidates": (c_int, [c_void_p, c_void_p, c_int64, c_int, c_void_p, c_int64, c_void_p, c_void_p, c_void_p, c_int, c_int,
                                             c_void_p]),
     "sdfr_candidate_band": (c_int, [c_void_p, c_void_p, c_void_p, c_int64, c_int, c_int, c_void_p, c_float, c_void_p, c_int, c_void_p, c_void_p,
diff --git a/sdflabel_amd/batch.py b/sdflabel_amd/batch.py
--- a/sdflabel_amd/batch.py
+++ b/sdflabel_amd/batch.py
@@ -43,6 +43,7 @@
             self.fwd_balance = torch.empty(int(lib.sdfr_mlp_balance_bytes(self.G)) // 4, dtype=torch.int32, device=dev)
             with _lib.guard(dev):
                 ck(lib.sdfr_mlp_balance_init(P(self.fwd_balance), P(self.fwd_order), self.G, _lib.stream_ptr()), "sdfr_mlp_balance_init")
+            self.band_rank_max_rows = int(lib.sdfr_band_select_rank_max_rows())
         self.cap = int(cap) if cap is not None else max(256, self.G // 8)
         self._init_extents(K, max_pixels, max_side)
         self._alloc_common()
@@ -309,7 +310,12 @@
     def _decoder_plain(self, L, st, mlp_events, events):
         B, G, cap = self.B, self.G, self.cap
         fwd = L.sdfr_mlp_forward_f16 if self.f16 else (L.sdfr_mlp_forward_split if self.split else L.sdfr_mlp_forward)
-        if self.fwd_order is not None and os.environ.get("SDFR_FWD_ORDER", "1") != "0" and os.environ.get("SDFR_FWD_BALANCE", "1") != "0":
+        balanced = self.fwd_order is not None and os.environ.get("SDFR_FWD_ORDER", "1") != "0" and os.environ.get("SDFR_FWD_BALANCE", "1") != "0"
+        rank_fused = balanced and B * G <= self.band_rank_max_rows and os.environ.get("SDFR_BAND_FUSED", "1") != "0"
+        if rank_fused:
+            ck(L.sdfr_mlp_forward_balanced_deferred(self.handle.h, P(self.inputs), B * G, P(self.sdf), P(self.mask_ws), P(self.fwd_balance), G, st),
+               "sdfr_mlp_forward_balanced_deferred")
+        elif balanced:
             ck(L.sdfr_mlp_forward_balanced(self.handle.h, P(self.inputs), B * G, P(self.sdf), P(self.mask_ws), P(self.fwd_balance), G, st),
                "sdfr_mlp_forward_balanced")
         elif self.fwd_order is not None and os.environ.get("SDFR_FWD_ORDER", "1") != "0":
@@ -319,8 +325,12 @@
             ck(fwd(self.handle.h, P(self.inputs), B * G, P(self.sdf), P(self.mask_ws), st), fwd.__name__)
         if mlp_events is not None:
             mlp_events[1].record()
-        ck(L.sdfr_band_select_ex(P(self.sdf), G, B, self.thr, None, None, P(self.idx), cap, P(self.cnt), None, P(self.scratch), P(self.over), 1, st),
-           "sdfr_band_select_ex")
+        if rank_fused:
+            ck(L.sdfr_band_select_rank(P(self.sdf), G, B, self.thr, None, None, P(self.idx), cap, P(self.cnt), None, P(self.over), 1,
+                                       P(self.fwd_balance), G, st), "sdfr_band_select_rank")
+        else:
+            ck(L.sdfr_band_select_ex(P(self.sdf), G, B, self.thr, None, None, P(self.idx), cap, P(self.cnt), None, P(self.scratch), P(self.over), 1,
+                                     st), "sdfr_band_select_ex")
         if "jacobian" in events:
             events["jacobian"][0].record()
         ck(L.sdfr_mlp_jacobian(self.handle.h, P(self.inputs), G, B, P(self.idx), cap, P(self.cnt), P(self.J), P(self.sdf_band), P(self.sdf),
diff --git a/sdflabel_amd/csrc/band_rank.hip b/sdflabel_amd/csrc/band_rank.hip
--- /dev/null
+++ b/sdflabel_amd/csrc/band_rank.hip
@@ -0,0 +1,105 @@
+#include "sdfr_common.h"
+#include "tile_balance_rank.h"
+
+constexpr int SDFR_BR_NT = 1024, SDFR_BR_WAVES = SDFR_BR_NT / 64;
+constexpr int SDFR_BR_ROWS = SDFR_BR_NT;
+constexpr int SDFR_BR_FLY = 8;
+
+__device__ __forceinline__ int sdfr_br_in(float v, float thr) { return fabsf(v) < thr ? 1 : 0; }
+
+__global__ __launch_bounds__(SDFR_BR_NT) void sdfr_band_rank_kernel(const float* __restrict__ sdf, int64_t G, int B, float thr,
+                                                                  const float* __restrict__ thr_extra, const int32_t* __restrict__ skip,
+                                                                  int32_t* __restrict__ idx, int cap, int32_t* __restrict__ cnt,
+                                                                  int32_t* __restrict__ slot, int32_t* __restrict__ over, int over_bit, int nblk,
+                                                                  int nsel, int32_t* __restrict__ state, int64_t order_rows, int nrank) {
+    const int bid = (int)blockIdx.x;
+    if (bid >= nsel) {
+        sdfr_tb_rank_block<SDFR_BR_NT>(state, order_rows, bid - nsel, nrank);
+        return;
+    }
+    const int tid = threadIdx.x, lane = tid & 63, wv = tid >> 6;
+    if (G == 0) {
+        for (int b = tid; b < B; b += SDFR_BR_NT) cnt[b] = 0;
+        return;
+    }
+    const int b = bid / nblk, blk = nblk - 1 - bid % nblk;
+    if (skip && skip[b]) return;
+    if (thr_extra) thr += thr_extra[b];
+    const float* __restrict__ p = sdf + (int64_t)b * G;
+    const int64_t r0 = (int64_t)blk * SDFR_BR_ROWS;
+    const int64_t g = r0 + tid;
+    const bool in = g < G && sdfr_br_in(p[g], thr);
+    int front = 0;
+    int64_t head = (int64_t)((4u - (uint32_t)((uintptr_t)p >> 2)) & 3u);
+    if (head > r0) head = r0;
+    if (tid < head) front += sdfr_br_in(p[tid], thr);
+    const float4* __restrict__ p4 = reinterpret_cast<const float4*>(p + head);
+    const int nv = (int)((r0 - head) >> 2);
+    for (int i0 = 0; i0 < nv; i0 += SDFR_BR_NT * SDFR_BR_FLY) {
+        float4 q[SDFR_BR_FLY];
+#pragma unroll
+        for (int u = 0; u < SDFR_BR_FLY; ++u) {
+            const int i = i0 + u * SDFR_BR_NT + tid;
+            q[u] = p4[i < nv ? i : nv - 1];
+        }
+#pragma unroll
+        for (int u = 0; u < SDFR_BR_FLY; ++u) {
+            const int c = sdfr_br_in(q[u].x, thr) + sdfr_br_in(q[u].y, thr) + sdfr_br_in(q[u].z, thr) + sdfr_br_in(q[u].w, thr);
+            front += i0 + u * SDFR_BR_NT + tid < nv ? c : 0;
+        }
+    }
+    const int64_t tail = head + 4 * (int64_t)nv;
+    if (tail + tid < r0) front += sdfr_br_in(p[tail + tid], thr);
+#pragma unroll
+    for (int d = 32; d >= 1; d >>= 1) front += __shfl_xor(front, d, 64);
+    __shared__ int wfront[SDFR_BR_WAVES];
+    __shared__ int wc[SDFR_BR_WAVES];
+    const unsigned long long bal = __ballot(in);
+    if (lane == 0) {
+        wc[wv] = __popcll(bal);
+        wfront[wv] = front;
+    }
+    __syncthreads();
+    int base = 0, woff = 0, tot = 0;
+#pragma unroll
+    for (int w = 0; w < SDFR_BR_WAVES; ++w) {
+        const int c = wc[w];
+        base += wfront[w];
+        woff += w < wv ? c : 0;
+        tot += c;
+    }
+    const int rank = base + woff + __popcll(bal & ((1ull << lane) - 1ull));
+    if (g < G) {
+        int sl = -1;
+        if (in && rank < cap) {
+            idx[(int64_t)b * cap + rank] = (int32_t)g;
+            sl = rank;
+        }
+        if (slot) slot[(int64_t)b * G + g] = sl;
+    }
+    if (blk == nblk - 1 && tid == 0) {
+        cnt[b] = base + tot;
+        if (over && base + tot > cap) atomicOr(&over[b], over_bit);
+    }
+}
+
+#define SDFR_BAND_RANK_MAX_ROWS ((int64_t)256000)
+extern "C" int64_t sdfr_band_select_rank_max_rows(void) { return SDFR_BAND_RANK_MAX_ROWS; }
+
+extern "C" int sdfr_band_select_rank(const float* sdf, int64_t G, int B, float thr, const float* thr_extra, const int32_t* skip, int32_t* idx,
+                                     int cap, int32_t* cnt, int32_t* slot, int32_t* over, int over_bit, void* balance_state, int64_t order_rows,
+                                     void* stream) {
+    SDFR_REQUIRE(sdf && idx && cnt, "sdfr_band_select_rank: NULL argument");
+    SDFR_REQUIRE(G >= 0 && B >= 0 && cap >= 0, "sdfr_band_select_rank: negative size");
+    SDFR_REQUIRE(!balance_state || (order_rows > 0 && order_rows < (int64_t)1 << 31), "sdfr_band_select_rank: order_rows=%lld out of range",
+                 (long long)order_rows);
+    const int64_t nblk = G > 0 ? (G + SDFR_BR_ROWS - 1) / SDFR_BR_ROWS : 1;
+    const int64_t nsel = B == 0 ? 0 : (G > 0 ? nblk * B : 1);
+    const int nrank = balance_state && sdfr_tb_ranked(order_rows) ? sdfr_tb_rank_blocks(order_rows, SDFR_BR_NT) : 0;
+    SDFR_REQUIRE(nsel + nrank < (int64_t)1 << 31, "sdfr_band_select_rank: G=%lld rows of B=%d crops exceed one launch", (long long)G, B);
+    if (nsel + nrank == 0) return SDFR_OK;
+    hipLaunchKernelGGL(sdfr_band_rank_kernel, dim3((unsigned)(nsel + nrank)), dim3(SDFR_BR_NT), 0, (hipStream_t)stream, sdf, G, B, thr, thr_extra, skip,
+                       idx, cap, cnt, slot, over, over_bit, (int)nblk, (int)nsel, (int32_t*)balance_state, order_rows, nrank);
+    SDFR_LAUNCH_CHECK();
+    return SDFR_OK;
+}
diff --git a/sdflabel_amd/csrc/kcjd_slots.h b/sdflabel_amd/csrc/kcjd_slots.h
--- /dev/null
+++ b/sdflabel_amd/csrc/kcjd_slots.h
@@ -0,0 +1,24 @@
+#pragma once
+#include "kcj_slots.h"
+
+SDFR_KCJ_HD uint32_t sdfr_kcjd_spread8(uint32_t byte) {
+    uint32_t s = byte & 0xFFu;
+    s = (s | (s << 12)) & 0x000F000Fu;
+    s = (s | (s << 6)) & 0x03030303u;
+    s = (s | (s << 3)) & 0x11111111u;
+    return s;
+}
+SDFR_KCJ_HD uint32_t sdfr_kcjd_group_part(uint32_t w, int j, int g) { return sdfr_kcjd_spread8(w >> (8 * j)) << g; }
+SDFR_KCJ_HD uint32_t sdfr_kcjd_chain_word(uint32_t w0, uint32_t w1, uint32_t w2, uint32_t w3, int j) {
+    return sdfr_kcjd_group_part(w0, j, 0) | sdfr_kcjd_group_part(w1, j, 1) | sdfr_kcjd_group_part(w2, j, 2) | sdfr_kcjd_group_part(w3, j, 3);
+}
+SDFR_KCJ_HD int sdfr_kcjd_rank_in_word(uint32_t word, int front, int q, int g) {
+    const int bit = 4 * (q & 7) + g;
+    return front + sdfr_kcj_popc(word & ((1u << bit) - 1u));
+}
+SDFR_KCJ_HD int sdfr_kcjd_rank(const uint32_t c[4], int q, int g) {
+    int front = 0;
+    for (int j = 0; j < (q >> 3); ++j) front += sdfr_kcj_popc(c[j]);
+    return sdfr_kcjd_rank_in_word(c[q >> 3], front, q, g);
+}
+SDFR_KCJ_HD int sdfr_kcjd_dead_pos(int tot) { return tot < 511 ? tot : 511; }
diff --git a/sdflabel_amd/csrc/mlp.hip b/sdflabel_amd/csrc/mlp.hip
--- a/sdflabel_amd/csrc/mlp.hip
+++ b/sdflabel_amd/csrc/mlp.hip
@@ -144,7 +144,7 @@
         SDFR_HIP_CHECK(hipMalloc(&d->d_Wkj, Wkj.size() * sizeof(float)));
         SDFR_HIP_CHECK(hipMemcpy(d->d_Wkj, Wkj.data(), Wkj.size() * sizeof(float), hipMemcpyHostToDevice));
         P.Wkj = d->d_Wkj;
-        P.jcompact = finite ? 1 : 0;
+        P.jcompact = finite ? 2 : 0;
     }
     P.Wf = d->d_Wf; P.Wb = d->d_Wb; P.Wh = d->d_Wh; P.Ws = d->d_Ws; P.Wbh = d->d_Wbh; P.bias = d->d_bias; P.w_last = d->d_wlast; P.fwd_np = 2;
     *out = d;
@@ -252,17 +252,17 @@
     return SDFR_OK;
 }
 
-extern "C" int sdfr_mlp_forward_balanced(const sdfr_decoder* d, const float* inputs, int64_t n, float* sdf, uint32_t* mask_ws, void* state,
-                                         int64_t order_rows, void* stream) {
-    SDFR_REQUIRE(d && inputs && sdf && state, "sdfr_mlp_forward_balanced: NULL argument");
-    SDFR_REQUIRE(n >= 0 && n < (int64_t)1 << 31, "sdfr_mlp_forward_balanced: n=%lld out of range", (long long)n);
-    SDFR_REQUIRE(order_rows > 0, "sdfr_mlp_forward_balanced: order_rows=%lld must be positive", (long long)order_rows);
-    SDFR_REQUIRE(n % order_rows == 0, "sdfr_mlp_forward_balanced: n=%lld is not a multiple of order_rows=%lld", (long long)n, (long long)order_rows);
-    SDFR_REQUIRE(d->HP == 512 && !d->has_ln, "sdfr_mlp_forward_balanced: needs a float32 decoder of padded width 512 without LayerNorm (this one: %d%s)",
+static int forward_balanced_impl(const char* who, bool rank, const sdfr_decoder* d, const float* inputs, int64_t n, float* sdf, uint32_t* mask_ws,
+                                 void* state, int64_t order_rows, void* stream) {
+    SDFR_REQUIRE(d && inputs && sdf && state, "%s: NULL argument", who);
+    SDFR_REQUIRE(n >= 0 && n < (int64_t)1 << 31, "%s: n=%lld out of range", who, (long long)n);
+    SDFR_REQUIRE(order_rows > 0, "%s: order_rows=%lld must be positive", who, (long long)order_rows);
+    SDFR_REQUIRE(n % order_rows == 0, "%s: n=%lld is not a multiple of order_rows=%lld", who, (long long)n, (long long)order_rows);
+    SDFR_REQUIRE(d->HP == 512 && !d->has_ln, "%s: needs a float32 decoder of padded width 512 without LayerNorm (this one: %d%s)", who,
                  d->HP, d->has_ln ? ", LayerNorm" : "");
     SDFR_REQUIRE(!mask_ws || ((n + 127) / 128) * 128 * (int64_t)(d->n_lin - 1) < (int64_t)1 << 31,
-                 "sdfr_mlp_forward_balanced: n=%lld rows with masks of %d layers exceed the kernel's line index", (long long)n, d->n_lin - 1);
-    SDFR_DEVICE_CHECK(d, "sdfr_mlp_forward_balanced");
+                 "%s: n=%lld rows with masks of %d layers exceed the kernel's line index", who, (long long)n, d->n_lin - 1);
+    SDFR_DEVICE_CHECK(d, who);
     if (n == 0) return SDFR_OK;
     int32_t* st = (int32_t*)state;
     const bool ranked = sdfr_tb_ranked(order_rows);
@@ -273,11 +273,21 @@
     P.tile_at = st + sdfr_tb_at_word(order_rows);
     sdfr_launch_fwd_f32_512_ordered(P, n, st + sdfr_tb_order_word(order_rows), order_rows, (hipStream_t)stream);
     SDFR_LAUNCH_CHECK();
-    if (ranked) {
+    if (ranked && rank) {
         sdfr_launch_tile_balance(st, order_rows, (hipStream_t)stream);
         SDFR_LAUNCH_CHECK();
     }
     return SDFR_OK;
+}
+
+extern "C" int sdfr_mlp_forward_balanced(const sdfr_decoder* d, const float* inputs, int64_t n, float* sdf, uint32_t* mask_ws, void* state,
+                                         int64_t order_rows, void* stream) {
+    return forward_balanced_impl("sdfr_mlp_forward_balanced", true, d, inputs, n, sdf, mask_ws, state, order_rows, stream);
+}
+
+extern "C" int sdfr_mlp_forward_balanced_deferred(const sdfr_decoder* d, const float* inputs, int64_t n, float* sdf, uint32_t* mask_ws, void* state,
+                                                  int64_t order_rows, void* stream) {
+    return forward_balanced_impl("sdfr_mlp_forward_balanced_deferred", false, d, inputs, n, sdf, mask_ws, state, order_rows, stream);
 }
 
 #ifndef SDFR_COUNTED_TILE16_ROWS
diff --git a/sdflabel_amd/csrc/mlp_balance.hip b/sdflabel_amd/csrc/mlp_balance.hip
--- a/sdflabel_amd/csrc/mlp_balance.hip
+++ b/sdflabel_amd/csrc/mlp_balance.hip
@@ -1,8 +1,6 @@
 #include <hip/hip_runtime.h>
 #include "sdfr_common.h"
-#include "tile_balance.h"
-
-constexpr int TB_NT = 256, TB_WAVES = TB_NT / 64;
+#include "tile_balance_rank.h"
 
 __global__ __launch_bounds__(256) void sdfr_tile_balance_init_kernel(int32_t* __restrict__ state, const int32_t* __restrict__ order, int64_t order_rows) {
     const int64_t i = (int64_t)blockIdx.x * blockDim.x + threadIdx.x;
@@ -16,41 +14,7 @@
 }
 
 __global__ __launch_bounds__(TB_NT) void sdfr_tile_balance_kernel(int32_t* __restrict__ state, int64_t order_rows) {
-    __shared__ int32_t cost[SDFR_TB_MAX_CHUNKS];
-    __shared__ int last_reader;
-    const int T = (int)sdfr_tb_chunks(order_rows), full = (int)sdfr_tb_full_chunks(order_rows);
-    int32_t* g_cost = state + sdfr_tb_cost_word(order_rows);
-    int32_t* g_last = state + sdfr_tb_last_word(order_rows);
-    int32_t* g_at = state + sdfr_tb_at_word(order_rows);
-    int32_t* ctl = state + sdfr_tb_ctl_word(order_rows);
-    int32_t* order = state + sdfr_tb_order_word(order_rows);
-    const int32_t* fixed = state + sdfr_tb_fixed_word(order_rows);
-    const int tid = threadIdx.x, lane = tid & 63, wave = tid >> 6;
-    const int c = (int)blockIdx.x * TB_WAVES + wave;
-    const int64_t i = (int64_t)c * SDFR_TB_CHUNK + lane;
-    const bool moves = c < T && i < order_rows;
-    const int32_t entry = moves ? fixed[i] : 0;
-    for (int k = tid; k < T; k += TB_NT) cost[k] = g_cost[k];
-    __syncthreads();
-    if (c < T) {
-        int r = c;
-        if (c < full) {
-            r = sdfr_tb_rank_part(cost, full, c, lane, 64);
-#pragma unroll
-            for (int d = 32; d >= 1; d >>= 1) r += __shfl_xor(r, d, 64);
-        }
-        if (lane == 0) {
-            g_last[c] = cost[c];
-            g_at[r] = c;
-        }
-        if (moves) order[sdfr_tb_dest(c, r, lane, full)] = entry;
-    }
-    if (tid == 0) last_reader = atomicAdd(ctl, 1) == (int)gridDim.x - 1 ? 1 : 0;
-    __syncthreads();
-    if (last_reader) {
-        for (int k = tid; k < T; k += TB_NT) g_cost[k] = 0;
-        if (tid == 0) ctl[0] = 0;
-    }
+    sdfr_tb_rank_block<TB_NT>(state, order_rows, (int)blockIdx.x, (int)gridDim.x);
 }
 
 void sdfr_launch_tile_balance_init(int32_t* state, const int32_t* order, int64_t order_rows, hipStream_t s) {
@@ -59,5 +23,5 @@
 }
 
 void sdfr_launch_tile_balance(int32_t* state, int64_t order_rows, hipStream_t s) {
-    hipLaunchKernelGGL(sdfr_tile_balance_kernel, dim3(sdfr_cdiv(sdfr_tb_chunks(order_rows), TB_WAVES)), dim3(TB_NT), 0, s, state, order_rows);
+    hipLaunchKernelGGL(sdfr_tile_balance_kernel, dim3(sdfr_tb_rank_blocks(order_rows, TB_NT)), dim3(TB_NT), 0, s, state, order_rows);
 }
diff --git a/sdflabel_amd/csrc/mlp_jac.hip b/sdflabel_amd/csrc/mlp_jac.hip
--- a/sdflabel_amd/csrc/mlp_jac.hip
+++ b/sdflabel_amd/csrc/mlp_jac.hip
@@ -38,6 +38,8 @@
         MlpParams Q = P;
         const char* e = getenv("SDFR_JAC_COMPACT");
         if (e && e[0] == '0') Q.jcompact = 0;
+        const char* st = getenv("SDFR_JAC_STAGE");
+        if (st && st[0] == '0' && Q.jcompact) Q.jcompact = 1;
         hipLaunchKernelGGL((sdfr_mlp_kernel<float, 16, SDFR_JAC_SMALL_FT, 1, SDFR_JAC_SMALL_NW, SDFR_JAC_SMALL_PF, 3>), dim3(sdfr_cdiv(cap, 16), B),
                            dim3(64 * SDFR_JAC_SMALL_NW), 0, s, Q);
     }
diff --git a/sdflabel_amd/csrc/mlp_kernel.h b/sdflabel_amd/csrc/mlp_kernel.h
--- a/sdflabel_amd/csrc/mlp_kernel.h
+++ b/sdflabel_amd/csrc/mlp_kernel.h
@@ -2,6 +2,7 @@
 #include "sdfr_common.h"
 #include "kc_slots.h"
 #include "kcj_slots.h"
+#include "kcjd_slots.h"
 #include "tile_balance.h"
 #include <math.h>
 #include <type_traits>
@@ -1314,7 +1315,8 @@
     if constexpr (JAC) {
     uint32_t raw[NP * FT * RG];
     const bool kcj_on = KCJ && P.jcompact && P.Wkj;
-    uint32_t kcj_w[4] = {0u, 0u, 0u, 0u};
+    const bool kcj_fast = P.jcompact >= 2;
+    uint32_t kcj_w[4] = {0u, 0u, 0u, 0u}, kcj_c[4] = {0u, 0u, 0u, 0u};
     int kcj_n = 0;
     auto kcj_vote = [&](int l, const uint32_t* raw) {
         const int prev_out = P.L[l - 1].out_dim;
@@ -1337,6 +1339,14 @@
         x |= __builtin_amdgcn_update_dpp(0, x, 0x128, 0xf, 0xf, false);
 #pragma unroll
         for (int g = 0; g < 4; ++g) kcj_w[g] = (uint32_t)__builtin_amdgcn_readlane(x, 16 * g);
+        if (kcj_fast) {
+#pragma unroll
+            for (int j = 0; j < 4; ++j) {
+                const int part = (int)sdfr_kcjd_group_part((uint32_t)x, j, lg);
+                kcj_c[j] = (uint32_t)(__builtin_amdgcn_readlane(part, 0) | __builtin_amdgcn_readlane(part, 16) | __builtin_amdgcn_readlane(part, 32) |
+                                      __builtin_amdgcn_readlane(part, 48));
+            }
+        }
         if (lane == 0) reinterpret_cast<int*>(kcj_cnt4)[wave] = sdfr_kcj_count(kcj_w[0], kcj_w[1], kcj_w[2], kcj_w[3]);
     };
     const bool kcj_top = kcj_on && P.n_mfma >= 2;
@@ -1522,6 +1532,18 @@
                 off = __builtin_amdgcn_readfirstlane(off);
                 tot = __builtin_amdgcn_readfirstlane(tot);
                 const uint32_t mine = lg == 0 ? kcj_w[0] : lg == 1 ? kcj_w[1] : lg == 2 ? kcj_w[2] : kcj_w[3];
+                if (kcj_fast) {
+                    int cfront[4];
+                    cfront[0] = off;
+#pragma unroll
+                    for (int j = 1; j < 4; ++j) cfront[j] = cfront[j - 1] + sdfr_kcj_popc(kcj_c[j - 1]);
+                    const int dead = sdfr_kcjd_dead_pos(tot);
+#pragma unroll
+                    for (int q = 0; q < 32; ++q) {
+                        const int pos = ((mine >> q) & 1u) ? sdfr_kcjd_rank_in_word(kcj_c[q >> 3], cfront[q >> 3], q, lg) : dead;
+                        act_e[sdfr_kcj_elem(pos, lp)] = acc[q >> 2][0][q & 3];
+                    }
+                } else {
                 int n = off;
 #pragma unroll
                 for (int q = 0; q < 32; ++q) {
@@ -1530,6 +1552,7 @@
                     const int front = ((b0 << 2) | ((b0 + b1) << 4) | ((b0 + b1 + b2) << 6)) >> (2 * lg) & 3;
                     if ((mine >> q) & 1u) act_e[sdfr_kcj_elem(n + front, lp)] = acc[q >> 2][0][q & 3];
                     n += b0 + b1 + b2 + b3;
+                }
                 }
 #pragma unroll
                 for (int h = 0; h < 2; ++h) {
diff --git a/sdflabel_amd/csrc/tile_balance_rank.h b/sdflabel_amd/csrc/tile_balance_rank.h
--- /dev/null
+++ b/sdflabel_amd/csrc/tile_balance_rank.h
@@ -0,0 +1,46 @@
+#pragma once
+#include <hip/hip_runtime.h>
+#include "tile_balance.h"
+
+constexpr int TB_NT = 256;
+
+static inline int sdfr_tb_rank_blocks(int64_t order_rows, int nt) { return (int)((sdfr_tb_chunks(order_rows) + nt / 64 - 1) / (nt / 64)); }
+
+template <int NT>
+__device__ __forceinline__ void sdfr_tb_rank_block(int32_t* __restrict__ state, int64_t order_rows, int blk, int nblk) {
+    __shared__ int32_t cost[SDFR_TB_MAX_CHUNKS];
+    __shared__ int last_reader;
+    const int T = (int)sdfr_tb_chunks(order_rows), full = (int)sdfr_tb_full_chunks(order_rows);
+    int32_t* g_cost = state + sdfr_tb_cost_word(order_rows);
+    int32_t* g_last = state + sdfr_tb_last_word(order_rows);
+    int32_t* g_at = state + sdfr_tb_at_word(order_rows);
+    int32_t* ctl = state + sdfr_tb_ctl_word(order_rows);
+    int32_t* order = state + sdfr_tb_order_word(order_rows);
+    const int32_t* fixed = state + sdfr_tb_fixed_word(order_rows);
+    const int tid = threadIdx.x, lane = tid & 63, wave = tid >> 6;
+    const int c = blk * (NT / 64) + wave;
+    const int64_t i = (int64_t)c * SDFR_TB_CHUNK + lane;
+    const bool moves = c < T && i < order_rows;
+    const int32_t entry = moves ? fixed[i] : 0;
+    for (int k = tid; k < T; k += NT) cost[k] = g_cost[k];
+    __syncthreads();
+    if (c < T) {
+        int r = c;
+        if (c < full) {
+            r = sdfr_tb_rank_part(cost, full, c, lane, 64);
+#pragma unroll
+            for (int d = 32; d >= 1; d >>= 1) r += __shfl_xor(r, d, 64);
+        }
+        if (lane == 0) {
+            g_last[c] = cost[c];
+            g_at[r] = c;
+        }
+        if (moves) order[sdfr_tb_dest(c, r, lane, full)] = entry;
+    }
+    if (tid == 0) last_reader = atomicAdd(ctl, 1) == nblk - 1 ? 1 : 0;
+    __syncthreads();
+    if (last_reader) {
+        for (int k = tid; k < T; k += NT) g_cost[k] = 0;
+        if (tid == 0) ctl[0] = 0;
+    }
+}
```

Result: faster. 56.97 million rays/s, median of 6 (+1.1%).
